# sbokov/AddingDisparityFiltering

Measured on AMD Instinct MI355X. Metric: filtered Mpixels/s (+ achieved HBM GB/s) on 4K disparity, 1/2/4/8 GPUs vs CPU ref, higher is better.
Workload: dtype f32

## Files before the change

### addingdisparityfiltering_amd/__init__.py

```python
from .ximgproc import (
    AdfError,
    COLOR_BGR2GRAY,
    DisparityFilter,
    DisparityWLSFilter,
    FastGlobalSmootherFilter,
    INTER_LINEAR,
    PATH_CONF_BAND,
    PATH_FUSED_FIRST_PASS,
    PATH_MERGED_PREP,
    PATH_SCALED_FUSED,
    PATH_SCALED_HALF,
    SOLVER_EXACT,
    SOLVER_WAVE,
    StereoBM,
    StereoMatcher,
    StereoSGBM,
    UNKNOWN_DISPARITY,
    computeBadPixelPercent,
    computeMSE,
    createDisparityWLSFilter,
    createDisparityWLSFilterGeneric,
    createFastGlobalSmootherFilter,
    createRightMatcher,
    cvtColor,
    fastGlobalSmootherFilter,
    filterSpeckles,
    releaseCachedMemory,
    getDisparityVis,
    halfSize,
    matcherViews,
    readGT,
    resize,
    speckleWorkspaceBytes,
)

__version__ = "0.1.0"
```

### addingdisparityfiltering_amd/_lib.py

```python
import ctypes as C
import os

_HERE = os.path.dirname(os.path.abspath(__file__))
LIB_PATH = os.environ.get("ADF_WLS_LIB") or os.path.join(_HERE, "libadf_wls.so")

ADF_OK, ADF_EBADARG, ADF_ESIZE, ADF_EHIP, ADF_ENOMEM, ADF_ENODEV = range(6)
SOLVER_EXACT, SOLVER_WAVE = 0, 1
PATH_CONF_BAND, PATH_FUSED_FIRST_PASS, PATH_MERGED_PREP, PATH_SCALED_FUSED, PATH_SCALED_HALF = 1, 2, 4, 8, 16
DEPTH_8U, DEPTH_16S, DEPTH_32F = 0, 3, 5


class AdfError(RuntimeError):

    def __init__(self, code, msg):
        super().__init__("adf error %d: %s" % (code, msg))
        self.code = code


class KernelTime(C.Structure):
    _fields_ = [("name", C.c_char * 48), ("launches", C.c_int), ("total_ms", C.c_double),
                ("alg_bytes", C.c_double), ("moved_bytes", C.c_double)]


class Rect(C.Structure):
    _fields_ = [("x", C.c_int), ("y", C.c_int), ("width", C.c_int), ("height", C.c_int)]


_vp, _i, _d, _pd, _sz = C.c_void_p, C.c_int, C.c_double, C.c_ssize_t, C.c_size_t
_FILTER_DEV = [_vp, _i, _vp, _pd, _pd, _vp, _pd, _pd, _i, _i, _i, _vp, _pd, _pd, _vp, _pd, _pd,
               C.POINTER(Rect), _vp]
_FILTER_SCALED_DEV = [_vp, _i, _vp, _pd, _pd, _i, _i, _vp, _pd, _pd, _i, _i, _i, _vp, _pd, _pd, _vp, _pd, _pd,
                      C.POINTER(Rect), _vp]
SYMBOLS = [
    ("adf_version", _i, []),
    ("adf_last_error", C.c_char_p, []),
    ("adf_device_count", _i, []),
    ("adf_device_pci_bus_id", _i, [_i, C.c_char_p, _i]),
    ("adf_wls_create", _i, [C.POINTER(_vp), _i, _i, _i, _i, _i, _i]),
    ("adf_wls_destroy", None, [_vp]),
    ("adf_wls_set_lambda", _i, [_vp, _d]),
    ("adf_wls_get_lambda", _i, [_vp, C.POINTER(_d)]),
    ("adf_wls_set_sigma_color", _i, [_vp, _d]),
    ("adf_wls_get_sigma_color", _i, [_vp, C.POINTER(_d)]),
    ("adf_wls_set_lrc_thresh", _i, [_vp, _i]),
    ("adf_wls_get_lrc_thresh", _i, [_vp, C.POINTER(_i)]),
    ("adf_wls_set_depth_discontinuity_radius", _i, [_vp, _i]),
    ("adf_wls_get_depth_discontinuity_radius", _i, [_vp, C.POINTER(_i)]),
    ("adf_wls_set_fgs_params", _i, [_vp, _d, _i]),
    ("adf_wls_set_solver", _i, [_vp, _i]),
    ("adf_wls_get_solver", _i, [_vp, C.POINTER(_i)]),
    ("adf_wls_get_last_solver", _i, [_vp, C.POINTER(_i)]),
    ("adf_wls_get_last_path", _i, [_vp, C.POINTER(_i)]),
    ("adf_wls_filter_device", _i, _FILTER_DEV),
    ("adf_wls_filter_host", _i, _FILTER_DEV[:-1]),
    ("adf_wls_filter_scaled_device", _i, _FILTER_SCALED_DEV),
    ("adf_wls_filter_scaled_host", _i, _FILTER_SCALED_DEV[:-1]),
    ("adf_wls_get_confidence_device", _i, [_vp, _i, _vp, _pd, _vp]),
    ("adf_wls_get_confidence_host", _i, [_vp, _i, _vp, _pd]),
    ("adf_wls_get_device", _i, [_vp, C.POINTER(_i)]),
    ("adf_wls_get_roi", _i, [_vp, C.POINTER(Rect)]),
    ("adf_wls_sync", _i, [_vp, _vp]),
    ("adf_wls_workspace_bytes", _sz, [_vp]),
    ("adf_wls_profile_enable", _i, [_vp, _i]),
    ("adf_wls_profile_read", _i, [_vp, _vp, _i, C.POINTER(_i)]),
    ("adf_fgs_create", _i, [C.POINTER(_vp), _vp, _pd, _i, _i, _i, _d, _d, _d, _i, _i]),
    ("adf_fgs_create_device", _i, [C.POINTER(_vp), _vp, _pd, _i, _i, _i, _d, _d, _d, _i, _i, _vp]),
    ("adf_fgs_destroy", None, [_vp]),
    ("adf_release_cached_memory", None, []),
    ("adf_weight_table_host", _i, [C.c_float, _vp, _i]),
    ("adf_fgs_get_device", _i, [_vp, C.POINTER(_i)]),
    ("adf_fgs_get_solver", _i, [_vp, C.POINTER(_i)]),
    ("adf_fgs_filter_host", _i, [_vp, _vp, _pd, _vp, _pd, _i, _i]),
    ("adf_fgs_filter_device", _i, [_vp, _vp, _pd, _vp, _pd, _i, _i, _vp]),
    ("adf_compute_mse_host", _i, [_vp, _pd, _vp, _pd, _i, _i, C.POINTER(Rect), C.POINTER(_d)]),
    ("adf_compute_mse_device", _i, [_vp, _pd, _vp, _pd, _i, _i, C.POINTER(Rect), C.POINTER(_d), _vp]),
    ("adf_compute_bad_pixel_percent_host", _i, [_vp, _pd, _vp, _pd, _i, _i, C.POINTER(Rect), _i, C.POINTER(_d)]),
    ("adf_compute_bad_pixel_percent_device", _i, [_vp, _pd, _vp, _pd, _i, _i, C.POINTER(Rect), _i, C.POINTER(_d), _vp]),
    ("adf_get_disparity_vis_host", _i, [_vp, _pd, _vp, _pd, _i, _i, _d]),
    ("adf_get_disparity_vis_device", _i, [_vp, _pd, _vp, _pd, _i, _i, _d, _vp]),
    ("adf_bm_create", _i, [C.POINTER(_vp), _i, _i]),
    ("adf_bm_destroy", None, [_vp]),
    ("adf_bm_set_params", _i, [_vp, _i, _i, _i, _i, _i, _i]),
    ("adf_bm_get_device", _i, [_vp, C.POINTER(_i)]),
    ("adf_bm_get_params", _i, [_vp] + [C.POINTER(_i)] * 6),
    ("adf_bm_compute_device", _i, [_vp, _i, _vp, _pd, _pd, _vp, _pd, _pd, _i, _i, _vp, _pd, _pd, _vp]),
    ("adf_bm_compute_both_device", _i, [_vp, _i, _vp, _pd, _pd, _vp, _pd, _pd, _i, _i, _vp, _pd, _pd, _vp, _pd, _pd, _vp]),
    ("adf_bm_compute_host", _i, [_vp, _i, _vp, _pd, _pd, _vp, _pd, _pd, _i, _i, _vp, _pd, _pd]),
    ("adf_sgbm_create", _i, [C.POINTER(_vp), _i, _i, _i]),
    ("adf_sgbm_destroy", None, [_vp]),
    ("adf_sgbm_get_device", _i, [_vp, C.POINTER(_i)]),
    ("adf_sgbm_set_params", _i, [_vp] + [_i] * 8),
    ("adf_sgbm_get_params", _i, [_vp] + [C.POINTER(_i)] * 8),
    ("adf_sgbm_set_disp12_max_diff", _i, [_vp, _i]),
    ("adf_sgbm_get_disp12_max_diff", _i, [_vp, C.POINTER(_i)]),
    ("adf_sgbm_compute_device", _i, [_vp, _i, _vp, _pd, _pd, _vp, _pd, _pd, _i, _i, _i, _vp, _pd, _pd, _vp]),
    ("adf_sgbm_compute_host", _i, [_vp, _i, _vp, _pd, _pd, _vp, _pd, _pd, _i, _i, _i, _vp, _pd, _pd]),
    ("adf_filter_speckles_workspace_bytes", _sz, [_i, _i, _i]),
    ("adf_filter_speckles_device", _i, [_i, _vp, _pd, _pd, _i, _i, _i, _i, _i, _vp, _sz, _vp]),
    ("adf_filter_speckles_host", _i, [_i, _vp, _pd, _pd, _i, _i, _i, _i, _i]),
    ("adf_half_size", _i, [_i, C.POINTER(_i)]),
    ("adf_prepare_views_device", _i, [_i, _vp, _pd, _pd, _i, _i, _i, _vp, _pd, _pd, _i, _i, _i, _vp]),
    ("adf_prepare_views_host", _i, [_i, _vp, _pd, _pd, _i, _i, _i, _vp, _pd, _pd, _i, _i, _i]),
]

_lib = None


def lib():
    global _lib
    if _lib is None:
        if not os.path.exists(LIB_PATH):
            raise ImportError(
                "%s is missing: build the HIP extension first "
                "(python -c 'import __graft_entry__ as g; g.build()')" % LIB_PATH)
        L = C.CDLL(LIB_PATH)
        for name, res, args in SYMBOLS:
            try:
                fn = getattr(L, name)
            except AttributeError:
                if os.environ.get("ADF_WLS_LIB"):
                    continue
                raise
            fn.restype = res
            fn.argtypes = args
        _lib = L
    return _lib


def check(rc):
    if rc != ADF_OK:
        raise AdfError(rc, lib().adf_last_error().decode("utf-8", "replace"))


def device_pci_bus_id(device):
    buf = C.create_string_buffer(64)
    check(lib().adf_device_pci_bus_id(int(device), buf, 64))
    return buf.value.decode()
```

### addingdisparityfiltering_amd/csrc/adf_api.hip

```cpp
#include "adf_host.h"

#include <cmath>
#include <cstdio>
#include <cstdlib>
#include <cstring>
#include <new>

using namespace adf;

static inline int round_up(int v, int m) { return (v + m - 1) / m * m; }

static Geom make_geom(int W, int H, int rx, int ry, int rw, int rh)
{
    Geom g;
    g.W = W; g.H = H; g.rx = rx; g.ry = ry; g.rw = rw; g.rh = rh;
    g.pw = round_up(rw, 64);
    g.ph = round_up(rh, 64);
    size_t a = (size_t)round_up(rh, TILE_ROWS) * g.pw, b = (size_t)rw * g.ph;
    g.plane = ((a > b ? a : b) + 63) / 64 * 64;
    g.frame = (size_t)W * H;
    g.cx0 = (4 - (rx & 3)) & 3;
    g.cpitch = round_up(W + g.cx0 + 3, 4);
    g.cframe = (size_t)g.cpitch * H;
    return g;
}

static Geom plain_conf_layout(Geom g) { g.cx0 = 0; g.cpitch = g.W; g.cframe = g.frame; return g; }

enum KClass { K_FILL = 0, K_WEIGHTS, K_DISC, K_LRC, K_PROLOGUE, K_PASS_H_FIRST, K_PASS_H, K_PASS_V, K_PASS_V_LAST, K_RESIZE, K_COUNT };
static const char* const kclass_names[K_COUNT] = {"fill_outside", "weights", "discontinuity", "lrc_confidence",
                                                  "plain_prologue", "pass_h_first", "pass_h", "pass_v", "pass_v_last", "resize"};
struct Profiler {
    bool on = false;
    struct Rec { int cls; hipEvent_t a, b; double alg, moved; };
    std::vector<Rec> recs;
    std::vector<hipEvent_t> pool;
    hipEvent_t get()
    {
        if (!pool.empty()) { hipEvent_t e = pool.back(); pool.pop_back(); return e; }
        hipEvent_t e = nullptr;
        if (hipEventCreate(&e) != hipSuccess) return nullptr;
        return e;
    }
    void clear() { for (auto& r : recs) { pool.push_back(r.a); pool.push_back(r.b); } recs.clear(); }
    void destroy() { clear(); for (auto e : pool) hipEventDestroy(e); pool.clear(); }
};
struct ProfScope {
    Profiler* p; hipStream_t st; Profiler::Rec r{};
    ProfScope(Profiler* prof, int cls, double alg, double moved, hipStream_t s) : p(prof && prof->on ? prof : nullptr), st(s)
    {
        if (!p) return;
        r.cls = cls; r.alg = alg; r.moved = moved; r.a = p->get(); r.b = p->get();
        if (r.a) hipEventRecord(r.a, st);
    }
    ~ProfScope()
    {
        if (!p) return;
        if (r.b) hipEventRecord(r.b, st);
        if (r.a && r.b) p->recs.push_back(r);
    }
};

struct SolvePlanes {
    float* CH; float* CV;
    float* D; float* F0; float* F1;
    float* A0; float* A1;
    float* B0; float* B1;
};

struct FinalOut {
    int epilogue; void* out; ptrdiff_t stride, pair_stride; int x0, y0, cn, c;
};

static double epilogue_bytes(int epilogue) { return epilogue == EPI_F32 ? 4.0 : epilogue == EPI_U8 ? 1.0 : 2.0; }

template <class Args>
static void set_final_out(Args& a, const FinalOut& fo)
{
    a.out = fo.out; a.out_stride = fo.stride; a.out_pair_stride = fo.pair_stride;
    a.out_x0 = fo.x0; a.out_y0 = fo.y0; a.out_cn = fo.cn; a.out_c = fo.c;
}

static int run_passes(bool wave, const Geom& g, const SolvePlanes& p, int n_rhs, float lambda, float atten, int num_iter,
                      const FinalOut& fo, int n_pairs, hipStream_t st, Profiler* prof = nullptr,
                      const FusedInputs* fuse = nullptr)
{
    const double px = (double)g.rw * g.rh * n_pairs;
    float lam = lambda;
    for (int it = 0; it < num_iter; it++, lam *= atten) {
        const bool fused = it == 0 && fuse, last = it == num_iter - 1;
        const int epi = last ? fo.epilogue : EPI_PLANES;
        const double lo_b = (fused && fuse->lo_conf) ? 6.0 * fuse->lo_scale_x * fuse->lo_scale_y : 6.0;
        const double hb = fused ? (4.0 + lo_b + 8.0) * px : (4.0 + 8.0 * n_rhs) * px;
        const double out_b = (last ? epilogue_bytes(fo.epilogue) : 4.0 * n_rhs) * px;
        const double vb = (4.0 + 4.0 * n_rhs) * px + out_b;
        if (wave) {
            WavePassArgs h{}, v{};
            h.C = p.CH; h.U0 = p.A0; h.U1 = p.A1;
            h.nscan = g.rh; h.len = g.rw; h.pitch = g.pw; h.plane = g.plane; h.lambda = lam;
            if (fused) h.fuse = *fuse;
            v.C = p.CV; v.U0 = p.A0; v.U1 = p.A1;
            v.nscan = g.rw; v.len = g.rh; v.pitch = g.pw; v.plane = g.plane; v.lambda = lam;
            if (last) set_final_out(v, fo);
            {
                ProfScope ps(prof, fused ? K_PASS_H_FIRST : K_PASS_H, hb, hb, st);
                HIP_TRY(launch_wave_hpass(h, n_rhs, n_pairs, st));
            }
            ProfScope ps(prof, last ? K_PASS_V_LAST : K_PASS_V, vb, vb, st);
            HIP_TRY(launch_wave_vpass(v, n_rhs, epi, n_pairs, st));
        } else {
            PassArgs h{}, v{};
            h.C = p.CH; h.U0 = p.A0; h.U1 = p.A1; h.D = p.D; h.F0 = p.F0; h.F1 = p.F1; h.O0 = p.B0; h.O1 = p.B1;
            h.nscan = g.rh; h.len = g.rw; h.pitch_in = g.ph; h.pitch_out = g.pw; h.plane = g.plane; h.lambda = lam;
            v.C = p.CV; v.U0 = p.B0; v.U1 = p.B1; v.D = p.D; v.F0 = p.F0; v.F1 = p.F1; v.O0 = p.A0; v.O1 = p.A1;
            v.nscan = g.rw; v.len = g.rh; v.pitch_in = g.pw; v.pitch_out = g.ph; v.plane = g.plane; v.lambda = lam;
            if (last) set_final_out(v, fo);
            {
                ProfScope ps(prof, K_PASS_H, hb, (12.0 + 16.0 * n_rhs) * px, st);
                HIP_TRY(launch_exact_pass(h, n_rhs, EPI_PLANES, n_pairs, st));
            }
            ProfScope ps(prof, last ? K_PASS_V_LAST : K_PASS_V, vb, (12.0 + 12.0 * n_rhs) * px + out_b, st);
            HIP_TRY(launch_exact_pass(v, n_rhs, epi, n_pairs, st));
        }
    }
    return ADF_OK;
}

static bool wave_fits(const Geom& g)
{
    return g.rw >= 2 && g.rh >= 2 && g.rw <= wave_max_row_len() && g.rh <= wave_max_col_len();
}

struct ConfResize {
    float* clo; int dW, dH; adf_rect rlo;
    Geom ghi;
    bool band_map;
    int n_pairs;
};

struct adf_wls {
    int device = 0;
    int left_offset = 0, right_offset = 0, top_offset = 0, bottom_offset = 0;
    int min_disp = 0;
    bool use_confidence = true;
    double lambda = 8000.0, sigma_color = 1.0;
    int lrc_thresh = 24, disc_radius = 5;
    float roll_off = 0.001f;
    double atten = 0.25; int num_iter = 3;
    int solver = ADF_SOLVER_WAVE;
    int last_solver = ADF_SOLVER_WAVE;
    adf_rect roi{0, 0, 0, 0};
    int last_W = 0, last_H = 0, last_pairs = 0;
    int last_cpitch = 0, last_cx0 = 0;
    long long conf_sig[4] = {0, 0, 0, 0};
    int last_path = 0;
    Lut lut;
    DevBuf ws;
    DevBuf conf;
    DevBuf stage;
    DevBuf scaled;
    size_t ws_limit = (size_t)64 << 30;
    Profiler prof;
    long long ws_sig[8] = {0, 0, 0, 0, 0, 0, 0, 0};
    hipStream_t side = nullptr;
    hipEvent_t ev_fork = nullptr, ev_join = nullptr;
    bool overlap = true;
    struct LazyConf { bool pending = false; ConfResize resize{}; } lazy_conf;
    bool scaled_half = true;
    bool scaled_fuse = true;
    bool conf_band = true;
    bool merge_small = true;
    static bool null_caller_of(hipStream_t s) { return s == nullptr || s == hipStreamLegacy || s == hipStreamPerThread; }
    int ensure_side(hipStream_t caller)
    {
        if (side) return ADF_OK;
        int least = 0, greatest = 0, prio = 0, cp = 0;
        if (hipDeviceGetStreamPriorityRange(&least, &greatest) != hipSuccess) { least = greatest = 0; (void)hipGetLastError(); }
        if (null_caller_of(caller) || stream_is_capturing(caller) || hipStreamGetPriority(caller, &cp) != hipSuccess) { cp = 0; (void)hipGetLastError(); }
        prio = (cp != greatest) ? greatest : (greatest < least ? greatest + 1 : greatest);
        if (null_caller_of(caller)) HIP_TRY(hipStreamCreateWithFlags(&side, hipStreamNonBlocking));
        else HIP_TRY(hipStreamCreateWithPriority(&side, hipStreamNonBlocking, prio));
        HIP_TRY(hipEventCreateWithFlags(&ev_fork, hipEventDisableTiming));
        HIP_TRY(hipEventCreateWithFlags(&ev_join, hipEventDisableTiming));
        return ADF_OK;
    }
};

extern "C" int adf_wls_create(adf_wls_t** out, int use_confidence, int l, int r, int t, int b, int min_disp)
{
    if (!out) return fail(ADF_EBADARG, "adf_wls_create: out is NULL");
    *out = nullptr;
    if (l < 0 || r < 0 || t < 0 || b < 0) return fail(ADF_EBADARG, "adf_wls_create: negative offset");
    int n = 0;
    if (hipGetDeviceCount(&n) != hipSuccess || n <= 0)
        return fail(ADF_ENODEV, "adf_wls_create: no HIP device visible");
    adf_wls* h = new (std::nothrow) adf_wls();
    if (!h) return fail(ADF_ENOMEM, "adf_wls_create: out of host memory");
    if (hipGetDevice(&h->device) != hipSuccess) { delete h; return fail(ADF_EHIP, "hipGetDevice failed"); }
    h->use_confidence = use_confidence != 0;
    h->left_offset = l; h->right_offset = r; h->top_offset = t; h->bottom_offset = b;
    h->min_disp = 0; (void)min_disp;
    if (const char* e = getenv("ADF_WS_LIMIT_GB")) {
        double gb = atof(e);
        if (gb > 0) h->ws_limit = (size_t)(gb * (double)((size_t)1 << 30));
    }
    if (const char* e = getenv("ADF_NO_OVERLAP")) h->overlap = atoi(e) == 0;
    if (const char* e = getenv("ADF_CONF_BAND")) h->conf_band = atoi(e) != 0;
    if (const char* e = getenv("ADF_SCALED_FUSE")) h->scaled_fuse = atoi(e) != 0;
    if (const char* e = getenv("ADF_LO_HALF")) h->scaled_half = atoi(e) != 0;
    if (const char* e = getenv("ADF_MERGE_SMALL")) h->merge_small = atoi(e) != 0;
    *out = h;
    return ADF_OK;
}

extern "C" void adf_wls_destroy(adf_wls_t* h)
{
    if (!h) return;
    DeviceScope ds(h->device);
    h->lut.release(); h->ws.release(); h->conf.release(); h->stage.release(); h->scaled.release();
    h->prof.destroy();
    if (h->ev_fork) hipEventDestroy(h->ev_fork);
    if (h->ev_join) hipEventDestroy(h->ev_join);
    if (h->side) hipStreamDestroy(h->side);
    delete h;
}


extern "C" int adf_wls_set_lambda(adf_wls_t* h, double v) { NEED_HANDLE(h); h->lambda = v; return ADF_OK; }
extern "C" int adf_wls_get_lambda(const adf_wls_t* h, double* v) { NEED_HANDLE(h); if (v) *v = h->lambda; return ADF_OK; }
extern "C" int adf_wls_set_sigma_color(adf_wls_t* h, double v) { NEED_HANDLE(h); h->sigma_color = v; return ADF_OK; }
extern "C" int adf_wls_get_sigma_color(const adf_wls_t* h, double* v) { NEED_HANDLE(h); if (v) *v = h->sigma_color; return ADF_OK; }
extern "C" int adf_wls_set_lrc_thresh(adf_wls_t* h, int v) { NEED_HANDLE(h); h->lrc_thresh = v; return ADF_OK; }
extern "C" int adf_wls_get_lrc_thresh(const adf_wls_t* h, int* v) { NEED_HANDLE(h); if (v) *v = h->lrc_thresh; return ADF_OK; }
extern "C" int adf_wls_set_depth_discontinuity_radius(adf_wls_t* h, int v) { NEED_HANDLE(h); h->disc_radius = v; return ADF_OK; }
extern "C" int adf_wls_get_depth_discontinuity_radius(const adf_wls_t* h, int* v) { NEED_HANDLE(h); if (v) *v = h->disc_radius; return ADF_OK; }

extern "C" int adf_wls_set_fgs_params(adf_wls_t* h, double atten, int num_iter)
{
    NEED_HANDLE(h);
    if (num_iter < 1) return fail(ADF_EBADARG, "num_iter must be >= 1 (FGS.cpp:143)");
    h->atten = atten; h->num_iter = num_iter;
    return ADF_OK;
}

extern "C" int adf_wls_set_solver(adf_wls_t* h, int solver)
{
    NEED_HANDLE(h);
    if (solver != ADF_SOLVER_EXACT && solver != ADF_SOLVER_WAVE) return fail(ADF_EBADARG, "unknown solver %d", solver);
    h->solver = solver;
    return ADF_OK;
}
extern "C" int adf_wls_get_solver(const adf_wls_t* h, int* v) { NEED_HANDLE(h); if (v) *v = h->solver; return ADF_OK; }
extern "C" int adf_wls_get_last_solver(const adf_wls_t* h, int* v) { NEED_HANDLE(h); if (v) *v = h->last_solver; return ADF_OK; }
extern "C" int adf_wls_get_last_path(const adf_wls_t* h, int* v) { NEED_HANDLE(h); if (v) *v = h->last_path; return ADF_OK; }

extern "C" int adf_wls_get_device(const adf_wls_t* h, int* device) { NEED_HANDLE(h); if (device) *device = h->device; return ADF_OK; }
extern "C" int adf_wls_get_roi(const adf_wls_t* h, adf_rect* roi) { NEED_HANDLE(h); if (roi) *roi = h->roi; return ADF_OK; }
extern "C" size_t adf_wls_workspace_bytes(const adf_wls_t* h)
{
    return h ? h->ws.bytes + h->conf.bytes + h->stage.bytes + h->scaled.bytes + h->lut.bytes() : 0;
}

extern "C" int adf_wls_sync(adf_wls_t* h, void* stream)
{
    NEED_HANDLE(h);
    DeviceScope ds(h->device);
    HIP_TRY(hipStreamSynchronize((hipStream_t)stream));
    return ADF_OK;
}

static int ensure_conf_planes(adf_wls* h, const Geom& g, int n_pairs, hipStream_t st)
{
    int rc = h->conf.reserve(g.cframe * sizeof(float) * (size_t)n_pairs, st, FILL_ZERO);
    if (rc) return rc;
    const long long sig[4] = {g.W, g.H, g.cx0, n_pairs};
    if (memcmp(sig, h->conf_sig, sizeof(sig)) != 0) {
        HIP_TRY(hipMemsetAsync(h->conf.p, 0, h->conf.bytes, st));
        memcpy(h->conf_sig, sig, sizeof(sig));
    }
    return ADF_OK;
}

static size_t wls_pair_ws_bytes(const Geom& g, bool conf, bool wave, bool disc_maps)
{
    size_t planes = wave ? (conf ? 4 : 3) : (conf ? 9 : 6);
    return planes * g.plane * sizeof(float) + (conf && disc_maps ? 2 * g.frame * sizeof(float) : 0);
}

static int resolve_roi(const adf_wls* h, const adf_rect* roi_in, int w, int hgt, adf_rect& roi)
{
    if (roi_in && roi_in->width * roi_in->height != 0) roi = *roi_in;
    else roi = adf_rect{h->left_offset, h->top_offset, w - h->left_offset - h->right_offset, hgt - h->top_offset - h->bottom_offset};
    if (roi.width <= 0 || roi.height <= 0 || roi.x < 0 || roi.y < 0 || roi.x + roi.width > w || roi.y + roi.height > hgt)
        return fail(ADF_ESIZE, "ROI (%d,%d,%d,%d) does not fit a %dx%d map", roi.x, roi.y, roi.width, roi.height, w, hgt);
    return ADF_OK;
}

static int check_right_map(const int16_t* dispR, ptrdiff_t sR, int w)
{
    if (!dispR) return fail(ADF_EBADARG, "disparity_map_right is required with use_confidence");
    if (sR < (ptrdiff_t)w * 2) return fail(ADF_ESIZE, "right disparity stride smaller than a row");
    return ADF_OK;
}

static int check_radius(const adf_wls* h)
{
    if (h->disc_radius < 0 || h->disc_radius > max_disc_radius())
        return fail(ADF_EBADARG, "depth discontinuity radius %d outside [0,%d]", h->disc_radius, max_disc_radius());
    return ADF_OK;
}

static float* const UNALLOCATED = reinterpret_cast<float*>(uintptr_t(256));

static WavePassArgs first_pass_probe(const FusedInputs& f, int len)
{
    WavePassArgs a{};
    a.fuse = f; a.len = len;
    return a;
}

static FusedInputs view_fuse(const float* conf, const int16_t* dl, ptrdiff_t sL, ptrdiff_t psL, const Geom& g)
{
    FusedInputs f{};
    f.conf_in = conf; f.conf_frame = g.cframe; f.conf_pitch = g.cpitch; f.conf_x0 = g.cx0 + g.rx; f.conf_y0 = g.ry;
    f.dl_in = dl; f.dl_stride = sL; f.dl_pair_stride = psL; f.dl_x0 = g.rx; f.dl_y0 = g.ry;
    return f;
}

struct ScaledStage {
    const int16_t* dispL; ptrdiff_t sL, psL;
    const int16_t* dispR; ptrdiff_t sR, psR;
    float resize_factor, x_ratio;
    char* dhi; size_t dhi_bytes;
    float *cl, *cr;
    ConfResize lo;
    bool fuse_lo;
    float* taps;
};

static FusedInputs lo_fuse(const adf_wls* h, const ScaledStage& s, int first, const Geom& g)
{
    const ConfResize& c = s.lo;
    const size_t lo = (size_t)c.dW * c.dH;
    FusedInputs f{};
    f.lo_conf = c.clo + (size_t)first * lo; f.lo_conf_stride = c.dW; f.lo_conf_pair = (ptrdiff_t)lo;
    f.lo_dl = (const int16_t*)((const char*)s.dispL + (ptrdiff_t)first * s.psL); f.lo_dl_stride = s.sL; f.lo_dl_pair = s.psL;
    f.lo_w = c.dW; f.lo_h = c.dH; f.hi_x0 = g.rx; f.hi_y0 = g.ry;
    f.lo_scale_x = (double)c.dW / c.ghi.W; f.lo_scale_y = (double)c.dH / c.ghi.H; f.lo_post_scale = s.x_ratio;
    if (c.band_map) {
        f.lo_zero_outside = 1; f.lo_vx0 = c.rlo.x; f.lo_vy0 = c.rlo.y; f.lo_vx1 = c.rlo.x + c.rlo.width; f.lo_vy1 = c.rlo.y + c.rlo.height;
    }
    f.lo_taps = s.taps; f.lo_half = h->scaled_half ? 1 : 0;
    return f;
}

static int resize_conf_planes(adf_wls_t* h, const ConfResize& c, hipStream_t st, Profiler* prof)
{
    const size_t lo = (size_t)c.dW * c.dH;
    const Geom& ghi = c.ghi;
    const double Fhi = (double)ghi.W * ghi.H * c.n_pairs;
    ResizeArgs rc32{c.clo, (ptrdiff_t)c.dW * 4, (ptrdiff_t)(lo * 4), c.dW, c.dH, (float*)h->conf.p + ghi.cx0, (ptrdiff_t)ghi.cpitch * 4,
                    (ptrdiff_t)(ghi.cframe * 4), ghi.W, ghi.H, (double)c.dW / ghi.W, (double)c.dH / ghi.H, 1.0f, 0};
    if (c.band_map) { rc32.zero_outside = 1; rc32.vx0 = c.rlo.x; rc32.vy0 = c.rlo.y; rc32.vx1 = c.rlo.x + c.rlo.width; rc32.vy1 = c.rlo.y + c.rlo.height; }
    ProfScope ps(prof, K_RESIZE, 4.0 * Fhi + 4.0 * (double)lo * c.n_pairs, 4.0 * Fhi + 4.0 * (double)lo * c.n_pairs, st);
    HIP_TRY(launch_resize_linear(rc32, c.n_pairs, st));
    return ADF_OK;
}

static int scaled_conf_map(adf_wls_t* h, const ScaledStage& s, hipStream_t st, Profiler* prof)
{
    const ConfResize& c = s.lo;
    const Geom glo = plain_conf_layout(make_geom(c.dW, c.dH, c.rlo.x, c.rlo.y, c.rlo.width, c.rlo.height));
    const size_t lo = (size_t)c.dW * c.dH;
    const double Plo = (double)c.rlo.width * c.rlo.height * c.n_pairs;
    const int rrx = c.dW - (c.rlo.x + c.rlo.width);
    const float roll_off = h->roll_off / (s.resize_factor * s.resize_factor);
    const int thresh_lo = (int)(s.resize_factor * h->lrc_thresh);
    if (c.band_map) {
        ConfBandArgs ba{s.dispL, s.sL, s.psL, s.dispR, s.sR, s.psR, c.clo, glo, rrx, thresh_lo, h->disc_radius, roll_off, 0};
        ProfScope ps(prof, K_LRC, 8.0 * Plo, 8.0 * Plo, st);
        HIP_TRY(launch_conf_band(ba, c.n_pairs, st));
        return ADF_OK;
    }
    DiscArgs da{{s.dispL, s.dispR}, {s.sL, s.sR}, {s.psL, s.psR}, {c.rlo.x, rrx}, c.rlo.y, c.rlo.width, c.rlo.height,
                h->disc_radius, roll_off, {s.cl, s.cr}, c.dW, lo, -1};
    {
        ProfScope ps(prof, K_DISC, 4.0 * Plo, 12.0 * Plo, st);
        HIP_TRY(launch_discontinuity(da, c.n_pairs, st));
    }
    LrcArgs la{s.dispL, s.sL, s.psL, s.dispR, s.sR, s.psR, s.cl, s.cr, c.clo, nullptr, 0, 0, 0, nullptr, nullptr, glo, rrx, thresh_lo, ORIENT_N};
    ProfScope ps(prof, K_LRC, 4.0 * (double)lo * c.n_pairs, 4.0 * (double)lo * c.n_pairs + 12.0 * Plo, st);
    HIP_TRY(launch_lrc_prologue(la, c.n_pairs, st));
    return ADF_OK;
}

static int scaled_resize(adf_wls_t* h, const ScaledStage& s, hipStream_t st, Profiler* prof)
{
    const ConfResize& c = s.lo;
    int rc = h->use_confidence ? resize_conf_planes(h, c, st, prof) : ADF_OK;
    if (rc) return rc;
    const int W = c.ghi.W, H = c.ghi.H;
    const size_t lo = (size_t)c.dW * c.dH;
    const double Fhi = (double)W * H * c.n_pairs;
    ResizeArgs r16{s.dispL, s.sL, s.psL, c.dW, c.dH, s.dhi, (ptrdiff_t)W * 2, (ptrdiff_t)s.dhi_bytes, W, H, (double)c.dW / W, (double)c.dH / H, s.x_ratio, 1};
    ProfScope ps(prof, K_RESIZE, 2.0 * Fhi + 2.0 * (double)lo * c.n_pairs, 2.0 * Fhi + 2.0 * (double)lo * c.n_pairs, st);
    HIP_TRY(launch_resize_linear(r16, c.n_pairs, st));
    return ADF_OK;
}

enum ConfStage {
    CONF_NONE,
    CONF_SCALED,
    CONF_SCALED_LO,
    CONF_MERGED,
    CONF_BAND,
    CONF_LEFT,
    CONF_TWO_KERNEL,
};

struct ChunkPlan {
    ConfStage stage;
    bool fork_weights;
    bool outside_on_side;
};

struct WlsPlan {
    bool wave;
    bool fused_first;
    bool band;
    size_t per_pair; int chunk;
    ChunkPlan full, tail;
    int path;
};

static ChunkPlan plan_chunk(const adf_wls* h, ConfStage stage, bool wave)
{
    const bool fork = stage != CONF_NONE && stage != CONF_MERGED && h->overlap;
    return ChunkPlan{stage, fork, fork && wave && stage != CONF_TWO_KERNEL};
}

static WlsPlan plan_wls(const adf_wls* h, const Geom& g, int n_pairs, const int16_t* dispL, ptrdiff_t sL, ptrdiff_t psL,
                        ptrdiff_t sG, int gch, const ScaledStage* scaled)
{
    WlsPlan p{};
    const bool conf = h->use_confidence;
    p.wave = h->solver == ADF_SOLVER_WAVE && wave_fits(g);
    ConfStage stage = !conf ? CONF_NONE
                    : scaled ? (scaled->fuse_lo ? CONF_SCALED_LO : CONF_SCALED)
                    : (p.wave && h->disc_radius <= conf_left_max_radius()) ? CONF_LEFT : CONF_TWO_KERNEL;
    const float* planes = h->conf.p ? (const float*)h->conf.p : UNALLOCATED;
    p.fused_first = stage == CONF_SCALED_LO ||
                    ((stage == CONF_SCALED || stage == CONF_LEFT) && p.wave &&
                     wave_hpass_can_fuse(first_pass_probe(view_fuse(planes, dispL, sL, psL, g), g.rw)));
    p.band = stage == CONF_LEFT && p.fused_first && h->conf_band && conf_band_fits(g, h->disc_radius);
    if (p.band) stage = CONF_BAND;
    p.per_pair = wls_pair_ws_bytes(g, conf, p.wave, !p.band);
    p.chunk = (int)(h->ws_limit / p.per_pair);
    if (p.chunk < 1) p.chunk = 1;
    if (p.chunk > n_pairs) p.chunk = n_pairs;
    auto chunk_of = [&](int n) {
        const bool merged = p.band && h->merge_small && prep_small_fits(g, h->disc_radius, gch, n) && prep_small_guide_fits(g, sG, gch);
        return plan_chunk(h, merged ? CONF_MERGED : stage, p.wave);
    };
    p.full = chunk_of(p.chunk);
    p.tail = chunk_of(n_pairs % p.chunk ? n_pairs % p.chunk : p.chunk);
    p.path = ((p.band || (scaled && scaled->lo.band_map)) ? ADF_PATH_CONF_BAND : 0) |
             (p.fused_first ? ADF_PATH_FUSED_FIRST_PASS : 0) |
             ((p.full.stage == CONF_MERGED || p.tail.stage == CONF_MERGED) ? ADF_PATH_MERGED_PREP : 0);
    if (stage == CONF_SCALED_LO)
        p.path |= ADF_PATH_SCALED_FUSED |
                  (wave_hpass_lo_half(first_pass_probe(lo_fuse(h, *scaled, 0, g), g.rw)) ? ADF_PATH_SCALED_HALF : 0);
    return p;
}

static int wls_filter_impl(adf_wls_t* h, int n_pairs,
                           const int16_t* dispL, ptrdiff_t sL, ptrdiff_t psL,
                           const uint8_t* view, ptrdiff_t sG, ptrdiff_t psG, int gch, int W, int H,
                           int16_t* out, ptrdiff_t sO, ptrdiff_t psO,
                           const int16_t* dispR, ptrdiff_t sR, ptrdiff_t psR,
                           const adf_rect* roi_in, hipStream_t st, const ScaledStage* scaled = nullptr)
{
    NEED_HANDLE(h);
    if (!dispL || W <= 0 || H <= 0) return fail(ADF_EBADARG, "disparity_map_left is empty");
    if (!view || (gch != 1 && gch != 3)) return fail(ADF_EBADARG, "left_view must be CV_8UC1 or CV_8UC3");
    if (!out) return fail(ADF_EBADARG, "filtered_disparity_map is NULL");
    if (n_pairs < 1) return fail(ADF_EBADARG, "n_pairs must be >= 1");
    if (sL < (ptrdiff_t)W * 2 || sO < (ptrdiff_t)W * 2 || sG < (ptrdiff_t)W * gch)
        return fail(ADF_ESIZE, "row stride smaller than a row");
    const bool conf = h->use_confidence;
    int rc;
    if (conf && !scaled && (rc = check_right_map(dispR, sR, W))) return rc;
    if (h->lambda < 0 || h->sigma_color < 0) return fail(ADF_EBADARG, "lambda and sigma_color must be >= 0 (FGS.cpp:143)");
    adf_rect roi;
    if ((rc = resolve_roi(h, roi_in, W, H, roi))) return rc;
    if (conf && (rc = check_radius(h))) return rc;

    DeviceScope ds(h->device);
    const Geom g = make_geom(W, H, roi.x, roi.y, roi.width, roi.height);
    h->lazy_conf.pending = false;
    h->roi = roi; h->last_W = W; h->last_H = H; h->last_pairs = n_pairs;
    h->last_cpitch = g.cpitch; h->last_cx0 = g.cx0; h->last_path = 0;

    if ((rc = h->lut.ensure((float)h->sigma_color, st))) return rc;
    const WlsPlan plan = plan_wls(h, g, n_pairs, dispL, sL, psL, sG, gch, scaled);
    const bool wave = plan.wave;
    h->last_solver = wave ? ADF_SOLVER_WAVE : ADF_SOLVER_EXACT;
    if ((rc = h->ws.reserve(plan.per_pair * (size_t)plan.chunk, st, FILL_ZERO))) return rc;
    if (conf && !scaled && (rc = ensure_conf_planes(h, g, n_pairs, st))) return rc;
    {
        const long long sig[8] = {W, H, roi.x, roi.y, roi.width, roi.height, (long long)plan.band * 4 + (long long)wave * 2 + conf, plan.chunk};
        if (memcmp(sig, h->ws_sig, sizeof(sig)) != 0) {
            HIP_TRY(hipMemsetAsync(h->ws.p, 0, h->ws.bytes, st));
            memcpy(h->ws_sig, sig, sizeof(sig));
        }
    }
    float* base = (float*)h->ws.p;
    auto take = [&](size_t elems) { float* p = base; base += elems * (size_t)plan.chunk; return p; };
    SolvePlanes p{};
    p.CH = take(g.plane); p.CV = take(g.plane); p.A0 = take(g.plane);
    if (!wave) { p.D = take(g.plane); p.F0 = take(g.plane); p.B0 = take(g.plane); }
    float *cL = nullptr, *cR = nullptr;
    if (conf) {
        p.A1 = take(g.plane);
        if (!wave) { p.F1 = take(g.plane); p.B1 = take(g.plane); }
        if (!plan.band) { cL = take(g.frame); cR = take(g.frame); }
    }
    const int orient_h = wave ? ORIENT_N : ORIENT_T;
    const int orient_u2 = wave ? ORIENT_PAIR : ORIENT_T;
    const int orient_cv = wave ? ORIENT_STRIP : ORIENT_N;
    const int16_t fill = (int16_t)(16 * (h->min_disp - 1));
    const int rrx = W - (roi.x + roi.width);
    const int thresh = (int)(1.0f * h->lrc_thresh);
    Profiler* prof = &h->prof;
    h->last_path = plan.path;

    for (int first = 0; first < n_pairs; first += plan.chunk) {
        const int n = (n_pairs - first < plan.chunk) ? n_pairs - first : plan.chunk;
        const ChunkPlan& cp = n == plan.chunk ? plan.full : plan.tail;
        const int16_t* dL = (const int16_t*)((const char*)dispL + (ptrdiff_t)first * psL);
        const int16_t* dR = dispR ? (const int16_t*)((const char*)dispR + (ptrdiff_t)first * psR) : nullptr;
        const uint8_t* gv = view + (ptrdiff_t)first * psG;
        int16_t* o = (int16_t*)((char*)out + (ptrdiff_t)first * psO);
        float* confp = conf ? (float*)h->conf.p + (size_t)first * g.cframe : nullptr;
        const double F = (double)g.frame * n, P = (double)g.rw * g.rh * n;
        OutsideArgs oa{o, sO, psO, fill, scaled ? nullptr : confp, g};
        const double ob = (oa.conf ? 6.0 : 2.0) * (F - P);
        auto fill_outside = [&](hipStream_t s) { ProfScope ps(prof, K_FILL, ob, ob, s); return launch_outside(oa, n, s); };
        WeightArgs wa{gv, sG, psG, gch, h->lut.cur, p.CH, p.CV, orient_h, orient_cv, g,
                      wave ? nullptr : p.B0};
        ConfBandArgs ba{dL, sL, psL, dR, sR, psR, confp, g, rrx, thresh, h->disc_radius, h->roll_off, 0};
        DiscArgs da{{dL, dR}, {sL, sR}, {psL, psR}, {roi.x, rrx}, roi.y, roi.width, roi.height, h->disc_radius, h->roll_off,
                    {cL, cR}, W, g.frame, cp.stage == CONF_LEFT ? 1 : -1};
        const FusedInputs fuse = cp.stage == CONF_SCALED_LO ? lo_fuse(h, *scaled, first, g) : view_fuse(confp, dL, sL, psL, g);

        hipStream_t wst = st;
        if (cp.fork_weights) {
            if ((rc = h->ensure_side(st))) return rc;
            HIP_TRY(hipEventRecord(h->ev_fork, st));
            HIP_TRY(hipStreamWaitEvent(h->side, h->ev_fork, 0));
            wst = h->side;
        }
        if (cp.stage == CONF_NONE || cp.outside_on_side) HIP_TRY(fill_outside(wst));
        if (cp.stage == CONF_NONE && scaled && first == 0 && (rc = scaled_resize(h, *scaled, st, prof))) return rc;
        if (cp.stage != CONF_MERGED) {
            ProfScope ps(prof, K_WEIGHTS, (gch + 8.0) * P, (gch + 8.0) * P, wst);
            HIP_TRY(launch_weights(wa, n, wst));
        }
        if (cp.fork_weights) HIP_TRY(hipEventRecord(h->ev_join, h->side));

        switch (cp.stage) {
        case CONF_NONE: {
            PlainPrologueArgs pa{dL, sL, psL, ADF_16S, 1, 0, p.A0, g, orient_h};
            ProfScope ps(prof, K_PROLOGUE, 6.0 * P, 6.0 * P, st);
            HIP_TRY(launch_plain_prologue(pa, n, st));
            break;
        }
        case CONF_SCALED: {
            if (!cp.outside_on_side) HIP_TRY(fill_outside(st));
            if (first == 0 && ((rc = scaled_conf_map(h, *scaled, st, prof)) || (rc = scaled_resize(h, *scaled, st, prof)))) return rc;
            if (plan.fused_first) break;
            PlainPrologueArgs pa{dL, sL, psL, ADF_16S, 1, 0, p.A0, g, orient_u2, confp, p.A1};
            ProfScope ps(prof, K_PROLOGUE, 14.0 * P, 14.0 * P, st);
            HIP_TRY(launch_plain_prologue(pa, n, st));
            break;
        }
        case CONF_SCALED_LO:
            if (!cp.outside_on_side) HIP_TRY(fill_outside(st));
            if (first != 0) break;
            if ((rc = scaled_conf_map(h, *scaled, st, prof))) return rc;
            if (!stream_is_capturing(st)) h->lazy_conf = adf_wls::LazyConf{true, scaled->lo};
            else if ((rc = resize_conf_planes(h, scaled->lo, st, prof))) return rc;
            break;
        case CONF_MERGED: {
            const double b = (8.0 + gch + 8.0) * P + 6.0 * (F - P);
            ProfScope ps(prof, K_LRC, b, b, st);
            HIP_TRY(launch_prep_small(ba, wa, oa, n, st));
            break;
        }
        case CONF_BAND: {
            {
                ProfScope ps(prof, K_LRC, 8.0 * P, 8.0 * P, st);
                HIP_TRY(launch_conf_band(ba, n, st));
            }
            if (!cp.outside_on_side) HIP_TRY(fill_outside(st));
            break;
        }
        case CONF_LEFT: {
            {
                ProfScope ps(prof, K_DISC, 2.0 * P, 6.0 * P, st);
                HIP_TRY(launch_discontinuity(da, n, st));
            }
            const bool fused = plan.fused_first;
            ConfLeftArgs ca{dL, sL, psL, dR, sR, psR, cR, confp, fused ? nullptr : p.A0, fused ? nullptr : p.A1,
                            g, rrx, thresh, h->disc_radius, h->roll_off};
            {
                const double wu = fused ? 0.0 : 8.0;
                ProfScope ps(prof, K_LRC, (4.0 + wu) * P, (12.0 + wu) * P, st);
                HIP_TRY(launch_conf_left(ca, n, st));
            }
            if (!cp.outside_on_side) HIP_TRY(fill_outside(st));
            break;
        }
        case CONF_TWO_KERNEL: {
            {
                ProfScope ps(prof, K_DISC, 4.0 * P, 12.0 * P, st);
                HIP_TRY(launch_discontinuity(da, n, st));
            }
            LrcArgs la{dL, sL, psL, dR, sR, psR, cL, cR, confp, o, sO, psO, fill, p.A0, p.A1, g, rrx, thresh, orient_u2};
            ProfScope ps(prof, K_LRC, 4.0 * F + 8.0 * P + 2.0 * (F - P), 4.0 * F + 20.0 * P + 2.0 * (F - P), st);
            HIP_TRY(launch_lrc_prologue(la, n, st));
            break;
        }
        }
        if (cp.fork_weights) HIP_TRY(hipStreamWaitEvent(st, h->ev_join, 0));
        FinalOut fo{conf ? EPI_WLS_CONF : EPI_I16, o, sO, psO, roi.x, roi.y, 1, 0};
        rc = run_passes(wave, g, p, conf ? 2 : 1, (float)h->lambda, (float)h->atten, h->num_iter, fo, n, st, prof,
                        plan.fused_first ? &fuse : nullptr);
        if (rc) return rc;
    }
    return ADF_OK;
}

extern "C" int adf_wls_filter_device(adf_wls_t* h, int n_pairs,
                                     const int16_t* dispL, ptrdiff_t sL, ptrdiff_t psL,
                                     const uint8_t* view, ptrdiff_t sG, ptrdiff_t psG, int gch, int W, int H,
                                     int16_t* out, ptrdiff_t sO, ptrdiff_t psO,
                                     const int16_t* dispR, ptrdiff_t sR, ptrdiff_t psR,
                                     const adf_rect* roi_in, void* stream)
{
    return wls_filter_impl(h, n_pairs, dispL, sL, psL, view, sG, psG, gch, W, H, out, sO, psO, dispR, sR, psR, roi_in,
                           (hipStream_t)stream);
}

extern "C" int adf_wls_filter_scaled_device(adf_wls_t* h, int n_pairs,
                                            const int16_t* dispL, ptrdiff_t sL, ptrdiff_t psL, int dW, int dH,
                                            const uint8_t* view, ptrdiff_t sG, ptrdiff_t psG, int gch, int W, int H,
                                            int16_t* out, ptrdiff_t sO, ptrdiff_t psO,
                                            const int16_t* dispR, ptrdiff_t sR, ptrdiff_t psR,
                                            const adf_rect* roi_in, void* stream)
{
    NEED_HANDLE(h);
    hipStream_t st = (hipStream_t)stream;
    if (dW == W && dH == H)
        return wls_filter_impl(h, n_pairs, dispL, sL, psL, view, sG, psG, gch, W, H, out, sO, psO, dispR, sR, psR, roi_in, st);
    if (!dispL || dW <= 0 || dH <= 0 || W <= 0 || H <= 0) return fail(ADF_EBADARG, "disparity_map_left is empty");
    if (n_pairs < 1) return fail(ADF_EBADARG, "n_pairs must be >= 1");
    if (sL < (ptrdiff_t)dW * 2) return fail(ADF_ESIZE, "row stride smaller than a row");
    const bool conf = h->use_confidence;
    int rc;
    if (conf && ((rc = check_right_map(dispR, sR, dW)) || (rc = check_radius(h)))) return rc;
    adf_rect rlo;
    if ((rc = resolve_roi(h, roi_in, dW, dH, rlo))) return rc;
    const float resize_factor = dW / (float)W;
    const float x_ratio = W / (float)dW, y_ratio = H / (float)dH;
    adf_rect rhi{(int)(rlo.x * x_ratio), (int)(rlo.y * y_ratio), (int)(rlo.width * x_ratio), (int)(rlo.height * y_ratio)};
    if (rhi.width <= 0 || rhi.height <= 0 || rhi.x + rhi.width > W || rhi.y + rhi.height > H)
        return fail(ADF_ESIZE, "scaled ROI (%d,%d,%d,%d) does not fit the %dx%d view", rhi.x, rhi.y, rhi.width, rhi.height, W, H);

    DeviceScope ds(h->device);
    h->lazy_conf.pending = false;
    const size_t lo = (size_t)dW * dH, hi = (size_t)W * H;
    const Geom ghi = make_geom(W, H, rhi.x, rhi.y, rhi.width, rhi.height);
    ScaledStage s{dispL, sL, psL, dispR, sR, psR, resize_factor, x_ratio, nullptr, 0, nullptr, nullptr,
                  ConfResize{UNALLOCATED, dW, dH, rlo, ghi, false, n_pairs}, false, nullptr};
    s.lo.band_map = conf && h->conf_band &&
                    conf_band_fits(plain_conf_layout(make_geom(dW, dH, rlo.x, rlo.y, rlo.width, rlo.height)), h->disc_radius);
    s.fuse_lo = conf && h->scaled_fuse && h->solver == ADF_SOLVER_WAVE && wave_fits(ghi) &&
                wave_hpass_can_fuse_lo(first_pass_probe(lo_fuse(h, s, 0, ghi), ghi.rw));
    s.dhi_bytes = s.fuse_lo ? 0 : (hi * 2 + 255) / 256 * 256;
    const size_t maps_bytes = ((size_t)n_pairs * (s.dhi_bytes + (conf ? 3 * lo * sizeof(float) : 0)) + 255) / 256 * 256;
    const size_t need = maps_bytes + (s.fuse_lo ? 2 * ((size_t)rhi.width + 4) * sizeof(float) : 0);
    if ((rc = h->scaled.reserve(need, st, FILL_ZERO))) return rc;
    s.dhi = (char*)h->scaled.p;
    s.cl = (float*)(s.dhi + (size_t)n_pairs * s.dhi_bytes);
    s.cr = s.cl + (size_t)n_pairs * lo;
    s.lo.clo = s.cr + (size_t)n_pairs * lo;
    s.taps = s.fuse_lo ? (float*)((char*)h->scaled.p + maps_bytes) : nullptr;
    if (conf && (rc = ensure_conf_planes(h, ghi, n_pairs, st))) return rc;
    rc = wls_filter_impl(h, n_pairs, s.fuse_lo ? dispL : (const int16_t*)s.dhi, (ptrdiff_t)W * 2, (ptrdiff_t)s.dhi_bytes,
                         view, sG, psG, gch, W, H, out, sO, psO, nullptr, 0, 0, &rhi, st, &s);
    h->roi = rlo;
    return rc;
}

extern "C" int adf_wls_filter_scaled_host(adf_wls_t* h, int n_pairs,
                                          const int16_t* dispL, ptrdiff_t sL, ptrdiff_t psL, int dW, int dH,
                                          const uint8_t* view, ptrdiff_t sG, ptrdiff_t psG, int gch, int W, int H,
                                          int16_t* out, ptrdiff_t sO, ptrdiff_t psO,
                                          const int16_t* dispR, ptrdiff_t sR, ptrdiff_t psR,
                                          const adf_rect* roi)
{
    NEED_HANDLE(h);
    if (!dispL || !view || !out || W <= 0 || H <= 0 || dW <= 0 || dH <= 0 || n_pairs < 1)
        return fail(ADF_EBADARG, "adf_wls_filter_host: empty input");
    if (gch != 1 && gch != 3) return fail(ADF_EBADARG, "left_view must be CV_8UC1 or CV_8UC3");
    if (h->use_confidence && !dispR) return fail(ADF_EBADARG, "disparity_map_right is required with use_confidence");
    DeviceScope ds(h->device);
    hipStream_t st = nullptr;
    const size_t dbytes = (size_t)dW * dH * 2, obytes = (size_t)W * H * 2, gbytes = (size_t)W * H * gch;
    const size_t dpad = (dbytes + 255) / 256 * 256, opad = (obytes + 255) / 256 * 256, gpad = (gbytes + 255) / 256 * 256;
    const size_t need = (size_t)n_pairs * (2 * dpad + opad + gpad);
    int rc = h->stage.reserve(need, st, FILL_ZERO);
    if (rc) return rc;
    char* dLd = (char*)h->stage.p;
    char* dRd = dLd + (size_t)n_pairs * dpad;
    char* od = dRd + (size_t)n_pairs * dpad;
    char* gd = od + (size_t)n_pairs * opad;
    if ((rc = copy_images(dLd, (size_t)dW * 2, dpad, dispL, sL, psL, (size_t)dW * 2, dH, n_pairs, hipMemcpyHostToDevice, st))) return rc;
    if (dispR && (rc = copy_images(dRd, (size_t)dW * 2, dpad, dispR, sR, psR, (size_t)dW * 2, dH, n_pairs, hipMemcpyHostToDevice, st))) return rc;
    if ((rc = copy_images(gd, (size_t)W * gch, gpad, view, sG, psG, (size_t)W * gch, H, n_pairs, hipMemcpyHostToDevice, st))) return rc;
    rc = adf_wls_filter_scaled_device(h, n_pairs, (const int16_t*)dLd, (ptrdiff_t)dW * 2, (ptrdiff_t)dpad, dW, dH,
                                      (const uint8_t*)gd, (ptrdiff_t)W * gch, (ptrdiff_t)gpad, gch, W, H,
                                      (int16_t*)od, (ptrdiff_t)W * 2, (ptrdiff_t)opad,
                                      dispR ? (const int16_t*)dRd : nullptr, (ptrdiff_t)dW * 2, (ptrdiff_t)dpad, roi, st);
    if (rc) return rc;
    if ((rc = copy_images(out, sO, psO, od, (size_t)W * 2, opad, (size_t)W * 2, H, n_pairs, hipMemcpyDeviceToHost, st))) return rc;
    HIP_TRY(hipStreamSynchronize(st));
    return ADF_OK;
}

extern "C" int adf_wls_filter_host(adf_wls_t* h, int n_pairs,
                                   const int16_t* dispL, ptrdiff_t sL, ptrdiff_t psL,
                                   const uint8_t* view, ptrdiff_t sG, ptrdiff_t psG, int gch, int W, int H,
                                   int16_t* out, ptrdiff_t sO, ptrdiff_t psO,
                                   const int16_t* dispR, ptrdiff_t sR, ptrdiff_t psR,
                                   const adf_rect* roi)
{
    return adf_wls_filter_scaled_host(h, n_pairs, dispL, sL, psL, W, H, view, sG, psG, gch, W, H, out, sO, psO,
                                      dispR, sR, psR, roi);
}

extern "C" int adf_wls_profile_enable(adf_wls_t* h, int on)
{
    NEED_HANDLE(h);
    DeviceScope ds(h->device);
    h->prof.clear();
    h->prof.on = on != 0;
    return ADF_OK;
}

extern "C" int adf_wls_profile_read(adf_wls_t* h, adf_kernel_time* out, int capacity, int* count)
{
    NEED_HANDLE(h);
    if (!out || !count || capacity < 1) return fail(ADF_EBADARG, "adf_wls_profile_read: bad output buffer");
    DeviceScope ds(h->device);
    adf_kernel_time acc[K_COUNT];
    memset(acc, 0, sizeof(acc));
    for (int k = 0; k < K_COUNT; k++) snprintf(acc[k].name, sizeof(acc[k].name), "%s", kclass_names[k]);
    for (auto& r : h->prof.recs) {
        HIP_TRY(hipEventSynchronize(r.b));
        float ms = 0.0f;
        HIP_TRY(hipEventElapsedTime(&ms, r.a, r.b));
        acc[r.cls].launches++; acc[r.cls].total_ms += ms; acc[r.cls].alg_bytes += r.alg; acc[r.cls].moved_bytes += r.moved;
    }
    int n = 0;
    for (int k = 0; k < K_COUNT && n < capacity; k++)
        if (acc[k].launches) out[n++] = acc[k];
    *count = n;
    return ADF_OK;
}

static int conf_copy(adf_wls_t* h, int pair, float* dst, ptrdiff_t stride, hipMemcpyKind kind, hipStream_t st)
{
    if (!dst) return fail(ADF_EBADARG, "confidence destination is NULL");
    if (!h->use_confidence || !h->conf.p || h->last_pairs == 0)
        return fail(ADF_EBADARG, "no confidence map: filter() has not run with use_confidence");
    if (pair < 0 || pair >= h->last_pairs) return fail(ADF_EBADARG, "pair %d out of range [0,%d)", pair, h->last_pairs);
    if (stride < (ptrdiff_t)h->last_W * 4) return fail(ADF_ESIZE, "confidence stride smaller than a row");
    if (h->lazy_conf.pending) {
        int rc = resize_conf_planes(h, h->lazy_conf.resize, st, nullptr);
// ... 214 lines not shown
```

### addingdisparityfiltering_amd/csrc/adf_host.h

```cpp
#pragma once

#include "adf_internal.h"
#include "../../include/adf_wls.h"

#include <memory>
#include <vector>

namespace adf {

int fail(int code, const char* fmt, ...);

#define HIP_TRY(expr)                                                                              \
    do {                                                                                           \
        hipError_t e_ = (expr);                                                                    \
        if (e_ != hipSuccess)                                                                      \
            return adf::fail(e_ == hipErrorOutOfMemory ? ADF_ENOMEM : ADF_EHIP, "%s failed: %s",   \
                             #expr, hipGetErrorString(e_));                                        \
    } while (0)
#define NEED_HANDLE(h) do { if (!(h)) return adf::fail(ADF_EBADARG, "%s: handle is NULL", __func__); } while (0)

struct DeviceScope {
    int prev = -1; bool switched = false;
    explicit DeviceScope(int dev)
    {
        if (hipGetDevice(&prev) == hipSuccess && prev != dev) switched = hipSetDevice(dev) == hipSuccess;
    }
    ~DeviceScope() { if (switched) hipSetDevice(prev); }
};

bool stream_is_capturing(hipStream_t st);

enum Fill { FILL_NONE, FILL_ZERO };
struct DevBuf {
    void* p = nullptr; size_t bytes = 0;
    int reserve(size_t need, hipStream_t st, Fill fill);
    void release() { if (p) hipFree(p); p = nullptr; bytes = 0; }
};

hipError_t device_malloc(void** p, size_t bytes);
void* cache_take(int device, size_t need, hipStream_t st, size_t* bytes);
void cache_give(int device, void* p, size_t bytes, hipStream_t st);
void cache_give_event(int device, void* p, size_t bytes, hipEvent_t ready);

struct Scratch {
    int device = 0; void* p = nullptr; size_t bytes = 0; hipStream_t st = nullptr;
    Scratch() = default;
    Scratch(const Scratch&) = delete;
    Scratch& operator=(const Scratch&) = delete;
    int take(size_t need, hipStream_t stream);
    ~Scratch() { if (p) cache_give(device, p, bytes, st); }
};

struct LutTable;
struct Lut {
    static constexpr int LUT_CACHE = 8;
    struct Entry { std::shared_ptr<LutTable> t; unsigned long long used; };
    std::vector<Entry> tables;
    const float* cur = nullptr;
    unsigned long long tick = 0;
    size_t bytes() const { return tables.size() * sizeof(float) * ADF_LUT_LEVELS; }
    int ensure(float s, hipStream_t st);
    void release() { tables.clear(); cur = nullptr; }
};

int copy_images(void* dst, size_t dst_pitch, ptrdiff_t dst_image_stride, const void* src, size_t src_pitch,
                ptrdiff_t src_image_stride, size_t row_bytes, size_t rows, int n, hipMemcpyKind kind, hipStream_t st);

}
```

### addingdisparityfiltering_amd/csrc/adf_host.hip

```cpp
#include "adf_host.h"

#include <cmath>
#include <cstdarg>
#include <cstdio>
#include <mutex>
#include <thread>

using namespace adf;

static thread_local char g_err[512] = "";

int adf::fail(int code, const char* fmt, ...)
{
    va_list ap;
    va_start(ap, fmt);
    vsnprintf(g_err, sizeof(g_err), fmt, ap);
    va_end(ap);
    return code;
}

extern "C" int adf_version(void) { return ADF_VERSION; }
extern "C" const char* adf_last_error(void) { return g_err; }
extern "C" int adf_device_count(void)
{
    int n = 0;
    if (hipGetDeviceCount(&n) != hipSuccess) return 0;
    return n;
}

extern "C" int adf_device_pci_bus_id(int device, char* buf, int len)
{
    if (!buf || len < 16) return fail(ADF_EBADARG, "adf_device_pci_bus_id: buffer of at least 16 bytes required");
    buf[0] = 0;
    HIP_TRY(hipDeviceGetPCIBusId(buf, len, device));
    return ADF_OK;
}

bool adf::stream_is_capturing(hipStream_t st)
{
    hipStreamCaptureStatus cs = hipStreamCaptureStatusNone;
    if (hipStreamIsCapturing(st, &cs) != hipSuccess) { (void)hipGetLastError(); return false; }
    return cs != hipStreamCaptureStatusNone;
}

int adf::DevBuf::reserve(size_t need, hipStream_t st, Fill fill)
{
    if (need <= bytes) return ADF_OK;
    if (p) { HIP_TRY(hipStreamSynchronize(st)); HIP_TRY(hipFree(p)); p = nullptr; bytes = 0; }
    need = (need + 255) / 256 * 256;
    HIP_TRY(device_malloc(&p, need));
    bytes = need;
    if (fill == FILL_ZERO) HIP_TRY(hipMemsetAsync(p, 0, need, st));
    return ADF_OK;
}

struct adf::LutTable {
    int device = 0; float sigma = 0; float* dev = nullptr;
    LutTable() = default;
    LutTable(const LutTable&) = delete;
    LutTable& operator=(const LutTable&) = delete;
    ~LutTable() { if (dev) { DeviceScope ds(device); hipFree(dev); } }
};

struct LutStore {
    static constexpr size_t CAP = 16;
    std::mutex m;
    std::vector<std::shared_ptr<LutTable>> tables;
    static LutStore& get() { static LutStore* s = new LutStore; return *s; }
    std::shared_ptr<LutTable> find(int device, float sigma)
    {
        std::lock_guard<std::mutex> lk(m);
        for (size_t k = 0; k < tables.size(); k++)
            if (tables[k]->device == device && tables[k]->sigma == sigma) {
                auto t = tables[k];
                tables.erase(tables.begin() + (ptrdiff_t)k); tables.push_back(t);
                return t;
            }
        return nullptr;
    }
    void add(const std::shared_ptr<LutTable>& t)
    {
        std::lock_guard<std::mutex> lk(m);
        if (tables.size() >= CAP) tables.erase(tables.begin());
        tables.push_back(t);
    }
    void clear() { std::lock_guard<std::mutex> lk(m); tables.clear(); }
};

static void lut_build_host(float s, float* host)
{
    auto span = [&](int a, int b) { for (int i = a; i < b; i++) host[i] = -expf(-sqrtf((float)i) / s); };
    int n = ADF_LUT_LEVELS;
    if (s > 0.0f) {
        const double lim = 110.0 * (double)s;
        if (lim * lim * 1.001 + 2.0 < (double)ADF_LUT_LEVELS) {
            int i0 = (int)(lim * lim * 1.001) + 2;
            while (i0 < ADF_LUT_LEVELS && !(-sqrtf((float)i0) / s <= -110.0f)) i0++;
            n = i0;
        }
    }
    for (int i = n; i < ADF_LUT_LEVELS; i++) host[i] = -0.0f;
    unsigned hw = std::thread::hardware_concurrency();
    int nt = (int)(hw >= 16 ? 8 : hw >= 4 ? hw / 2 : 1);
    if (n < 32768) nt = 1;
    if (nt <= 1) { span(0, n); return; }
    std::vector<std::thread> th;
    const int per = (n + nt - 1) / nt;
    bool ok = true;
    int done = std::min(per, n);
    for (int t = 1; t < nt && ok; t++) {
        const int a = t * per, b = std::min(n, a + per);
        if (a >= b) break;
        try { th.emplace_back(span, a, b); done = b; } catch (...) { ok = false; }
    }
    span(0, std::min(per, n));
    for (auto& t : th) t.join();
    if (done < n) span(done, n);
}

int adf::Lut::ensure(float s, hipStream_t st)
{
    for (auto& e : tables)
        if (e.t->sigma == s) { e.used = ++tick; cur = e.t->dev; return ADF_OK; }
    if ((int)tables.size() >= LUT_CACHE) {
        size_t lru = 0;
        for (size_t k = 1; k < tables.size(); k++) if (tables[k].used < tables[lru].used) lru = k;
        HIP_TRY(hipStreamSynchronize(st));
        tables.erase(tables.begin() + (ptrdiff_t)lru);
    }
    int device = 0;
    HIP_TRY(hipGetDevice(&device));
    std::shared_ptr<LutTable> t = LutStore::get().find(device, s);
    if (!t) {
        std::vector<float> host(ADF_LUT_LEVELS);
        lut_build_host(s, host.data());
        float* d = nullptr;
        HIP_TRY(hipMalloc(&d, sizeof(float) * ADF_LUT_LEVELS));
        hipError_t e = hipMemcpy(d, host.data(), sizeof(float) * ADF_LUT_LEVELS, hipMemcpyHostToDevice);
        if (e != hipSuccess) { hipFree(d); return fail(ADF_EHIP, "LUT upload failed: %s", hipGetErrorString(e)); }
        t = std::make_shared<LutTable>();
        t->device = device; t->sigma = s; t->dev = d;
        LutStore::get().add(t);
    }
    tables.push_back(Entry{t, ++tick});
    cur = t->dev;
    return ADF_OK;
}

struct BlockCache {
    struct Ent { int device; void* p; size_t bytes; hipEvent_t ready; };
    static constexpr size_t CAP_BYTES = (size_t)3 << 30;
    static constexpr size_t CAP_ENTRIES = 8;
    std::mutex m;
    std::vector<Ent> ents;
    size_t total = 0;
    static BlockCache& get() { static BlockCache* c = new BlockCache; return *c; }
    static void drop(const Ent& e)
    {
        DeviceScope ds(e.device);
        if (e.ready) { hipEventSynchronize(e.ready); hipEventDestroy(e.ready); }
        hipFree(e.p);
    }
    void* take(int device, size_t need, hipStream_t st, size_t* bytes)
    {
        Ent hit{};
        {
            std::lock_guard<std::mutex> lk(m);
            size_t best = ents.size();
            for (size_t k = 0; k < ents.size(); k++)
                if (ents[k].device == device && ents[k].bytes >= need && ents[k].bytes <= need + need / 4 + ((size_t)1 << 20) &&
                    (best == ents.size() || ents[k].bytes < ents[best].bytes))
                    best = k;
            if (best == ents.size()) return nullptr;
            hit = ents[best];
            ents.erase(ents.begin() + (ptrdiff_t)best);
            total -= hit.bytes;
        }
        if (hit.ready) {
            const hipError_t e = hipStreamWaitEvent(st, hit.ready, 0);
            if (e != hipSuccess) hipEventSynchronize(hit.ready);
            hipEventDestroy(hit.ready);
        }
        *bytes = hit.bytes;
        return hit.p;
    }
    void give(int device, void* p, size_t bytes, hipEvent_t ready)
    {
        std::vector<Ent> out;
        {
            std::lock_guard<std::mutex> lk(m);
            ents.push_back(Ent{device, p, bytes, ready});
            total += bytes;
            while (!ents.empty() && (total > CAP_BYTES || ents.size() > CAP_ENTRIES)) {
                out.push_back(ents.front());
                total -= ents.front().bytes;
                ents.erase(ents.begin());
            }
        }
        for (auto& e : out) drop(e);
    }
    void clear()
    {
        std::vector<Ent> out;
        { std::lock_guard<std::mutex> lk(m); out.swap(ents); total = 0; }
        for (auto& e : out) drop(e);
    }
};

extern "C" int adf_weight_table_host(float sigma_color, float* table, int levels)
{
    if (!table || levels != ADF_LUT_LEVELS) return fail(ADF_EBADARG, "table must hold %d floats", ADF_LUT_LEVELS);
    if (!(sigma_color >= 0.0f)) return fail(ADF_EBADARG, "sigma_color must be >= 0 (FGS.cpp:143)");
    lut_build_host(sigma_color, table);
    return ADF_OK;
}

namespace adf {
hipError_t device_malloc(void** p, size_t bytes)
{
    hipError_t e = hipMalloc(p, bytes);
    if (e == hipErrorOutOfMemory) {
        (void)hipGetLastError();
        BlockCache::get().clear();
        e = hipMalloc(p, bytes);
    }
    if (e != hipSuccess) *p = nullptr;
    return e;
}

void* cache_take(int device, size_t need, hipStream_t st, size_t* bytes) { return BlockCache::get().take(device, need, st, bytes); }

void cache_give(int device, void* p, size_t bytes, hipStream_t st)
{
    hipEvent_t ev = nullptr;
    if (hipEventCreateWithFlags(&ev, hipEventDisableTiming) != hipSuccess || hipEventRecord(ev, st) != hipSuccess) {
        (void)hipGetLastError();
        if (ev) hipEventDestroy(ev);
        ev = nullptr;
        hipStreamSynchronize(st);
    }
    BlockCache::get().give(device, p, bytes, ev);
}

void cache_give_event(int device, void* p, size_t bytes, hipEvent_t ready) { BlockCache::get().give(device, p, bytes, ready); }

int Scratch::take(size_t need, hipStream_t stream)
{
    if (hipGetDevice(&device) != hipSuccess) return fail(ADF_ENODEV, "no HIP device");
    st = stream;
    if ((p = cache_take(device, need, st, &bytes))) return ADF_OK;
    HIP_TRY(device_malloc(&p, need));
    bytes = need;
    return ADF_OK;
}

int copy_images(void* dst, size_t dst_pitch, ptrdiff_t dst_image_stride, const void* src, size_t src_pitch,
                ptrdiff_t src_image_stride, size_t row_bytes, size_t rows, int n, hipMemcpyKind kind, hipStream_t st)
{
    for (int k = 0; k < n; k++)
        HIP_TRY(hipMemcpy2DAsync((char*)dst + k * dst_image_stride, dst_pitch, (const char*)src + k * src_image_stride, src_pitch,
                                 row_bytes, rows, kind, st));
    return ADF_OK;
}
}

extern "C" void adf_release_cached_memory(void)
{
    BlockCache::get().clear();
    LutStore::get().clear();
}
```

### addingdisparityfiltering_amd/csrc/adf_internal.h

```cpp
#pragma once

#include <hip/hip_runtime.h>
#include <stddef.h>
#include <stdint.h>

#define ADF_LUT_LEVELS (3 * 256 * 256)
#define ADF_EPS 1e-43f

namespace adf {

struct Geom {
    int W, H;
    int rx, ry, rw, rh;
    int pw, ph;
    size_t plane;
    size_t frame;
    int cpitch, cx0;
    size_t cframe;
};

enum Orient { ORIENT_N = 0, ORIENT_T = 1, ORIENT_PAIR = 2, ORIENT_STRIP = 3 };
#define ADF_STRIP 16
constexpr int TILE_ROWS = 2;

enum Epilogue {
    EPI_PLANES = 0,
    EPI_WLS_CONF = 1,
    EPI_I16 = 2,
    EPI_F32 = 3,
    EPI_U8 = 4
};

struct DiscArgs {
    const int16_t* disp[2]; ptrdiff_t stride[2], pair_stride[2];
    int rx[2]; int ry, rw, rh;
    int radius; float roll_off;
    float* dst[2]; int W; size_t frame;
    int only_view;
};

struct ConfLeftArgs {
    const int16_t* dL; ptrdiff_t sL, psL;
    const int16_t* dR; ptrdiff_t sR, psR;
    const float* cR;
    float* conf;
    float* U0; float* U1;
    Geom g; int rrx; int thresh;
    int radius; float roll_off;
};

struct ConfBandArgs {
    const int16_t* dL; ptrdiff_t sL, psL;
    const int16_t* dR; ptrdiff_t sR, psR;
    float* conf;
    Geom g; int rrx; int thresh;
    int radius; float roll_off;
    int rows_per_band;
};

struct OutsideArgs {
    int16_t* out; ptrdiff_t stride, pair_stride; int16_t fill;
    float* conf;
    Geom g;
};

struct LrcArgs {
    const int16_t* dL; ptrdiff_t sL, psL;
    const int16_t* dR; ptrdiff_t sR, psR;
    const float* cL; const float* cR;
    float* conf;
    int16_t* out; ptrdiff_t sO, psO; int16_t fill;
    float* U0; float* U1;
    Geom g; int rrx;
    int thresh; int orient;
};

struct PlainPrologueArgs {
    const void* src; ptrdiff_t stride, pair_stride;
    int depth, cn, c;
    float* U0; Geom g; int orient;
    const float* conf; float* U1;
    int pair2, c2;
};

struct ResizeArgs {
    const void* src; ptrdiff_t sstride, spair; int sw, sh;
    void* dst; ptrdiff_t dstride, dpair; int dw, dh;
    double scale_x, scale_y;
    float post_scale; int is16;
    int zero_outside = 0, vx0 = 0, vy0 = 0, vx1 = 0, vy1 = 0;
};

struct WeightArgs {
    const uint8_t* guide; ptrdiff_t stride, pair_stride; int ch;
    const float* lut;
    float* chor; float* cvert; int chor_orient, cvert_orient;
    Geom g;
    float* scratch;
};

struct PassArgs {
    const float* C; const float* U0; const float* U1;
    float* D; float* F0; float* F1;
    float* O0; float* O1;
    void* out; ptrdiff_t out_stride, out_pair_stride;
    int out_x0, out_y0, out_cn, out_c;
    int nscan, len, pitch_in, pitch_out;
    size_t plane;
    float lambda;
};

struct FusedInputs {
    const float* conf_in; size_t conf_frame; int conf_pitch, conf_x0, conf_y0;
    const int16_t* dl_in; ptrdiff_t dl_stride, dl_pair_stride; int dl_x0, dl_y0;
    const float* lo_conf; ptrdiff_t lo_conf_stride, lo_conf_pair;
    const int16_t* lo_dl; ptrdiff_t lo_dl_stride, lo_dl_pair;
    int lo_w, lo_h, hi_x0, hi_y0;
    double lo_scale_x, lo_scale_y; float lo_post_scale;
    int lo_zero_outside, lo_vx0, lo_vy0, lo_vx1, lo_vy1;
    int lo_half;
    float* lo_taps;
};

struct WavePassArgs {
    const float* C; float* U0; float* U1;
    FusedInputs fuse;
    void* out; ptrdiff_t out_stride, out_pair_stride;
    int out_x0, out_y0, out_cn, out_c;
    int nscan, len, pitch;
    size_t plane;
    float lambda;
};
static_assert(sizeof(WavePassArgs) == 280 && offsetof(WavePassArgs, out) == 208 && offsetof(WavePassArgs, nscan) == 248 &&
              offsetof(WavePassArgs, plane) == 264 && offsetof(WavePassArgs, lambda) == 272, "WavePassArgs layout");

hipError_t launch_discontinuity(const DiscArgs& a, int n_pairs, hipStream_t st);
hipError_t launch_lrc_prologue(const LrcArgs& a, int n_pairs, hipStream_t st);
hipError_t launch_conf_left(const ConfLeftArgs& a, int n_pairs, hipStream_t st);
hipError_t launch_outside(const OutsideArgs& a, int n_pairs, hipStream_t st);
bool conf_band_fits(const Geom& g, int radius);
hipError_t launch_conf_band(const ConfBandArgs& a, int n_pairs, hipStream_t st);
bool prep_small_guide_fits(const Geom& g, ptrdiff_t guide_stride, int channels);
bool prep_small_fits(const Geom& g, int radius, int channels, int n_pairs);
hipError_t launch_prep_small(const ConfBandArgs& c, const WeightArgs& w, const OutsideArgs& o, int n_pairs, hipStream_t st);
int conf_left_max_radius();
hipError_t launch_plain_prologue(const PlainPrologueArgs& a, int n_pairs, hipStream_t st);
hipError_t launch_weights(const WeightArgs& a, int n_pairs, hipStream_t st);
hipError_t launch_resize_linear(const ResizeArgs& a, int n_pairs, hipStream_t st);
hipError_t launch_exact_pass(const PassArgs& a, int n_rhs, int epilogue, int n_pairs, hipStream_t st);
hipError_t launch_wave_hpass(const WavePassArgs& a, int n_rhs, int n_pairs, hipStream_t st);
hipError_t launch_wave_vpass(const WavePassArgs& a, int n_rhs, int epilogue, int n_pairs, hipStream_t st);
int wave_max_row_len();
bool wave_hpass_can_fuse(const WavePassArgs& a);
bool wave_hpass_can_fuse_lo(const WavePassArgs& a);
bool wave_hpass_lo_half(const WavePassArgs& a);
int wave_max_col_len();
int max_disc_radius();

#if defined(__HIPCC__)
__device__ __forceinline__ size_t pair_index(int i, int j, int pw)
{
    constexpr int TR = TILE_ROWS;
    return (size_t)(i / TR) * (size_t)(2 * TR * pw) + (size_t)((j >> 4) * (32 * TR) + (i % TR) * 32 + (j & 15));
}
__device__ __forceinline__ size_t strip_index(int i, int j, int rh)
{
    return ((size_t)(j >> 4) * (size_t)rh + (size_t)i) * ADF_STRIP + (size_t)(j & 15);
}
__device__ __forceinline__ int16_t sat16(float v)
{
    if (!(v >= -2147483648.0f && v < 2147483648.0f)) return (int16_t)-32768;
    float r = rintf(v);
    r = fminf(fmaxf(r, -32768.0f), 32767.0f);
    return (int16_t)(int)r;
}
__device__ __forceinline__ uint8_t sat8(float v)
{
    if (!(v >= -2147483648.0f && v < 2147483648.0f)) return (uint8_t)0;
    float r = rintf(v);
    r = fminf(fmaxf(r, 0.0f), 255.0f);
    return (uint8_t)(int)r;
}
__device__ __forceinline__ int reflect101(int p, int len)
{
    if (len == 1) return 0;
    while (p < 0 || p >= len) p = p < 0 ? -p : 2 * (len - 1) - p;
    return p;
}
#endif

}
```

### addingdisparityfiltering_amd/csrc/fgs_wave_h.hip

```cpp
#include "fgs_wave_common.h"

#include <algorithm>

namespace adf {

namespace {
using namespace wave;

constexpr int H_TWO_WAVE_MAX = 60;

constexpr int FUSE_NONE = 0, FUSE_VIEW = 1, FUSE_LO = 2, FUSE_LO_HALF = 3;

__host__ __device__ __forceinline__ void lin_tap(int d, double scale, int sn, int& s0, float& fx)
{
    fx = (float)(((double)d + 0.5) * scale - 0.5);
    s0 = (int)floorf(fx);
    fx -= (float)s0;
    if (s0 < 0) { fx = 0.0f; s0 = 0; }
    if (s0 >= sn - 1) { fx = 0.0f; s0 = sn - 1; }
}
__global__ void __launch_bounds__(256) lo_tap_table_kernel(float* table, int n, int len, int hi_x0, double scale, int sn)
{
    const int j = blockIdx.x * 256 + threadIdx.x;
    if (j >= n) return;
    int s0; float fx;
    lin_tap(hi_x0 + min(j, len - 1), scale, sn, s0, fx);
    table[j] = (float)s0 + fx;
}
__host__ __device__ constexpr int lo_row_cap(int m) { return (((m * 64) / 3) & ~7) < 168 ? 168 : (((m * 64) / 3) & ~7); }
__host__ __device__ constexpr int lo_stage_vec4(int m) { return 12 * lo_row_cap(m) > 256 * m ? (12 * lo_row_cap(m) + 15) / 16 : m * 16; }

template <int M, int R, int FUSED, int NW = 1>
__global__ void __launch_bounds__(64 * NW, (M > (NW == 2 ? 40 : H_TWO_WAVE_MAX) && R > 1) ? 1 : 2) wave_hpass_kernel(WavePassArgs a)
{
    static_assert(M % 4 == 0 && M >= 4, "chunk length must be a multiple of 4");
    static_assert(NW == 1 || NW == 2, "one or two wavefronts per row");
    constexpr bool LO = FUSED == FUSE_LO || FUSED == FUSE_LO_HALF;
    __shared__ float4 stage_all[NW][LO ? lo_stage_vec4(M) : M * 16];
    __shared__ float xch[NW == 2 ? 5 : 1];
    __shared__ float red[NW == 2 ? 5 : 1][NW == 2 ? 128 : 1];
    __shared__ float xsol[NW == 2 ? 2 : 1][NW == 2 ? 128 : 1];
    const int lane = threadIdx.x & 63, wv = NW == 2 ? (int)(threadIdx.x >> 6) : 0;
    float4* stage = stage_all[wv];
    const int v0 = wv * 16 * M;
    const size_t off = (size_t)blockIdx.y * a.plane + (size_t)blockIdx.x * a.pitch;
    const int nvec = a.pitch >> 2;
    constexpr bool PAIR = R > 1;
    constexpr int TR = TILE_ROWS;
    const size_t offU = PAIR ? (size_t)blockIdx.y * 2 * a.plane + (size_t)(blockIdx.x / TR) * (size_t)(2 * TR * a.pitch) + (size_t)(blockIdx.x % TR) * 32 : off;
#define ADF_PIDX(q) (PAIR ? ((((q) >> 3) * (8 * TR)) + ((q) & 7)) : (q))
    const int nvecU = PAIR ? 2 * nvec : nvec;
    constexpr int MQ = M / 4;
    float c[M], f0[M], f1[M];

    float4 tC[M / 4], t0[M / 4], t1[M / 4];
    {
        const float4* sC = reinterpret_cast<const float4*>(a.C + off);
        const float4* s0 = reinterpret_cast<const float4*>(a.U0 + offU);
        const float4* sF = nullptr; const char* sD = nullptr;
        if (FUSED == FUSE_VIEW) {
            sF = reinterpret_cast<const float4*>(a.fuse.conf_in + (size_t)blockIdx.y * a.fuse.conf_frame +
                                                 (size_t)(a.fuse.conf_y0 + blockIdx.x) * a.fuse.conf_pitch + a.fuse.conf_x0);
            sD = reinterpret_cast<const char*>(a.fuse.dl_in) + (ptrdiff_t)blockIdx.y * a.fuse.dl_pair_stride +
                 (ptrdiff_t)(a.fuse.dl_y0 + blockIdx.x) * a.fuse.dl_stride + (ptrdiff_t)a.fuse.dl_x0 * 2;
        }
        const int nfull = a.len >> 2, rem = a.len & 3;
        const int nfused = nfull + (rem ? 1 : 0);
        const unsigned dl_last = (unsigned)a.len * 2u - 8u;
        typedef short v4s_u __attribute__((ext_vector_type(4), aligned(2)));
        short4 draw[FUSED == FUSE_VIEW ? M / 4 : 1];
        const int u0 = PAIR ? 2 * v0 : v0;
        if constexpr (LO) {
            typedef float v4f __attribute__((ext_vector_type(4)));
            typedef float f4u __attribute__((ext_vector_type(4), aligned(4)));
            typedef short s8u __attribute__((ext_vector_type(8), aligned(2)));
            constexpr int KH = (MQ + 1) / 2;
            constexpr int CROW = lo_row_cap(M);
            constexpr int TC4 = (CROW / 4 + 63) / 64, TD8 = (CROW / 8 + 63) / 64;
            static_assert(12 * CROW <= 16 * lo_stage_vec4(M) && CROW % 8 == 0, "two confidence rows and two disparity rows fit the staging buffer");
            const int sw = a.fuse.lo_w, sh = a.fuse.lo_h;
#pragma unroll
            for (int k = 0; k < MQ; k++) {
                const int idx = v0 + 64 * k + lane;
                tC[k] = make_float4(0.f, 0.f, 0.f, 0.f); t0[k] = tC[k]; t1[k] = tC[k];
                if (idx < nvec) { const v4f q = __builtin_nontemporal_load(reinterpret_cast<const v4f*>(sC) + idx); tC[k] = make_float4(q.x, q.y, q.z, q.w); }
            }
            int sy; float fy;
            {
                const int dy = a.fuse.hi_y0 + (int)blockIdx.x;
                fy = (float)(((double)dy + 0.5) * a.fuse.lo_scale_y - 0.5);
                sy = (int)floorf(fy);
                fy -= (float)sy;
            }
            const float b0 = 1.0f - fy, b1 = fy;
            const bool post_scaled = a.fuse.lo_post_scale != 1.0f;
            int yr[2] = {min(max(sy, 0), sh - 1), min(max(sy + 1, 0), sh - 1)};
            yr[0] = __builtin_amdgcn_readfirstlane(yr[0]); yr[1] = __builtin_amdgcn_readfirstlane(yr[1]);
            const float* cbase = a.fuse.lo_conf + (ptrdiff_t)blockIdx.y * a.fuse.lo_conf_pair;
            const char* dbase = reinterpret_cast<const char*>(a.fuse.lo_dl) + (ptrdiff_t)blockIdx.y * a.fuse.lo_dl_pair;
            int ss[2], ns[2];
#pragma unroll
            for (int hh = 0; hh < 2; hh++) {
                const int cfirst = 64 * M * wv + 256 * (hh ? KH : 0);
                const int clast = min(64 * M * wv + 256 * (hh ? MQ : KH), a.len) - 1;
                int s_first = 0, s_last = -2; float f_;
                if (clast >= cfirst) { lin_tap(a.fuse.hi_x0 + cfirst, a.fuse.lo_scale_x, sw, s_first, f_); lin_tap(a.fuse.hi_x0 + clast, a.fuse.lo_scale_x, sw, s_last, f_); }
                ss[hh] = __builtin_amdgcn_readfirstlane(s_first);
                ns[hh] = __builtin_amdgcn_readfirstlane(s_last + 2 - s_first);
            }
            bool need_mask[2];
#pragma unroll
            for (int hh = 0; hh < 2; hh++)
                need_mask[hh] = a.fuse.lo_zero_outside && (yr[0] < a.fuse.lo_vy0 || yr[1] >= a.fuse.lo_vy1 || ss[hh] < a.fuse.lo_vx0 || min(ss[hh] + ns[hh], sw) > a.fuse.lo_vx1);
            v4f rc[2][2][TC4]; s8u rd[2][2][TD8];
            auto fetch = [&](int hh, v4f (&qc)[2][TC4], s8u (&qd)[2][TD8]) {
#pragma unroll
                for (int r = 0; r < 2; r++) {
                    const float* crow = cbase + (ptrdiff_t)yr[r] * a.fuse.lo_conf_stride;
                    const int16_t* drow = reinterpret_cast<const int16_t*>(dbase + (ptrdiff_t)yr[r] * a.fuse.lo_dl_stride);
#pragma unroll
                    for (int t = 0; t < TC4; t++) {
                        const int e = ss[hh] + 4 * (64 * t + lane);
                        qc[r][t] = v4f{0.f, 0.f, 0.f, 0.f};
                        if (4 * (64 * t + lane) < ns[hh]) {
                            if (e + 3 < sw) qc[r][t] = *reinterpret_cast<const f4u*>(crow + e);
                            else {
#pragma unroll
                                for (int c = 0; c < 4; c++) qc[r][t][c] = crow[min(e + c, sw - 1)];
                            }
                        }
                    }
#pragma unroll
                    for (int t = 0; t < TD8; t++) {
                        const int e = ss[hh] + 8 * (64 * t + lane);
                        qd[r][t] = s8u{0, 0, 0, 0, 0, 0, 0, 0};
                        if (8 * (64 * t + lane) < ns[hh]) {
                            if (e + 7 < sw) qd[r][t] = *reinterpret_cast<const s8u*>(drow + e);
                            else {
#pragma unroll
                                for (int c = 0; c < 8; c++) qd[r][t][c] = drow[min(e + c, sw - 1)];
                            }
                        }
                    }
                }
            };
            const float* Lf = reinterpret_cast<const float*>(stage);
            const short* Ls = reinterpret_cast<const short*>(stage) + 4 * CROW;
            v4f* Lf4 = reinterpret_cast<v4f*>(stage);
            typedef short s8a __attribute__((ext_vector_type(8)));
            s8a* Ls8 = reinterpret_cast<s8a*>(stage) + CROW / 2;
            auto put = [&](int hh, const v4f (&qc)[2][TC4], const s8u (&qd)[2][TD8]) {
                const bool rin0 = !a.fuse.lo_zero_outside || (yr[0] >= a.fuse.lo_vy0 && yr[0] < a.fuse.lo_vy1);
                const bool rin1 = !a.fuse.lo_zero_outside || (yr[1] >= a.fuse.lo_vy0 && yr[1] < a.fuse.lo_vy1);
#pragma unroll
                for (int t = 0; t < TC4; t++) {
                    const int i4 = 64 * t + lane, e = ss[hh] + 4 * i4;
                    v4f q0 = qc[0][t], q1 = qc[1][t];
                    if (need_mask[hh]) {
#pragma unroll
                        for (int c = 0; c < 4; c++) {
                            const int ec = min(e + c, sw - 1);
                            const bool cin = ec >= a.fuse.lo_vx0 && ec < a.fuse.lo_vx1;
                            if (!(rin0 && cin)) q0[c] = 0.0f;
                            if (!(rin1 && cin)) q1[c] = 0.0f;
                        }
                    }
                    if (4 * i4 < CROW) {
                        Lf4[2 * i4] = v4f{q0[0], q1[0], q0[1], q1[1]};
                        Lf4[2 * i4 + 1] = v4f{q0[2], q1[2], q0[3], q1[3]};
                    }
                }
#pragma unroll
                for (int t = 0; t < TD8; t++) {
                    const int i8 = 64 * t + lane;
                    const s8u q0 = qd[0][t], q1 = qd[1][t];
                    if (8 * i8 < CROW) {
                        Ls8[2 * i8] = s8a{q0[0], q1[0], q0[1], q1[1], q0[2], q1[2], q0[3], q1[3]};
                        Ls8[2 * i8 + 1] = s8a{q0[4], q1[4], q0[5], q1[5], q0[6], q1[6], q0[7], q1[7]};
                    }
                }
            };
            typedef float f4a8 __attribute__((ext_vector_type(4), aligned(8)));
            typedef short s4a4 __attribute__((ext_vector_type(4), aligned(4)));
            typedef float v2f __attribute__((ext_vector_type(2)));
            const v2f bb0 = {b0, b0}, bb1 = {b1, b1};
            v4f tp[MQ];
            auto load_taps = [&](int hh) {
#pragma unroll
                for (int k = (hh ? KH : 0); k < (hh ? MQ : KH); k++) {
                    const int idx = v0 + 64 * k + lane;
                    tp[k] = v4f{0.f, 0.f, 0.f, 0.f};
                    if (idx < nfused) tp[k] = reinterpret_cast<const v4f*>(a.fuse.lo_taps)[idx];
                }
            };
            fetch(0, rc[0], rd[0]);
            load_taps(0); load_taps(1);
#pragma unroll
            for (int hh = 0; hh < 2; hh++) {
                put(hh, rc[hh], rd[hh]);
                __syncthreads();
                if (hh == 0) {
                    asm volatile("" ::: "memory");
                    fetch(1, rc[1], rd[1]);
                }
#pragma unroll
                for (int k = (hh ? KH : 0); k < (hh ? MQ : KH); k++) {
                    int lane_t = lane;
                    asm volatile("" : "+v"(lane_t) :: "memory");
                    const int idx = v0 + 64 * k + lane_t;
                    f4a8 cq[4]; s4a4 dq[4]; float fxs[4];
                    if constexpr (FUSED == FUSE_LO_HALF) {
                        typedef short s8a4 __attribute__((ext_vector_type(8), aligned(4)));
                        const int sl0 = min(max((int)tp[k][0] - ss[hh], 0), CROW - 4);
                        const f4a8 ca = *reinterpret_cast<const f4a8*>(Lf + 2 * sl0), cb = *reinterpret_cast<const f4a8*>(Lf + 2 * sl0 + 4);
                        const s8a4 da = *reinterpret_cast<const s8a4*>(Ls + 2 * sl0);
                        cq[0] = f4a8{ca[0], ca[1], ca[2], ca[3]}; dq[0] = s4a4{da[0], da[1], da[2], da[3]};
                        cq[1] = f4a8{ca[2], ca[3], cb[0], cb[1]}; dq[1] = s4a4{da[2], da[3], da[4], da[5]};
                        cq[2] = cq[1]; dq[2] = dq[1];
                        cq[3] = f4a8{cb[0], cb[1], cb[2], cb[3]}; dq[3] = s4a4{da[4], da[5], da[6], da[7]};
#pragma unroll
                        for (int c = 0; c < 4; c++) fxs[c] = __builtin_amdgcn_fractf(tp[k][c]);
                    } else {
#pragma unroll
                    for (int c = 0; c < 4; c++) {
                        const float t = tp[k][c];
                        fxs[c] = __builtin_amdgcn_fractf(t);
                        const int sl = min(max((int)t - ss[hh], 0), CROW - 2);
                        cq[c] = *reinterpret_cast<const f4a8*>(Lf + 2 * sl);
                        dq[c] = *reinterpret_cast<const s4a4*>(Ls + 2 * sl);
                    }
                    }
                    float cv[4], dv[4];
#pragma unroll
                    for (int c = 0; c < 4; c++) {
                        const float a0 = 1.0f - fxs[c], a1 = fxs[c];
                        const v2f aa0 = {a0, a0}, aa1 = {a1, a1};
                        const v2f p0 = {cq[c][0], (float)dq[c][0]}, p1 = {cq[c][1], (float)dq[c][1]};
                        const v2f n0 = {cq[c][2], (float)dq[c][2]}, n1 = {cq[c][3], (float)dq[c][3]};
                        const v2f h0 = p0 * aa0 + n0 * aa1, h1 = p1 * aa0 + n1 * aa1;
                        const v2f v = h0 * bb0 + h1 * bb1;
                        const float q1 = fminf(fmaxf(rintf(v[1]), -32768.0f), 32767.0f);
                        const float q2 = fminf(fmaxf(rintf(q1 * a.fuse.lo_post_scale), -32768.0f), 32767.0f);
                        cv[c] = v[0];
                        dv[c] = post_scaled ? q2 : q1;
                    }
                    if (4 * (v0 + 64 * k + 64) > a.len) {
                        const int left = a.len - 4 * idx;
#pragma unroll
                        for (int c = 0; c < 4; c++) { const bool on = c < left; cv[c] = on ? cv[c] : 0.0f; dv[c] = on ? dv[c] : 0.0f; }
                    }
                    t1[k] = make_float4(cv[0], cv[1], cv[2], cv[3]);
                    t0[k] = make_float4(cv[0] * dv[0], cv[1] * dv[1], cv[2] * dv[2], cv[3] * dv[3]);
                    asm volatile("" : "+v"(t1[k].x), "+v"(t1[k].y), "+v"(t1[k].z), "+v"(t1[k].w),
                                      "+v"(t0[k].x), "+v"(t0[k].y), "+v"(t0[k].z), "+v"(t0[k].w));
                    __builtin_amdgcn_sched_barrier(0);
                }
                __syncthreads();
            }
        } else {
#pragma unroll
        for (int k = 0; k < M / 4; k++) {
            const int idx = v0 + 64 * k + lane, uidx = u0 + 64 * k + lane;
            tC[k] = make_float4(0.f, 0.f, 0.f, 0.f); t0[k] = tC[k]; t1[k] = tC[k];
            if (FUSED == FUSE_VIEW) draw[k] = make_short4(0, 0, 0, 0);
            if (FUSED == FUSE_VIEW) {
                typedef float v4f __attribute__((ext_vector_type(4)));
                if (idx < nvec) { const v4f q = __builtin_nontemporal_load(reinterpret_cast<const v4f*>(sC) + idx); tC[k] = make_float4(q.x, q.y, q.z, q.w); }
                if (idx < nfused) {
                    const v4f cq = __builtin_nontemporal_load(reinterpret_cast<const v4f*>(sF) + idx);
                    const unsigned doff = min((unsigned)idx * 8u, dl_last);
                    const v4s_u dq = __builtin_nontemporal_load(reinterpret_cast<const v4s_u*>(sD + doff));
                    t1[k] = make_float4(cq.x, cq.y, cq.z, cq.w);
                    draw[k] = make_short4(dq.x, dq.y, dq.z, dq.w);
                }
            } else {
                typedef float v4f __attribute__((ext_vector_type(4)));
                if (idx < nvec) { const v4f q = __builtin_nontemporal_load(reinterpret_cast<const v4f*>(sC) + idx); tC[k] = make_float4(q.x, q.y, q.z, q.w); }
                if (uidx < nvecU) { const v4f q = __builtin_nontemporal_load(reinterpret_cast<const v4f*>(s0) + ADF_PIDX(uidx)); t0[k] = make_float4(q.x, q.y, q.z, q.w); }
                if (PAIR && uidx + 64 * MQ < nvecU) { const v4f q = __builtin_nontemporal_load(reinterpret_cast<const v4f*>(s0) + ADF_PIDX(uidx + 64 * MQ)); t1[k] = make_float4(q.x, q.y, q.z, q.w); }
            }
        }
        }
        if (FUSED == FUSE_VIEW) {
            const int tl = nfull - v0;
            const int ktail = (rem && tl >= 0 && tl < 16 * M) ? (tl >> 6) : -1;
#pragma unroll
            for (int k = 0; k < M / 4; k++) {
                if (k == ktail && lane == (tl & 63)) {
                    const int sh = 16 * (4 - rem);
                    unsigned long long w = (unsigned long long)(unsigned short)draw[k].x | ((unsigned long long)(unsigned short)draw[k].y << 16) |
                                           ((unsigned long long)(unsigned short)draw[k].z << 32) | ((unsigned long long)(unsigned short)draw[k].w << 48);
                    w >>= sh;
                    draw[k] = make_short4((short)(w & 0xffff), (short)((w >> 16) & 0xffff), (short)((w >> 32) & 0xffff), (short)(w >> 48));
                    if (rem < 2) t1[k].y = 0.0f;
                    if (rem < 3) t1[k].z = 0.0f;
                    t1[k].w = 0.0f;
                }
                t0[k] = make_float4(t1[k].x * (float)draw[k].x, t1[k].y * (float)draw[k].y, t1[k].z * (float)draw[k].z, t1[k].w * (float)draw[k].w);
            }
        }
    }
#define ADF_TRANSPOSE_IN(T, DST, SCALE)                                                   \
    {                                                                                     \
        _Pragma("unroll") for (int k = 0; k < M / 4; k++) stage[64 * k + lane] = T[k];    \
        __syncthreads();                                                                  \
        _Pragma("unroll") for (int k = 0; k < M / 4; k++) {                               \
            const float4 v = stage[lane * (M / 4) + k];                                   \
            DST[4 * k + 0] = v.x * (SCALE); DST[4 * k + 1] = v.y * (SCALE);               \
            DST[4 * k + 2] = v.z * (SCALE); DST[4 * k + 3] = v.w * (SCALE);               \
        }                                                                                 \
        __syncthreads();                                                                  \
    }
#define ADF_PAIR_IN(T, HALF)                                                              \
    {                                                                                     \
        _Pragma("unroll") for (int k = 0; k < MQ; k++) stage[64 * k + lane] = T[k];       \
        __syncthreads();                                                                  \
        if ((lane >> 5) == (HALF)) {                                                      \
            _Pragma("unroll") for (int k = 0; k < MQ; k++) {                              \
                const int j = (lane & 31) * M + 4 * k;                                    \
                const int sidx = ((j >> 4) << 3) + ((j & 15) >> 2);                       \
                const float4 v = stage[sidx], w = stage[sidx + 4];                        \
                f0[4 * k + 0] = v.x; f0[4 * k + 1] = v.y; f0[4 * k + 2] = v.z; f0[4 * k + 3] = v.w; \
                f1[4 * k + 0] = w.x; f1[4 * k + 1] = w.y; f1[4 * k + 2] = w.z; f1[4 * k + 3] = w.w; \
            }                                                                             \
        }                                                                                 \
        __syncthreads();                                                                  \
    }
    ADF_TRANSPOSE_IN(tC, c, a.lambda)
    if (PAIR && FUSED == FUSE_NONE) {
        ADF_PAIR_IN(t0, 0)
        ADF_PAIR_IN(t1, 1)
    } else {
        ADF_TRANSPOSE_IN(t0, f0, 1.0f)
        if (R > 1) ADF_TRANSPOSE_IN(t1, f1, 1.0f)
        else {
#pragma unroll
            for (int i = 0; i < M; i++) f1[i] = 0.0f;
        }
    }
#undef ADF_PAIR_IN
#undef ADF_TRANSPOSE_IN

    float a_s = __shfl_up(c[M - 1], 1);
    if (lane == 0) a_s = 0.0f;
    if constexpr (NW == 2) {
        if (wv == 0 && lane == 63) xch[0] = c[M - 1];
        __syncthreads();
        if (wv == 1 && lane == 0) a_s = xch[0];
    }

    Boundary<float, R> bd;
    chunk_boundary<M, R>(c, f0, f1, a_s, bd);
    float nGS0 = __shfl_down(bd.GS0, 1), nGS1 = (R > 1) ? __shfl_down(bd.GS1, 1) : 0.0f;
    float nPS = __shfl_down(bd.PS, 1), nQS = __shfl_down(bd.QS, 1);
    if (lane == 63) { nGS0 = 0.0f; nGS1 = 0.0f; nPS = 0.0f; nQS = 0.0f; }
    if constexpr (NW == 2) {
        if (wv == 1 && lane == 0) { xch[1] = bd.GS0; xch[2] = (R > 1) ? bd.GS1 : 0.0f; xch[3] = bd.PS; xch[4] = bd.QS; }
        __syncthreads();
        if (wv == 0 && lane == 63) { nGS0 = xch[1]; nGS1 = xch[2]; nPS = xch[3]; nQS = xch[4]; }
    }
    float al, be, ga, p0, p1, xs0, xs1;
    separator_row<M, R>(c, f0, f1, bd, nGS0, nGS1, nPS, nQS, al, be, ga, p0, p1);
    float xL0, xL1;
    if constexpr (NW == 2) {
        const int g = 64 * wv + lane;
        red[0][g] = al; red[1][g] = be; red[2][g] = ga; red[3][g] = p0; red[4][g] = p1;
        __syncthreads();
        if (wv == 0) reduced128<R>(lane, red[0], red[1], red[2], red[3], red[4], 1, xsol[0], xsol[1]);
        __syncthreads();
        xs0 = xsol[0][g]; xs1 = (R > 1) ? xsol[1][g] : 0.0f;
        xL0 = g > 0 ? xsol[0][g - 1] : 0.0f; xL1 = (R > 1 && g > 0) ? xsol[1][g - 1] : 0.0f;
    } else {
        pcr64<R>(lane, al, be, ga, p0, p1, xs0, xs1);
        xL0 = __shfl_up(xs0, 1); xL1 = (R > 1) ? __shfl_up(xs1, 1) : 0.0f;
        if (lane == 0) { xL0 = 0.0f; xL1 = 0.0f; }
    }
    chunk_solve<M, R>(c, f0, f1, a_s, xL0, xL1, xs0, xs1);

    typedef float v4f __attribute__((ext_vector_type(4)));
    int lane_s = lane;
    asm volatile("" : "+v"(lane_s));
    if (!PAIR) {
#pragma unroll
        for (int k = 0; k < MQ; k++)
            stage[lane * MQ + k] = make_float4(f0[4 * k], f0[4 * k + 1], f0[4 * k + 2], f0[4 * k + 3]);
        __syncthreads();
        v4f* d4 = reinterpret_cast<v4f*>(a.U0 + off);
#pragma unroll
        for (int k = 0; k < MQ; k++) {
            const int idx = 64 * k + lane_s;
            if (v0 + idx < nvec) { const float4 q = stage[idx]; const v4f o = {q.x, q.y, q.z, q.w}; __builtin_nontemporal_store(o, d4 + v0 + idx); }
        }
    } else {
        v4f* d4 = reinterpret_cast<v4f*>(a.U0 + offU);
#pragma unroll
        for (int half = 0; half < 2; half++) {
            if ((lane >> 5) == half) {
#pragma unroll
                for (int k = 0; k < MQ; k++) {
                    const int j = (lane & 31) * M + 4 * k;
                    const int sidx = ((j >> 4) << 3) + ((j & 15) >> 2);
                    stage[sidx] = make_float4(f0[4 * k], f0[4 * k + 1], f0[4 * k + 2], f0[4 * k + 3]);
                    stage[sidx + 4] = make_float4(f1[4 * k], f1[4 * k + 1], f1[4 * k + 2], f1[4 * k + 3]);
                }
            }
            __syncthreads();
#pragma unroll
            for (int k = 0; k < MQ; k++) {
                const int idx = 2 * v0 + 64 * (k + half * MQ) + lane_s;
                if (idx < nvecU) { const float4 q = stage[64 * k + lane_s]; const v4f o = {q.x, q.y, q.z, q.w}; __builtin_nontemporal_store(o, d4 + ADF_PIDX(idx)); }
            }
            __syncthreads();
        }
    }
}

template <int M, int NW = 1>
hipError_t launch_h(const WavePassArgs& a, int n_rhs, int n_pairs, hipStream_t st)
{
    dim3 grid(a.nscan, n_pairs), block(64 * NW);
    if (a.fuse.lo_conf) {
        if (n_rhs != 2 || !a.fuse.lo_taps) return hipErrorInvalidValue;
        const int n = ((a.len + 3) / 4) * 4;
        hipLaunchKernelGGL(lo_tap_table_kernel, dim3((n + 255) / 256), dim3(256), 0, st, a.fuse.lo_taps, n, a.len, a.fuse.hi_x0, a.fuse.lo_scale_x, a.fuse.lo_w);
        if (wave_hpass_lo_half(a))
            hipLaunchKernelGGL((wave_hpass_kernel<M, 2, FUSE_LO_HALF, NW>), grid, block, 0, st, a);
        else
            hipLaunchKernelGGL((wave_hpass_kernel<M, 2, FUSE_LO, NW>), grid, block, 0, st, a);
    } else if (a.fuse.conf_in) {
        if (n_rhs != 2) return hipErrorInvalidValue;
        hipLaunchKernelGGL((wave_hpass_kernel<M, 2, FUSE_VIEW, NW>), grid, block, 0, st, a);
    } else if (n_rhs == 2) hipLaunchKernelGGL((wave_hpass_kernel<M, 2, FUSE_NONE, NW>), grid, block, 0, st, a);
    else hipLaunchKernelGGL((wave_hpass_kernel<M, 1, FUSE_NONE, NW>), grid, block, 0, st, a);
    return hipGetLastError();
}

constexpr Bucket ROW_BUCKETS[] = {{4, 64}, {8, 64}, {16, 64}, {20, 64}, {28, 64}, {40, 64}, {56, 64}, {60, 64}, {64, 64},
                                  {40, 128}, {48, 128}, {56, 128}, {60, 128}, {64, 128}};
constexpr int N_ROW_BUCKETS = sizeof(ROW_BUCKETS) / sizeof(ROW_BUCKETS[0]);

void pick_row_bucket(int len, int& m, int& nw)
{
    const Bucket& b = ROW_BUCKETS[bucket_index(ROW_BUCKETS, len)];
    m = b.m; nw = b.chunks / 64;
}

}

int wave_max_row_len() { return ROW_BUCKETS[N_ROW_BUCKETS - 1].m * ROW_BUCKETS[N_ROW_BUCKETS - 1].chunks; }

bool wave_hpass_can_fuse(const WavePassArgs& a)
{
    if (!a.fuse.conf_in || !a.fuse.dl_in) return false;
    if (a.len < 4 || a.fuse.conf_pitch % 4 != 0 || a.fuse.conf_x0 % 4 != 0 || a.fuse.conf_frame % 4 != 0) return false;
    if ((reinterpret_cast<uintptr_t>(a.fuse.conf_in) & 15u) != 0) return false;
    if (a.fuse.dl_stride % 2 != 0 || a.fuse.dl_pair_stride % 2 != 0 || (reinterpret_cast<uintptr_t>(a.fuse.dl_in) & 1u) != 0) return false;
    return true;
}

bool wave_hpass_lo_half(const WavePassArgs& a)
{
    if (!(a.fuse.lo_conf && a.fuse.lo_half && a.fuse.lo_scale_x == 0.5 && (a.fuse.hi_x0 & 1) == 0 && a.fuse.hi_x0 >= 2)) return false;
    int m, nw;
    pick_row_bucket(a.len, m, nw);
    return !(m == 60 && nw == 1);
}

bool wave_hpass_can_fuse_lo(const WavePassArgs& a)
{
    if (!a.fuse.lo_conf || !a.fuse.lo_dl || a.fuse.lo_w < 2 || a.fuse.lo_w > 65535 || a.fuse.lo_h < 1 || a.len < 2 || a.len > wave_max_row_len()) return false;
    if ((reinterpret_cast<uintptr_t>(a.fuse.lo_conf) & 3u) != 0 || (reinterpret_cast<uintptr_t>(a.fuse.lo_dl) & 1u) != 0) return false;
    if (a.fuse.lo_dl_stride % 2 != 0 || a.fuse.lo_dl_pair % 2 != 0) return false;
    if (!(a.fuse.lo_scale_x > 0.0 && a.fuse.lo_scale_y > 0.0) || a.fuse.hi_x0 < 0 || a.fuse.hi_y0 < 0) return false;
    int m, nw;
    pick_row_bucket(a.len, m, nw);
    const int mq = m / 4, kh = (mq + 1) / 2, cap = lo_row_cap(m);
    for (int wv = 0; wv < nw; wv++)
        for (int hh = 0; hh < 2; hh++) {
            const int cfirst = 64 * m * wv + 256 * (hh ? kh : 0);
            const int clast = std::min(64 * m * wv + 256 * (hh ? mq : kh), a.len) - 1;
            if (clast < cfirst) continue;
            int s_first, s_last; float f_;
            lin_tap(a.fuse.hi_x0 + cfirst, a.fuse.lo_scale_x, a.fuse.lo_w, s_first, f_);
            lin_tap(a.fuse.hi_x0 + clast, a.fuse.lo_scale_x, a.fuse.lo_w, s_last, f_);
            if (s_last + 2 - s_first > cap) return false;
        }
    return true;
}

hipError_t launch_wave_hpass(const WavePassArgs& a, int n_rhs, int n_pairs, hipStream_t st)
{
    if (a.len < 2 || a.len > wave_max_row_len() || a.pitch % 64 != 0 || a.pitch < a.len) return hipErrorInvalidValue;
    if (a.fuse.lo_conf && !wave_hpass_can_fuse_lo(a)) return hipErrorInvalidValue;
    if (!a.fuse.lo_conf && a.fuse.conf_in && !wave_hpass_can_fuse(a)) return hipErrorInvalidValue;
    return dispatch_index<N_ROW_BUCKETS>(bucket_index(ROW_BUCKETS, a.len), [&](auto I) {
        constexpr Bucket b = ROW_BUCKETS[decltype(I)::value];
        return launch_h<b.m, b.chunks / 64>(a, n_rhs, n_pairs, st);
    });
}

}
```

### addingdisparityfiltering_amd/csrc/fgs_wave_v.hip

```cpp
#include "fgs_wave_common.h"

namespace adf {

namespace {
using namespace wave;

constexpr int VT = 512;
constexpr int VC = 16;

template <int EPI>
__device__ __forceinline__ unsigned epi_pack16(v2f u0, v2f u1)
{
    v2f x = u0;
    if (EPI == EPI_WLS_CONF) {
        const v2f sc = vsplat(0x1p64f);
        x = u0 * (vrcp_nr(vfma(u1, sc, vsplat(ADF_EPS * 0x1p64f))) * sc);
    }
    const bool o0 = !(__builtin_fabsf(x.x) < 2147483648.0f), o1 = !(__builtin_fabsf(x.y) < 2147483648.0f);
    const int i0 = (int)(o0 ? -32768.0f : __builtin_rintf(x.x)), i1 = (int)(o1 ? -32768.0f : __builtin_rintf(x.y));
    typedef short s2 __attribute__((ext_vector_type(2)));
    return __builtin_bit_cast(unsigned, (s2)__builtin_amdgcn_cvt_pk_i16(i0, i1));
}

template <int M, int R, int EPI, int VCW = VC, int NCH = 64>
// ... 68 lines not shown
            nGS0 = *reinterpret_cast<const v2f*>(&nb[0][cidx + 1][2 * xp]); nGS1 = *reinterpret_cast<const v2f*>(&nb[1][cidx + 1][2 * xp]);
            nPS = *reinterpret_cast<const v2f*>(&nb[2][cidx + 1][2 * xp]); nQS = *reinterpret_cast<const v2f*>(&nb[3][cidx + 1][2 * xp]);
        }
        v2f al, be, ga, p0, p1;
        separator_row<M, R>(c, f0, f1, bd, nGS0, nGS1, nPS, nQS, al, be, ga, p0, p1);
        red[0][2 * xp][cidx] = al.x; red[1][2 * xp][cidx] = be.x; red[2][2 * xp][cidx] = ga.x;
        red[3][2 * xp][cidx] = p0.x; red[4][2 * xp][cidx] = p1.x;
        red[0][2 * xp + 1][cidx] = al.y; red[1][2 * xp + 1][cidx] = be.y; red[2][2 * xp + 1][cidx] = ga.y;
        red[3][2 * xp + 1][cidx] = p0.y; red[4][2 * xp + 1][cidx] = p1.y;
    }
    __syncthreads();
    if constexpr (NCH == 64) {
        const int wv = tid >> 6, lane = tid & 63;
#pragma unroll
        for (int e = 0; e < 2; e++) {
            const int cc = 2 * wv + e;
            float x0, x1;
            pcr64<R>(lane, red[0][cc][lane], red[1][cc][lane], red[2][cc][lane], red[3][cc][lane], red[4][cc][lane], x0, x1);
            xs[0][cc][lane] = x0; xs[1][cc][lane] = x1;
        }
    } else {
        const int cc = tid >> 6, lane = tid & 63;
        reduced128<R>(lane, red[0][cc], red[1][cc], red[2][cc], red[3][cc], red[4][cc], 1, xs[0][cc], xs[1][cc]);
    }
    __syncthreads();
    {
        const int cc = 2 * xp;
        const v2f xR0 = {xs[0][cc][cidx], xs[0][cc + 1][cidx]}, xR1 = {xs[1][cc][cidx], xs[1][cc + 1][cidx]};
        v2f xL0 = vsplat(0.0f), xL1 = xL0;
        if (cidx > 0) {
            xL0 = (v2f){xs[0][cc][cidx - 1], xs[0][cc + 1][cidx - 1]};
            xL1 = (v2f){xs[1][cc][cidx - 1], xs[1][cc + 1][cidx - 1]};
        }
        chunk_solve<M, R>(c, f0, f1, a_s, xL0, xL1, xR0, xR1);
    }

    unsigned voff = voff0;
    asm volatile("" : "+v"(voff));
    if (EPI == EPI_PLANES) {
#pragma unroll
        for (int i = 0; i < M; i++) {
            if (r0 + i < h) {
                *reinterpret_cast<v2f*>(b0 + voff) = f0[i];
                if (R > 1) *reinterpret_cast<v2f*>(b1 + voff) = f1[i];
            }
            voff += ADF_VSTEP(i);
        }
    } else {
        int r0e = r0, cole = col;
        asm volatile("" : "+v"(r0e), "+v"(cole));
        char* ob = reinterpret_cast<char*>(a.out) + (ptrdiff_t)blockIdx.y * a.out_pair_stride +
                   (ptrdiff_t)(a.out_y0 + r0e) * a.out_stride;
        const int esz = (EPI == EPI_F32) ? 4 : (EPI == EPI_U8) ? 1 : 2;
        unsigned ooff = (unsigned)((a.out_x0 + cole) * a.out_cn + a.out_c) * (unsigned)esz;
        const bool fast16 = (EPI == EPI_WLS_CONF || EPI == EPI_I16) && a.out_cn == 1;
        if (fast16 && (a.nscan & 1)) {
            const bool al4 = ((reinterpret_cast<uintptr_t>(a.out) | (uintptr_t)a.out_stride | (uintptr_t)a.out_pair_stride) & 3u) == 0 &&
                             ((a.out_x0 * 2) & 3) == 0;
            const int hv2 = (cole + 1 < a.nscan ? h : 0) - r0e;
            const int hv1 = (cole + 1 == a.nscan ? h : 0) - r0e;
            char* dst = ob + ooff;
#pragma unroll
            for (int i = 0; i < M; i++) {
                const unsigned v = epi_pack16<EPI>(f0[i], f1[i]);
                if (i < hv2) {
                    if (al4) *reinterpret_cast<unsigned*>(dst) = v;
                    else { reinterpret_cast<uint16_t*>(dst)[0] = (uint16_t)v; reinterpret_cast<uint16_t*>(dst)[1] = (uint16_t)(v >> 16); }
                }
                if (i < hv1) reinterpret_cast<uint16_t*>(dst)[0] = (uint16_t)v;
                dst += a.out_stride;
                ADF_STEP_FENCE();
            }
        } else if (fast16) {
            const bool al4 = ((reinterpret_cast<uintptr_t>(a.out) | (uintptr_t)a.out_stride | (uintptr_t)a.out_pair_stride) & 3u) == 0 &&
                             ((a.out_x0 * 2) & 3) == 0;
            const int hv = (cole < a.nscan ? h : 0) - r0e;
            char* dst = ob + ooff;
            if (al4) {
#pragma unroll
                for (int i = 0; i < M; i++) {
                    const unsigned v = epi_pack16<EPI>(f0[i], f1[i]);
                    if (i < hv) *reinterpret_cast<unsigned*>(dst) = v;
                    dst += a.out_stride;
                    ADF_STEP_FENCE();
                }
            } else {
#pragma unroll
                for (int i = 0; i < M; i++) {
                    const unsigned v = epi_pack16<EPI>(f0[i], f1[i]);
                    if (i < hv) {
                        reinterpret_cast<uint16_t*>(dst)[0] = (uint16_t)v;
                        reinterpret_cast<uint16_t*>(dst)[1] = (uint16_t)(v >> 16);
                    }
                    dst += a.out_stride;
                    ADF_STEP_FENCE();
                }
            }
        } else {
#pragma unroll
        for (int i = 0; i < M; i++) {
            if (r0 + i < h) {
#pragma unroll
                for (int e = 0; e < 2; e++) {
                    if (col + e < a.nscan) {
                        char* dst = ob + ooff + (unsigned)(e * a.out_cn * esz);
                        if (EPI == EPI_WLS_CONF) {
                            const float rcp = 1.0f / (f1[i][e] + ADF_EPS);
                            *reinterpret_cast<int16_t*>(dst) = sat16(f0[i][e] * rcp);
                        } else {
#pragma unroll
                            for (int r = 0; r < R; r++) {
                                const float x = r ? f1[i][e] : f0[i][e];
                                char* d = dst + r * esz;
                                if (EPI == EPI_I16) *reinterpret_cast<int16_t*>(d) = sat16(x);
                                else if (EPI == EPI_U8) *reinterpret_cast<uint8_t*>(d) = sat8(x);
                                else *reinterpret_cast<float*>(d) = x;
                            }
                        }
                    }
                }
            }
            ooff += (unsigned)a.out_stride;
        }
        }
    }
}

template <int M, int VCW = VC, int NCH = 64>
hipError_t launch_v(const WavePassArgs& a, int n_rhs, int epi, int n_pairs, hipStream_t st)
{
    dim3 grid(a.pitch / VCW, n_pairs), block(VT);
    constexpr int N_EPI = EPI_U8 + 1;
    if (n_rhs < 1 || n_rhs > 2 || epi < 0 || epi >= N_EPI) return hipErrorInvalidValue;
    return dispatch_index<2 * N_EPI>((n_rhs - 1) * N_EPI + epi, [&](auto K) {
        constexpr int R = decltype(K)::value / N_EPI + 1, EPI = decltype(K)::value % N_EPI;
        if constexpr (R == 1 && EPI == EPI_WLS_CONF) return hipErrorInvalidValue;
        else {
            hipLaunchKernelGGL((wave_vpass_kernel<M, R, EPI, VCW, NCH>), grid, block, 0, st, a);
            return hipGetLastError();
        }
    });
}

constexpr Bucket COL_BUCKETS[] = {{2, 64}, {4, 64}, {8, 64}, {12, 64}, {18, 64}, {26, 64}, {34, 64}, {20, 128}, {26, 128}, {34, 128}};
constexpr int N_COL_BUCKETS = sizeof(COL_BUCKETS) / sizeof(COL_BUCKETS[0]);

}

int wave_max_col_len() { return COL_BUCKETS[N_COL_BUCKETS - 1].m * COL_BUCKETS[N_COL_BUCKETS - 1].chunks; }

hipError_t launch_wave_vpass(const WavePassArgs& a, int n_rhs, int epilogue, int n_pairs, hipStream_t st)
{
    if (a.len < 2 || a.len > wave_max_col_len() || a.pitch % 64 != 0 || a.pitch < a.nscan) return hipErrorInvalidValue;
    return dispatch_index<N_COL_BUCKETS>(bucket_index(COL_BUCKETS, a.len), [&](auto I) {
        constexpr Bucket b = COL_BUCKETS[decltype(I)::value];
        return launch_v<b.m, b.chunks == 64 ? VC : VC / 2, b.chunks>(a, n_rhs, epilogue, n_pairs, st);
    });
}

}
```

### addingdisparityfiltering_amd/csrc/prep_bodies.h

```cpp
#pragma once
#include "adf_internal.h"

namespace adf {
namespace prep {

#define ADF_PREP_ST(p, v) __builtin_nontemporal_store((v), (p))

constexpr int WS_U = 4;
constexpr int WS_NT = 128;
constexpr int WS_COLS = 4;
constexpr int WS_BCOLS = WS_NT * WS_COLS;
constexpr int WS_LUT_HEAD = 2048;

template <int CH>
struct WsShared {
    float lut_head[WS_LUT_HEAD];
};

typedef unsigned ws_v4u __attribute__((ext_vector_type(4)));
typedef unsigned ws_v2u __attribute__((ext_vector_type(2)));
typedef float ws_v4f __attribute__((ext_vector_type(4)));

template <int CH> struct WsWin;
template <> struct WsWin<3> { ws_v4u a; unsigned b; };
template <> struct WsWin<1> { ws_v2u a; };
template <int CH> struct WsPrev { unsigned q[WS_COLS], qa[WS_COLS]; };

struct WsGuide {
    __amdgpu_buffer_rsrc_t rsrc; unsigned mis, stride;
};
__device__ __forceinline__ WsGuide ws_guide(uintptr_t base0, ptrdiff_t stride_bytes, int rows, int row_bytes)
{
    WsGuide gd;
    gd.mis = (unsigned)__builtin_amdgcn_readfirstlane((int)(base0 & 3u));
    const unsigned blo = (unsigned)__builtin_amdgcn_readfirstlane((int)(unsigned)((base0 - gd.mis) & 0xffffffffu));
    const unsigned bhi = (unsigned)__builtin_amdgcn_readfirstlane((int)(unsigned)((base0 - gd.mis) >> 32));
    gd.stride = (unsigned)__builtin_amdgcn_readfirstlane((int)(unsigned)stride_bytes);
    const unsigned records = (unsigned)__builtin_amdgcn_readfirstlane(
        (int)((gd.mis + (unsigned)(rows - 1) * gd.stride + (unsigned)row_bytes + 3u) & ~3u));
    gd.rsrc = __builtin_amdgcn_make_buffer_rsrc(reinterpret_cast<void*>((uintptr_t)blo | ((uintptr_t)bhi << 32)), (short)0, (int)records, 0x00020000);
    return gd;
}

template <int CH>
__device__ __forceinline__ WsWin<CH> ws_load(const WsGuide& gd, unsigned wo)
{
    WsWin<CH> w;
    if constexpr (CH == 3) {
        w.a = __builtin_amdgcn_raw_buffer_load_b128(gd.rsrc, wo, 0, 0);
        w.b = __builtin_amdgcn_raw_buffer_load_b32(gd.rsrc, wo + 16u, 0, 0);
    } else {
        w.a = __builtin_amdgcn_raw_buffer_load_b64(gd.rsrc, wo, 0, 0);
    }
    return w;
}

template <int CH>
__device__ __forceinline__ void ws_indices(const WsWin<CH>& w, unsigned m, WsPrev<CH>& pv, int (&hidx)[WS_COLS], int (&vidx)[WS_COLS])
{
    if constexpr (CH == 3) {
        const unsigned e0 = __builtin_amdgcn_alignbyte(w.a.y, w.a.x, m), e1 = __builtin_amdgcn_alignbyte(w.a.z, w.a.y, m);
        const unsigned e2 = __builtin_amdgcn_alignbyte(w.a.w, w.a.z, m), e3 = __builtin_amdgcn_alignbyte(w.b, w.a.w, m);
        unsigned p[WS_COLS + 1], pa[WS_COLS + 1];
        p[0] = e0 & 0x00ffffffu;
        p[1] = __builtin_amdgcn_perm(e1, e0, 0x0c050403u);
        p[2] = __builtin_amdgcn_perm(e2, e1, 0x0c040302u);
        p[3] = e2 >> 8;
        p[4] = e3 & 0x00ffffffu;
#pragma unroll
        for (int k = 0; k <= WS_COLS; k++) pa[k] = __builtin_amdgcn_udot4(p[k], p[k], 0u, false);
#pragma unroll
        for (int k = 0; k < WS_COLS; k++) {
            hidx[k] = (int)(pa[k] + pa[k + 1]) - 2 * (int)__builtin_amdgcn_udot4(p[k], p[k + 1], 0u, false);
            vidx[k] = (int)(pa[k] + pv.qa[k]) - 2 * (int)__builtin_amdgcn_udot4(p[k], pv.q[k], 0u, false);
            pv.q[k] = p[k]; pv.qa[k] = pa[k];
        }
    } else {
        const unsigned e = __builtin_amdgcn_alignbyte(w.a.y, w.a.x, m);
        const unsigned nb = __builtin_amdgcn_alignbyte(0u, w.a.y, m) & 0xffu;
#pragma unroll
        for (int k = 0; k < WS_COLS; k++) {
            const int v = (int)((e >> (8 * k)) & 0xffu);
            const int r = k < WS_COLS - 1 ? (int)((e >> (8 * k + 8)) & 0xffu) : (int)nb;
            const int u = (int)((pv.q[0] >> (8 * k)) & 0xffu);
            hidx[k] = (v - r) * (v - r);
            vidx[k] = (u - v) * (u - v);
        }
        pv.q[0] = e;
    }
}

__device__ __forceinline__ __amdgpu_buffer_rsrc_t ws_window(const void* p, size_t bytes)
{
    const uintptr_t b = reinterpret_cast<uintptr_t>(p);
    const unsigned lo = (unsigned)__builtin_amdgcn_readfirstlane((int)(unsigned)(b & 0xffffffffu));
    const unsigned hi = (unsigned)__builtin_amdgcn_readfirstlane((int)(unsigned)(b >> 32));
    const unsigned n = (unsigned)__builtin_amdgcn_readfirstlane((int)(unsigned)bytes);
    return __builtin_amdgcn_make_buffer_rsrc(reinterpret_cast<void*>((uintptr_t)lo | ((uintptr_t)hi << 32)), (short)0, (int)n, 0x00020000);
}
constexpr unsigned WS_DROP = 0x80000000u;

struct WsPending { float wl[2 * WS_COLS]; unsigned g[2 * WS_COLS]; };
__device__ __forceinline__ void ws_lookup_issue(const float* lut_head, const __amdgpu_buffer_rsrc_t& lutwin, const int (&hidx)[WS_COLS],
                                                const int (&vidx)[WS_COLS], WsPending& p)
{
#pragma unroll
    for (int k = 0; k < WS_COLS; k++) {
        p.wl[k] = lut_head[min(hidx[k], WS_LUT_HEAD - 1)];
        p.wl[WS_COLS + k] = lut_head[min(vidx[k], WS_LUT_HEAD - 1)];
    }
#pragma unroll
    for (int k = 0; k < WS_COLS; k++) {
        p.g[k] = __builtin_amdgcn_raw_buffer_load_b32(lutwin, hidx[k] >= WS_LUT_HEAD ? (unsigned)hidx[k] * 4u : WS_DROP, 0, 0);
        p.g[WS_COLS + k] = __builtin_amdgcn_raw_buffer_load_b32(lutwin, vidx[k] >= WS_LUT_HEAD ? (unsigned)vidx[k] * 4u : WS_DROP, 0, 0);
    }
}
__device__ __forceinline__ void ws_lookup_finish(const WsPending& p, float (&wh)[WS_COLS], float (&wv)[WS_COLS])
{
#pragma unroll
    for (int k = 0; k < WS_COLS; k++) {
        wh[k] = p.g[k] != 0u ? __uint_as_float(p.g[k]) : p.wl[k];
        wv[k] = p.g[WS_COLS + k] != 0u ? __uint_as_float(p.g[WS_COLS + k]) : p.wl[WS_COLS + k];
    }
}

struct WsOut {
    __amdgpu_buffer_rsrc_t chor, cvert; unsigned mh[WS_COLS], mv[WS_COLS]; unsigned ho, vo, hstep, vstep; bool st_ok, strip;
    __device__ __forceinline__ void init(const WeightArgs& a, size_t pz, int j0, int y_first)
    {
        const Geom& g = a.g;
        chor = ws_window(a.chor + pz * g.plane, g.plane * sizeof(float));
        cvert = ws_window(a.cvert + pz * g.plane, g.plane * sizeof(float));
        strip = a.cvert_orient == ORIENT_STRIP;
#pragma unroll
        for (int k = 0; k < WS_COLS; k++) { mh[k] = (j0 + k < g.rw - 1) ? 0xffffffffu : 0u; mv[k] = (j0 + k < g.rw) ? 0xffffffffu : 0u; }
        st_ok = j0 >= 0 && j0 < g.pw;
        ho = ((unsigned)y_first * (unsigned)g.pw + (unsigned)j0) * 4u;
        vo = (strip ? ((unsigned)(j0 >> 4) * (unsigned)g.rh + (unsigned)y_first) * ADF_STRIP + (unsigned)(j0 & 15)
                    : (unsigned)y_first * (unsigned)g.pw + (unsigned)j0) * 4u;
        hstep = (unsigned)g.pw * 4u; vstep = (strip ? (unsigned)ADF_STRIP : (unsigned)g.pw) * 4u;
    }
    __device__ __forceinline__ void store_h(int t, const float (&wh)[WS_COLS], bool on) const
    {
        ws_v4u o;
#pragma unroll
        for (int k = 0; k < WS_COLS; k++) o[k] = __float_as_uint(wh[k]) & mh[k];
        __builtin_amdgcn_raw_buffer_store_b128(o, chor, (on && st_ok) ? ho + (unsigned)t * hstep : WS_DROP, 0, 2 );
    }
    __device__ __forceinline__ void store_v(int t, const float (&wv)[WS_COLS], bool last_row, bool on) const
    {
        const unsigned last = last_row ? 0u : 0xffffffffu;
        ws_v4u o;
#pragma unroll
        for (int k = 0; k < WS_COLS; k++) o[k] = __float_as_uint(wv[k]) & mv[k] & last;
        const unsigned off = (on && st_ok) ? vo + (unsigned)t * vstep : WS_DROP;
        if (strip) __builtin_amdgcn_raw_buffer_store_b128(o, cvert, off, 0, 0);
        else __builtin_amdgcn_raw_buffer_store_b128(o, cvert, off, 0, 2);
    }
};

template <int CH>
__device__ __forceinline__ void weights_stream_body(const WeightArgs& a, int bx, int by, int nby, size_t pz, WsShared<CH>& sh, bool active)
{
    static_assert(CH == 1 || CH == 3, "guides have one or three channels");
    float (&lut_head)[WS_LUT_HEAD] = sh.lut_head;
    const Geom& g = a.g;
    const int tid = active ? (int)threadIdx.x : 0;
    if (active)
        for (int q = tid; q < WS_LUT_HEAD; q += WS_NT) lut_head[q] = a.lut[q];
    __syncthreads();
    const int ws_rows = (g.rh + nby - 1) / nby;
    const int x0 = bx * WS_BCOLS, y0 = by * ws_rows;
    if (!active || y0 >= g.rh) return;
    constexpr int WS_PRIO = 3;
    __builtin_amdgcn_s_setprio(WS_PRIO);
    const int nrows = min(ws_rows, g.rh - y0) + 1;
    const int j0 = x0 + WS_COLS * tid;

    const int r_first = g.ry + y0, r_last = g.ry + min(y0 + nrows - 1, g.rh - 1);
    const WsGuide gd = ws_guide(reinterpret_cast<uintptr_t>(a.guide) + (uintptr_t)((ptrdiff_t)pz * a.pair_stride + (ptrdiff_t)r_first * a.stride),
                                a.stride, r_last - r_first + 1, g.W * CH);
    const unsigned col_off = gd.mis + (unsigned)((g.rx + x0) * CH);
    const unsigned lane_off = (unsigned)(tid * WS_COLS * CH);
    auto row_off = [&](int n) -> unsigned { return col_off + (unsigned)(min(y0 + n, g.rh - 1) - y0) * gd.stride; };
    auto load = [&](int n) -> WsWin<CH> { return ws_load<CH>(gd, (row_off(n) & ~3u) + lane_off); };

    WsOut out;
    out.init(a, pz, j0, y0);
    const __amdgpu_buffer_rsrc_t lutwin = ws_window(a.lut, sizeof(float) * ADF_LUT_LEVELS);
    WsPrev<CH> pv;
#pragma unroll
    for (int k = 0; k < WS_COLS; k++) { pv.q[k] = 0; pv.qa[k] = 0; }
    WsWin<CH> nxt[WS_U], cur[WS_U];
#pragma unroll
    for (int s = 0; s < WS_U; s++) nxt[s] = load(s < nrows ? s : nrows - 1);
    WsPending pend;
    {
        int hidx[WS_COLS], vidx[WS_COLS];
        ws_indices<CH>(nxt[0], row_off(0) & 3u, pv, hidx, vidx);
        ws_lookup_issue(lut_head, lutwin, hidx, vidx, pend);
    }
    for (int n0 = 0; n0 < nrows; n0 += WS_U) {
#pragma unroll
        for (int s = 0; s < WS_U; s++) {
            cur[s] = nxt[s];
            if constexpr (CH == 3) asm volatile("" : "+v"(cur[s].a), "+v"(cur[s].b)); else asm volatile("" : "+v"(cur[s].a));
        }
#pragma unroll
        for (int s = 0; s < WS_U; s++) nxt[s] = load(min(n0 + WS_U + s, nrows - 1));
#pragma unroll
        for (int s = 0; s < WS_U; s++) {
            const int n = n0 + s;
            WsPending ahead;
            {
                int hidx[WS_COLS], vidx[WS_COLS];
                ws_indices<CH>(s + 1 < WS_U ? cur[s + 1 < WS_U ? s + 1 : 0] : nxt[0], row_off(min(n + 1, nrows - 1)) & 3u, pv, hidx, vidx);
                ws_lookup_issue(lut_head, lutwin, hidx, vidx, ahead);
            }
            float wh[WS_COLS], wv[WS_COLS];
            ws_lookup_finish(pend, wh, wv);
            out.store_h(n, wh, n < nrows - 1);
            out.store_v(n - 1, wv, y0 + n - 1 == g.rh - 1, n >= 1 && n < nrows);
            pend = ahead;
        }
    }
}


}
}
```

### addingdisparityfiltering_amd/csrc/weights_kernels.hip

```cpp
#include "adf_internal.h"
#include "prep_bodies.h"
#include <cstdlib>

namespace adf {

namespace {

#define ADF_ST(p, v) __builtin_nontemporal_store((v), (p))
constexpr int TX = 64, TY = 32, NT = 256;
constexpr int LUT_HEAD = 2048;

template <int CH>
__global__ void __launch_bounds__(NT) weights_kernel(WeightArgs a)
{
    constexpr int RB = (TX + 1) * CH;
    constexpr int RW = (RB + 3) / 4 + 1;
    __shared__ unsigned gw[(TY + 1) * RW];
    __shared__ int mis[TY + 1];
    __shared__ float th[TX * (TY + 1)];
    __shared__ float lut_head[LUT_HEAD];
    const Geom& g = a.g;
    const int tid = threadIdx.x, tx = tid % TX, ty = tid / TX;
    const int x0 = blockIdx.x * TX, y0 = blockIdx.y * TY;
    const size_t pz = blockIdx.z;
    const unsigned char* gp = a.guide + (ptrdiff_t)pz * a.pair_stride;
    const int last_px = min(x0 + TX, g.rw - 1);
    const int need = (last_px - x0 + 1) * CH;

    for (int rr = ty; rr < TY + 1; rr += NT / TX) {
        const int gi = min(y0 + rr, g.rh - 1);
        const unsigned char* rowp = gp + (ptrdiff_t)(g.ry + gi) * a.stride + (ptrdiff_t)(g.rx + x0) * CH;
        const int m = (int)(reinterpret_cast<uintptr_t>(rowp) & 3u);
        const unsigned* wp = reinterpret_cast<const unsigned*>(rowp - m);
        const int nw = (m + need + 3) >> 2;
        for (int w = tx; w < nw; w += TX) gw[rr * RW + w] = wp[w];
        if (tx == 0) mis[rr] = m;
    }
    for (int q = tid; q < LUT_HEAD; q += NT) lut_head[q] = a.lut[q];
    __syncthreads();

    const unsigned char* gb = reinterpret_cast<const unsigned char*>(gw);
    float* chor = a.chor + pz * g.plane;
    float* cvert = a.cvert + pz * g.plane;
    int hidx[TY / 4], vidx[TY / 4];
#pragma unroll
    for (int kk = 0; kk < TY / 4; kk++) {
        const int r = ty + 4 * kk;
        const unsigned char* p = gb + r * (RW * 4) + mis[r] + tx * CH;
        const unsigned char* pd = gb + (r + 1) * (RW * 4) + mis[r + 1] + tx * CH;
        int hi = 0, vi = 0;
#pragma unroll
        for (int c = 0; c < CH; c++) {
            const int v = p[c];
            const int dh = v - (int)p[CH + c];
            const int dv = v - (int)pd[c];
            hi += dh * dh; vi += dv * dv;
        }
        hidx[kk] = hi; vidx[kk] = vi;
    }
    float wh[TY / 4], wv[TY / 4];
    bool big = false;
#pragma unroll
    for (int kk = 0; kk < TY / 4; kk++) {
        wh[kk] = lut_head[min(hidx[kk], LUT_HEAD - 1)];
        wv[kk] = lut_head[min(vidx[kk], LUT_HEAD - 1)];
        big = big || hidx[kk] >= LUT_HEAD || vidx[kk] >= LUT_HEAD;
    }
    if (big) {
#pragma unroll
        for (int kk = 0; kk < TY / 4; kk++) {
            if (hidx[kk] >= LUT_HEAD) wh[kk] = a.lut[hidx[kk]];
            if (vidx[kk] >= LUT_HEAD) wv[kk] = a.lut[vidx[kk]];
        }
    }
    const int j = x0 + tx;
#pragma unroll
    for (int kk = 0; kk < TY / 4; kk++) {
        const int r = ty + 4 * kk;
        const int i = y0 + r;
        const bool ok = i < g.rh && j < g.rw;
        const float h = (j == g.rw - 1) ? 0.0f : wh[kk];
        const float v = (i == g.rh - 1) ? 0.0f : wv[kk];
        if (a.chor_orient == ORIENT_N) { if (ok) chor[(size_t)i * g.pw + j] = h; }
        else th[tx * (TY + 1) + r] = ok ? h : 0.0f;
        if (ok) cvert[a.cvert_orient == ORIENT_STRIP ? strip_index(i, j, g.rh) : (size_t)i * g.pw + j] = v;
    }
    if (a.chor_orient == ORIENT_T) {
        __syncthreads();
#pragma unroll
        for (int m = 0; m < TX / 8; m++) {
            const int cidx = tid / TY + 8 * m, ridx = tid % TY;
            const int jj = x0 + cidx, ii = y0 + ridx;
            if (jj < g.rw && ii < g.rh) chor[(size_t)jj * g.ph + ii] = th[cidx * (TY + 1) + ridx];
        }
    }
}

template <int CH>
__global__ void __launch_bounds__(prep::WS_NT) weights_stream_kernel(WeightArgs a)
{
    __shared__ prep::WsShared<CH> sh;
    prep::weights_stream_body<CH>(a, blockIdx.x, blockIdx.y, gridDim.y, blockIdx.z, sh, true);
}

__global__ void __launch_bounds__(256) transpose_n_to_t_kernel(const float* __restrict__ src, float* __restrict__ dst, Geom g)
{
    __shared__ float tile[64][65];
    const int tid = threadIdx.x;
    const int j0 = blockIdx.x * 64, i0 = blockIdx.y * 64;
    const size_t pb = (size_t)blockIdx.z * g.plane;
    const int c4 = tid & 15, r = tid >> 4;
#pragma unroll
    for (int m = 0; m < 4; m++) {
        const int row = r + 16 * m;
        float4 v = make_float4(0.f, 0.f, 0.f, 0.f);
        if (i0 + row < g.rh) v = *reinterpret_cast<const float4*>(src + pb + (size_t)(i0 + row) * g.pw + j0 + 4 * c4);
        tile[row][4 * c4 + 0] = v.x; tile[row][4 * c4 + 1] = v.y; tile[row][4 * c4 + 2] = v.z; tile[row][4 * c4 + 3] = v.w;
    }
    __syncthreads();
#pragma unroll
    for (int m = 0; m < 4; m++) {
        const int col = r + 16 * m;
        if (j0 + col < g.rw) {
            const float4 v = make_float4(tile[4 * c4 + 0][col], tile[4 * c4 + 1][col], tile[4 * c4 + 2][col], tile[4 * c4 + 3][col]);
            *reinterpret_cast<float4*>(dst + pb + (size_t)(j0 + col) * g.ph + i0 + 4 * c4) = v;
        }
    }
}

}

hipError_t launch_weights(const WeightArgs& a, int n_pairs, hipStream_t st)
{
    if (a.chor_orient == ORIENT_T && a.cvert_orient == ORIENT_N && a.scratch) {
        WeightArgs b = a;
        b.chor = a.scratch; b.chor_orient = ORIENT_N; b.scratch = nullptr;
        hipError_t e = launch_weights(b, n_pairs, st);
        if (e != hipSuccess) return e;
        dim3 grid(a.g.pw / 64, a.g.ph / 64, n_pairs);
        hipLaunchKernelGGL(transpose_n_to_t_kernel, grid, dim3(256), 0, st, a.scratch, a.chor, a.g);
        return hipGetLastError();
    }
    if (a.cvert_orient != ORIENT_N && !(a.cvert_orient == ORIENT_STRIP && a.chor_orient == ORIENT_N)) return hipErrorInvalidValue;
    static const bool force_generic = [] { const char* e = getenv("ADF_WEIGHTS_GENERIC"); return e && atoi(e) != 0; }();
    if (!force_generic && a.chor_orient == ORIENT_N && a.stride > 0 && a.stride < ((ptrdiff_t)1 << 29) && (size_t)a.g.W * a.ch < ((size_t)1 << 29)) {
        dim3 sgrid((a.g.rw + prep::WS_BCOLS - 1) / prep::WS_BCOLS, 1, n_pairs);
        {
            int rpb = 128;
            while (rpb > 16 && ((a.g.rh + rpb - 1) / rpb) * (int)(sgrid.x * sgrid.z) < 2048) rpb >>= 1;
            while (rpb > 4 && ((a.g.rh + rpb - 1) / rpb) * (int)(sgrid.x * sgrid.z) < 512) rpb >>= 1;
            while (rpb > 1 && (size_t)(rpb + 1) * (size_t)a.stride >= ((size_t)1 << 30)) rpb >>= 1;
            sgrid.y = (a.g.rh + rpb - 1) / rpb;
        }
        if (a.ch == 1) hipLaunchKernelGGL(weights_stream_kernel<1>, sgrid, dim3(prep::WS_NT), 0, st, a);
        else if (a.ch == 3) hipLaunchKernelGGL(weights_stream_kernel<3>, sgrid, dim3(prep::WS_NT), 0, st, a);
        else return hipErrorInvalidValue;
        return hipGetLastError();
    }
    dim3 grid((a.g.rw + TX - 1) / TX, (a.g.rh + TY - 1) / TY, n_pairs);
    if (a.ch == 1) hipLaunchKernelGGL(weights_kernel<1>, grid, dim3(NT), 0, st, a);
    else if (a.ch == 3) hipLaunchKernelGGL(weights_kernel<3>, grid, dim3(NT), 0, st, a);
    else return hipErrorInvalidValue;
    return hipGetLastError();
}

}
```

### addingdisparityfiltering_amd/ximgproc.py

```python
import ctypes as C
import math

import numpy as np

from . import _lib
from ._lib import AdfError, PATH_CONF_BAND, PATH_FUSED_FIRST_PASS, PATH_MERGED_PREP, PATH_SCALED_FUSED, PATH_SCALED_HALF, Rect, SOLVER_EXACT, SOLVER_WAVE

try:
    import torch
except Exception:
    torch = None


def _is_torch(a):
    return torch is not None and isinstance(a, torch.Tensor)


def _as_rect(roi):
    if roi is None:
        return None
    if isinstance(roi, Rect):
        return roi
    x, y, w, h = roi
    return Rect(int(x), int(y), int(w), int(h))


_ITEMSIZE = {np.int16: 2, np.uint8: 1, np.float32: 4}
_TORCH_DTYPE = {np.int16: torch.int16, np.uint8: torch.uint8, np.float32: torch.float32} if torch is not None else {}
_raw_stream = getattr(getattr(torch, "_C", None), "_cuda_getCurrentRawStream", None) if torch is not None else None


class _Image:

    def __init__(self, arr, dtype_np, what, batched, allow_channels=(1,)):
        self.keep = arr
        if _is_torch(arr):
            if not arr.is_cuda:
                arr = arr.cpu().numpy()
            else:
                if arr.dtype != _TORCH_DTYPE[dtype_np]:
                    raise AdfError(_lib.ADF_EBADARG, "%s must have dtype %s" % (what, _TORCH_DTYPE[dtype_np]))
                self.device = True
                isz = _ITEMSIZE[dtype_np]
                self.ptr = arr.data_ptr()
                self._finish(arr.shape, [q * isz for q in arr.stride()], isz, what, batched, allow_channels)
                return
        a = np.asarray(arr)
        if a.dtype != np.dtype(dtype_np):
            raise AdfError(_lib.ADF_EBADARG, "%s must have dtype %s (got %s)" % (what, np.dtype(dtype_np), a.dtype))
        self.device = False
        self.keep = a
        self.ptr = a.ctypes.data
        self._finish(a.shape, a.strides, a.itemsize, what, batched, allow_channels)

    def _finish(self, shape, strides, itemsize, what, batched, allow_channels):
        nd = len(shape)
        k = 1 if batched else 0
        if nd - k == 2:
            self.c, sc, sx = 1, itemsize, strides[k + 1]
        elif nd - k == 3:
            self.c, sc, sx = shape[k + 2], strides[k + 2], strides[k + 1]
        else:
            raise AdfError(_lib.ADF_EBADARG, "%s has an unsupported shape %s" % (what, tuple(shape)))
        self.n, self.pair_stride = (shape[0], strides[0]) if batched else (1, 0)
        self.h, self.w, self.stride = shape[k], shape[k + 1], strides[k]
        if self.n < 1 or self.h < 1 or self.w < 1:
            raise AdfError(_lib.ADF_EBADARG, "%s is empty" % what)
        if self.c not in allow_channels:
            raise AdfError(_lib.ADF_EBADARG, "%s must have %s channel(s)" % (what, " or ".join(map(str, allow_channels))))
        if sc != itemsize or sx != itemsize * self.c:
            raise AdfError(_lib.ADF_ESIZE, "%s rows must be dense (channel-interleaved, unit pixel stride)" % what)


def _empty(img, shape, dtype_np):
    if img.device:
        return torch.empty(shape, dtype=_TORCH_DTYPE[dtype_np], device=img.keep.device)
    return np.empty(shape, dtype_np)


def _out_like(img, batched, dtype_np):
    return _empty(img, (img.n, img.h, img.w) if batched else (img.h, img.w), dtype_np)


def _stream_of(img):
    if img.device:
        dev = img.keep.device
        if _raw_stream is not None and dev.index is not None:
            return _raw_stream(dev.index)
        return torch.cuda.current_stream(dev).cuda_stream
    return None


def _read(fn, ctype, *args):
    v = ctype()
    _lib.check(fn(*args, C.byref(v)))
    return v.value


_entries = {}


def _call(name, img, args):
    pair = _entries.get(name)
    if pair is None:
        pair = _entries[name] = (getattr(_lib.lib(), name + "_host"), getattr(_lib.lib(), name + "_device"))
    if img.device:
        _lib.check(pair[1](*args, _stream_of(img)))
    else:
        _lib.check(pair[0](*args))


class _Handle:
    _h, _destroy = None, None

    def __del__(self):
        h, self._h = self._h, None
        if h:
            try:
                getattr(_lib.lib(), self._destroy)(h)
            except Exception:
                pass


def _check_device(dev, imgs, what):
    for im in imgs:
        if im is not None and im.device and im.keep.device.index != dev:
            raise AdfError(_lib.ADF_EBADARG, "%s lives on cuda:%d; tensors on cuda:%s cannot be passed to it "
                                             "(create one handle per GPU)" % (what, dev, im.keep.device.index))


class DisparityFilter:

    def filter(self, disparity_map_left, left_view, filtered_disparity_map=None,
               disparity_map_right=None, ROI=None, right_view=None):
        raise NotImplementedError


class DisparityWLSFilter(_Handle, DisparityFilter):
    _destroy = "adf_wls_destroy"

    def __init__(self, use_confidence, left_offset=0, right_offset=0, top_offset=0, bottom_offset=0,
                 min_disp=0):
        self._h = C.c_void_p()
        _lib.check(_lib.lib().adf_wls_create(C.byref(self._h), int(bool(use_confidence)), left_offset,
                                             right_offset, top_offset, bottom_offset, min_disp))
        self._use_confidence = bool(use_confidence)
        self._last = None
        self._dev = _read(_lib.lib().adf_wls_get_device, C.c_int, self._h)

    def getLambda(self):
        return _read(_lib.lib().adf_wls_get_lambda, C.c_double, self._h)

    def setLambda(self, _lambda):
        _lib.check(_lib.lib().adf_wls_set_lambda(self._h, float(_lambda)))

    def getSigmaColor(self):
        return _read(_lib.lib().adf_wls_get_sigma_color, C.c_double, self._h)

    def setSigmaColor(self, _sigma_color):
        _lib.check(_lib.lib().adf_wls_set_sigma_color(self._h, float(_sigma_color)))

    def getLRCthresh(self):
        return _read(_lib.lib().adf_wls_get_lrc_thresh, C.c_int, self._h)

    def setLRCthresh(self, _LRC_thresh):
        _lib.check(_lib.lib().adf_wls_set_lrc_thresh(self._h, int(_LRC_thresh)))

    def getDepthDiscontinuityRadius(self):
        return _read(_lib.lib().adf_wls_get_depth_discontinuity_radius, C.c_int, self._h)

    def setDepthDiscontinuityRadius(self, _disc_radius):
        _lib.check(_lib.lib().adf_wls_set_depth_discontinuity_radius(self._h, int(_disc_radius)))

    def setFGSParams(self, lambda_attenuation=0.25, num_iter=3):
        _lib.check(_lib.lib().adf_wls_set_fgs_params(self._h, float(lambda_attenuation), int(num_iter)))

    def setSolver(self, solver):
        _lib.check(_lib.lib().adf_wls_set_solver(self._h, int(solver)))

    def getSolver(self):
        return _read(_lib.lib().adf_wls_get_solver, C.c_int, self._h)

    def getLastSolver(self):
        return _read(_lib.lib().adf_wls_get_last_solver, C.c_int, self._h)

    def getLastPath(self):
        return _read(_lib.lib().adf_wls_get_last_path, C.c_int, self._h)

    def enableProfiling(self, on=True):
        _lib.check(_lib.lib().adf_wls_profile_enable(self._h, int(bool(on))))

    def readProfile(self):
        buf = (_lib.KernelTime * 16)()
        n = C.c_int()
        _lib.check(_lib.lib().adf_wls_profile_read(self._h, buf, 16, C.byref(n)))
        return {buf[k].name.decode(): dict(launches=buf[k].launches, total_ms=buf[k].total_ms,
                                           alg_bytes=buf[k].alg_bytes, moved_bytes=buf[k].moved_bytes)
                for k in range(n.value)}

    def workspaceBytes(self):
        return int(_lib.lib().adf_wls_workspace_bytes(self._h))

    def filter(self, disparity_map_left, left_view, filtered_disparity_map=None,
               disparity_map_right=None, ROI=None, right_view=None):
        if disparity_map_left is None:
            raise AdfError(_lib.ADF_EBADARG, "disparity_map_left is empty")
        if left_view is None:
            raise AdfError(_lib.ADF_EBADARG, "left_view is empty")
        batched = len(disparity_map_left.shape) == 3
        dl = _Image(disparity_map_left, np.int16, "disparity_map_left", batched)
        gv = _Image(left_view, np.uint8, "left_view", batched, allow_channels=(1, 3))
        if gv.n != dl.n:
            raise AdfError(_lib.ADF_ESIZE, "batch sizes of disparity maps and views differ")
        dr = None
        if disparity_map_right is not None and getattr(disparity_map_right, "size", 1) != 0:
            dr = _Image(disparity_map_right, np.int16, "disparity_map_right", batched)
            if (dr.n, dr.h, dr.w) != (dl.n, dl.h, dl.w):
                raise AdfError(_lib.ADF_ESIZE, "left and right disparity maps differ in size")
        elif self._use_confidence:
            raise AdfError(_lib.ADF_EBADARG, "disparity_map_right is required with use_confidence")
        if gv.device != dl.device or (dr is not None and dr.device != dl.device):
            raise AdfError(_lib.ADF_EBADARG, "inputs must all be numpy arrays or all be CUDA tensors")
        if filtered_disparity_map is None:
            filtered_disparity_map = _out_like(gv, batched, np.int16)
        out = _Image(filtered_disparity_map, np.int16, "filtered_disparity_map", batched)
        if (out.n, out.h, out.w) != (gv.n, gv.h, gv.w) or out.device != dl.device:
            raise AdfError(_lib.ADF_ESIZE, "filtered_disparity_map has the wrong size or placement")
        if dl.device:
            _check_device(self._dev, (dl, gv, dr, out), "this DisparityWLSFilter")
        roi = _as_rect(ROI)
        args = (self._h, dl.n,
                dl.ptr, dl.stride, dl.pair_stride, dl.w, dl.h,
                gv.ptr, gv.stride, gv.pair_stride, gv.c, gv.w, gv.h,
                out.ptr, out.stride, out.pair_stride,
                dr.ptr if dr else None, dr.stride if dr else 0, dr.pair_stride if dr else 0,
                C.byref(roi) if roi is not None else None)
        if dl.device:
            _lib.check(_lib.lib().adf_wls_filter_scaled_device(*args, _stream_of(dl)))
        else:
            _lib.check(_lib.lib().adf_wls_filter_scaled_host(*args))
        self._last = (batched, dl.device, gv)
        return filtered_disparity_map

    def getConfidenceMap(self, pair=None):
        if self._last is None or not self._use_confidence:
            return np.zeros((0, 0), np.float32)
        batched, device, ex = self._last
        pairs = range(ex.n) if pair is None else [pair]
        outs = []
        for k in pairs:
            o = _empty(ex, (ex.h, ex.w), np.float32)
            _call("adf_wls_get_confidence", ex, (self._h, k, o.data_ptr() if device else o.ctypes.data, ex.w * 4))
            outs.append(o)
        if pair is not None or not batched:
            return outs[0]
        return torch.stack(outs) if device else np.stack(outs)

    def getROI(self):
        r = Rect()
        _lib.check(_lib.lib().adf_wls_get_roi(self._h, C.byref(r)))
        return (r.x, r.y, r.width, r.height)

    def sync(self, stream=None):
        _lib.check(_lib.lib().adf_wls_sync(self._h, stream))


def _accessors(*names):
    def pair(name):
        return (lambda self: getattr(self, name)), (lambda self, v: setattr(self, name, v))

    def add(cls):
        for name in names:
            for prefix, fn in zip(("get", "set"), pair(name)):
                fn.__name__ = prefix + name[0].upper() + name[1:]
                setattr(cls, fn.__name__, fn)
        return cls
    return add


@_accessors("minDisparity", "numDisparities", "blockSize", "disp12MaxDiff", "speckleWindowSize", "uniquenessRatio")
class StereoMatcher(_Handle):
    _channels = (1,)

    def __init__(self, minDisparity=0, numDisparities=16, blockSize=3):
        self.minDisparity, self.numDisparities, self.blockSize = minDisparity, numDisparities, blockSize
        self.disp12MaxDiff, self.speckleWindowSize, self.uniquenessRatio = -1, 0, 10

    def _views(self, left, right, device_only=None):
        nd = len(left.shape)
        color = 3 in self._channels and nd in (3, 4) and left.shape[-1] == 3
        batched = nd == (4 if color else 3)
        L = _Image(left, np.uint8, "left", batched, self._channels)
        R = _Image(right, np.uint8, "right", batched, self._channels)
        if device_only and not (L.device and R.device):
            raise AdfError(_lib.ADF_EBADARG, device_only)
        if (L.n, L.h, L.w, L.c) != (R.n, R.h, R.w, R.c):
            raise AdfError(_lib.ADF_ESIZE, "All the images must have the same size")
        return L, R, batched

    @staticmethod
    def _outputs(maps, names, L, batched, mismatch):
        maps = [_out_like(L, batched, np.int16) if m is None else m for m in maps]
        descs = [_Image(m, np.int16, what, batched) for m, what in zip(maps, names)]
        for D in descs:
            if (D.n, D.h, D.w) != (L.n, L.h, L.w) or D.device != L.device:
                raise AdfError(_lib.ADF_ESIZE, mismatch)
        return maps, descs

    def compute(self, left, right, disparity=None):
        self._refuse()
        if self.speckleWindowSize > 0:
            raise AdfError(_lib.ADF_EBADARG, "speckle filtering is not implemented inside compute(); "
                                             "use filterSpeckles on the result")
        L, R, batched = self._views(left, right)
        if L.device != R.device:
            raise AdfError(_lib.ADF_EBADARG, "left and right must live on the same side (host or device)")
        (disparity,), (D,) = self._outputs((disparity,), ("disparity",), L, batched, "disparity must match the views")
        self._prepare((L, R, D))
        _call(self._entry, L, self._args(L, R, D))
        return disparity


@_accessors("textureThreshold", "preFilterCap")
class StereoBM(StereoMatcher):
    _destroy, _entry = "adf_bm_destroy", "adf_bm_compute"

    def __init__(self, numDisparities=0, blockSize=21):
        super().__init__(0, numDisparities if numDisparities > 0 else 64, blockSize)
        self.textureThreshold, self.uniquenessRatio, self.preFilterCap = 10, 15, 31

    @staticmethod
    def create(numDisparities=0, blockSize=21):
        return StereoBM(numDisparities, blockSize)

    def _left_right_check_on(self):
        return 0 <= self.disp12MaxDiff < 1000000

# ... 386 lines not shown
```

### include/adf_wls.h

```cpp
#ifndef ADF_WLS_H
#define ADF_WLS_H

#include <stddef.h>
#include <stdint.h>

#ifdef __cplusplus
extern "C" {
#endif

#define ADF_VERSION 100

enum adf_status {
    ADF_OK = 0,
    ADF_EBADARG = 1,
    ADF_ESIZE = 2,
    ADF_EHIP = 3,
    ADF_ENOMEM = 4,
    ADF_ENODEV = 5
};

enum adf_solver { ADF_SOLVER_EXACT = 0, ADF_SOLVER_WAVE = 1 };

enum adf_depth { ADF_8U = 0, ADF_16S = 3, ADF_32F = 5 };

typedef struct adf_wls adf_wls_t;
typedef struct adf_fgs adf_fgs_t;

typedef struct adf_rect { int x, y, width, height; } adf_rect;

int adf_version(void);
const char* adf_last_error(void);
int adf_device_count(void);
int adf_device_pci_bus_id(int device, char* buf, int len);


int adf_wls_create(adf_wls_t** out, int use_confidence, int left_offset, int right_offset,
                   int top_offset, int bottom_offset, int min_disp);
void adf_wls_destroy(adf_wls_t* h);

int adf_wls_set_lambda(adf_wls_t* h, double lambda);
int adf_wls_get_lambda(const adf_wls_t* h, double* lambda);
int adf_wls_set_sigma_color(adf_wls_t* h, double sigma_color);
int adf_wls_get_sigma_color(const adf_wls_t* h, double* sigma_color);
int adf_wls_set_lrc_thresh(adf_wls_t* h, int lrc_thresh);
int adf_wls_get_lrc_thresh(const adf_wls_t* h, int* lrc_thresh);
int adf_wls_set_depth_discontinuity_radius(adf_wls_t* h, int radius);
int adf_wls_get_depth_discontinuity_radius(const adf_wls_t* h, int* radius);

int adf_wls_set_fgs_params(adf_wls_t* h, double lambda_attenuation, int num_iter);
int adf_wls_set_solver(adf_wls_t* h, int solver);
int adf_wls_get_solver(const adf_wls_t* h, int* solver);
int adf_wls_get_last_solver(const adf_wls_t* h, int* solver);
#define ADF_PATH_CONF_BAND 1
#define ADF_PATH_FUSED_FIRST_PASS 2
#define ADF_PATH_MERGED_PREP 4
#define ADF_PATH_SCALED_FUSED 8
#define ADF_PATH_SCALED_HALF 16
int adf_wls_get_last_path(const adf_wls_t* h, int* path_flags);

int adf_wls_filter_device(adf_wls_t* h, int n_pairs,
                          const int16_t* disp_left, ptrdiff_t disp_left_stride, ptrdiff_t disp_left_pair_stride,
                          const uint8_t* left_view, ptrdiff_t view_stride, ptrdiff_t view_pair_stride,
                          int view_channels, int W, int H,
                          int16_t* out, ptrdiff_t out_stride, ptrdiff_t out_pair_stride,
                          const int16_t* disp_right, ptrdiff_t disp_right_stride, ptrdiff_t disp_right_pair_stride,
                          const adf_rect* roi, void* stream);

int adf_wls_filter_host(adf_wls_t* h, int n_pairs,
                        const int16_t* disp_left, ptrdiff_t disp_left_stride, ptrdiff_t disp_left_pair_stride,
                        const uint8_t* left_view, ptrdiff_t view_stride, ptrdiff_t view_pair_stride,
                        int view_channels, int W, int H,
                        int16_t* out, ptrdiff_t out_stride, ptrdiff_t out_pair_stride,
                        const int16_t* disp_right, ptrdiff_t disp_right_stride, ptrdiff_t disp_right_pair_stride,
                        const adf_rect* roi);

int adf_wls_filter_scaled_device(adf_wls_t* h, int n_pairs,
                                 const int16_t* disp_left, ptrdiff_t disp_left_stride, ptrdiff_t disp_left_pair_stride,
                                 int disp_W, int disp_H,
                                 const uint8_t* left_view, ptrdiff_t view_stride, ptrdiff_t view_pair_stride,
                                 int view_channels, int W, int H,
                                 int16_t* out, ptrdiff_t out_stride, ptrdiff_t out_pair_stride,
                                 const int16_t* disp_right, ptrdiff_t disp_right_stride, ptrdiff_t disp_right_pair_stride,
                                 const adf_rect* roi, void* stream);
int adf_wls_filter_scaled_host(adf_wls_t* h, int n_pairs,
                               const int16_t* disp_left, ptrdiff_t disp_left_stride, ptrdiff_t disp_left_pair_stride,
                               int disp_W, int disp_H,
                               const uint8_t* left_view, ptrdiff_t view_stride, ptrdiff_t view_pair_stride,
                               int view_channels, int W, int H,
                               int16_t* out, ptrdiff_t out_stride, ptrdiff_t out_pair_stride,
                               const int16_t* disp_right, ptrdiff_t disp_right_stride, ptrdiff_t disp_right_pair_stride,
                               const adf_rect* roi);

int adf_wls_get_confidence_device(adf_wls_t* h, int pair, float* dst, ptrdiff_t dst_stride, void* stream);
int adf_wls_get_confidence_host(adf_wls_t* h, int pair, float* dst, ptrdiff_t dst_stride);
int adf_wls_get_device(const adf_wls_t* h, int* device);
int adf_wls_get_roi(const adf_wls_t* h, adf_rect* roi);
int adf_wls_sync(adf_wls_t* h, void* stream);
size_t adf_wls_workspace_bytes(const adf_wls_t* h);

typedef struct adf_kernel_time {
    char name[48];
    int launches;
    double total_ms;
    double alg_bytes;
    double moved_bytes;
} adf_kernel_time;
int adf_wls_profile_enable(adf_wls_t* h, int on);
int adf_wls_profile_read(adf_wls_t* h, adf_kernel_time* out, int capacity, int* count);


int adf_fgs_create(adf_fgs_t** out, const uint8_t* guide, ptrdiff_t guide_stride, int guide_channels,
                   int w, int h, double lambda, double sigma_color, double lambda_attenuation,
                   int num_iter, int solver);
int adf_fgs_create_device(adf_fgs_t** out, const uint8_t* guide, ptrdiff_t guide_stride, int guide_channels,
                          int w, int h, double lambda, double sigma_color, double lambda_attenuation,
                          int num_iter, int solver, void* stream);
void adf_fgs_destroy(adf_fgs_t* h);
void adf_release_cached_memory(void);
#define ADF_WEIGHT_TABLE_LEVELS (3 * 256 * 256)
int adf_weight_table_host(float sigma_color, float* table, int levels);
int adf_fgs_get_device(const adf_fgs_t* h, int* device);
int adf_fgs_get_solver(const adf_fgs_t* h, int* solver);

int adf_fgs_filter_host(adf_fgs_t* h, const void* src, ptrdiff_t src_stride, void* dst,
                        ptrdiff_t dst_stride, int depth, int channels);
int adf_fgs_filter_device(adf_fgs_t* h, const void* src, ptrdiff_t src_stride, void* dst,
                          ptrdiff_t dst_stride, int depth, int channels, void* stream);


#define ADF_UNKNOWN_DISPARITY 16320

int adf_compute_mse_host(const int16_t* gt, ptrdiff_t gt_stride, const int16_t* src, ptrdiff_t src_stride,
                         int W, int H, const adf_rect* roi, double* mse);
int adf_compute_mse_device(const int16_t* gt, ptrdiff_t gt_stride, const int16_t* src, ptrdiff_t src_stride,
                           int W, int H, const adf_rect* roi, double* mse, void* stream);
int adf_compute_bad_pixel_percent_host(const int16_t* gt, ptrdiff_t gt_stride, const int16_t* src, ptrdiff_t src_stride,
                                       int W, int H, const adf_rect* roi, int thresh, double* percent);
int adf_compute_bad_pixel_percent_device(const int16_t* gt, ptrdiff_t gt_stride, const int16_t* src, ptrdiff_t src_stride,
                                         int W, int H, const adf_rect* roi, int thresh, double* percent, void* stream);
int adf_get_disparity_vis_host(const int16_t* src, ptrdiff_t src_stride, uint8_t* dst, ptrdiff_t dst_stride,
                               int W, int H, double scale);
int adf_get_disparity_vis_device(const int16_t* src, ptrdiff_t src_stride, uint8_t* dst, ptrdiff_t dst_stride,
                                 int W, int H, double scale, void* stream);

typedef struct adf_bm adf_bm_t;
int adf_bm_create(adf_bm_t** out, int num_disparities, int block_size);
void adf_bm_destroy(adf_bm_t* h);
int adf_bm_set_params(adf_bm_t* h, int min_disparity, int num_disparities, int block_size,
                      int prefilter_cap, int texture_threshold, int uniqueness_ratio);
int adf_bm_get_device(const adf_bm_t* h, int* device);
int adf_bm_get_params(const adf_bm_t* h, int* min_disparity, int* num_disparities, int* block_size,
                      int* prefilter_cap, int* texture_threshold, int* uniqueness_ratio);
int adf_bm_compute_device(adf_bm_t* h, int n_pairs,
                          const uint8_t* left, ptrdiff_t left_stride, ptrdiff_t left_pair_stride,
                          const uint8_t* right, ptrdiff_t right_stride, ptrdiff_t right_pair_stride,
                          int W, int H,
                          int16_t* disparity, ptrdiff_t disp_stride, ptrdiff_t disp_pair_stride,
                          void* stream);
int adf_bm_compute_both_device(adf_bm_t* h, int n_pairs,
                               const uint8_t* left, ptrdiff_t left_stride, ptrdiff_t left_pair_stride,
                               const uint8_t* right, ptrdiff_t right_stride, ptrdiff_t right_pair_stride,
                               int W, int H,
                               int16_t* disp_left, ptrdiff_t disp_left_stride, ptrdiff_t disp_left_pair_stride,
                               int16_t* disp_right, ptrdiff_t disp_right_stride, ptrdiff_t disp_right_pair_stride,
                               void* stream);
int adf_bm_compute_host(adf_bm_t* h, int n_pairs,
                        const uint8_t* left, ptrdiff_t left_stride, ptrdiff_t left_pair_stride,
                        const uint8_t* right, ptrdiff_t right_stride, ptrdiff_t right_pair_stride,
                        int W, int H,
                        int16_t* disparity, ptrdiff_t disp_stride, ptrdiff_t disp_pair_stride);

#define ADF_SGBM_MODE_SGBM 0
#define ADF_SGBM_MODE_HH 1
#define ADF_SGBM_MODE_3WAY 2
typedef struct adf_sgbm adf_sgbm_t;
int adf_sgbm_create(adf_sgbm_t** out, int min_disparity, int num_disparities, int block_size);
void adf_sgbm_destroy(adf_sgbm_t* h);
int adf_sgbm_get_device(const adf_sgbm_t* h, int* device);
int adf_sgbm_set_params(adf_sgbm_t* h, int min_disparity, int num_disparities, int block_size, int P1, int P2,
                        int prefilter_cap, int uniqueness_ratio, int mode);
int adf_sgbm_set_disp12_max_diff(adf_sgbm_t* h, int disp12_max_diff);
int adf_sgbm_get_disp12_max_diff(const adf_sgbm_t* h, int* disp12_max_diff);
int adf_sgbm_get_params(const adf_sgbm_t* h, int* min_disparity, int* num_disparities, int* block_size, int* P1, int* P2,
                        int* prefilter_cap, int* uniqueness_ratio, int* mode);
int adf_sgbm_compute_device(adf_sgbm_t* h, int n_pairs,
                            const uint8_t* left, ptrdiff_t left_stride, ptrdiff_t left_pair_stride,
                            const uint8_t* right, ptrdiff_t right_stride, ptrdiff_t right_pair_stride,
                            int channels, int W, int H,
                            int16_t* disparity, ptrdiff_t disp_stride, ptrdiff_t disp_pair_stride,
                            void* stream);
int adf_sgbm_compute_host(adf_sgbm_t* h, int n_pairs,
                          const uint8_t* left, ptrdiff_t left_stride, ptrdiff_t left_pair_stride,
                          const uint8_t* right, ptrdiff_t right_stride, ptrdiff_t right_pair_stride,
                          int channels, int W, int H,
                          int16_t* disparity, ptrdiff_t disp_stride, ptrdiff_t disp_pair_stride);

size_t adf_filter_speckles_workspace_bytes(int n_maps, int W, int H);
int adf_filter_speckles_device(int n_maps, int16_t* img, ptrdiff_t stride, ptrdiff_t map_stride, int W, int H,
                               int new_val, int max_speckle_size, int max_diff,
                               void* workspace, size_t workspace_bytes, void* stream);
int adf_filter_speckles_host(int n_maps, int16_t* img, ptrdiff_t stride, ptrdiff_t map_stride, int W, int H,
                             int new_val, int max_speckle_size, int max_diff);

int adf_half_size(int n, int* half);
int adf_prepare_views_device(int n_images, const uint8_t* src, ptrdiff_t src_stride, ptrdiff_t src_image_stride,
                             int W, int H, int src_channels,
                             uint8_t* dst, ptrdiff_t dst_stride, ptrdiff_t dst_image_stride,
                             int dst_W, int dst_H, int dst_channels, void* stream);
int adf_prepare_views_host(int n_images, const uint8_t* src, ptrdiff_t src_stride, ptrdiff_t src_image_stride,
                           int W, int H, int src_channels,
                           uint8_t* dst, ptrdiff_t dst_stride, ptrdiff_t dst_image_stride,
// ... 7 lines not shown
```

Measured before the change: 40960.

## Store horizontal WLS weights as 16-bit LUT indices and look them up in the wave pass

Adds a weight format option where the weights kernel writes the horizontal edge weights as uint16 indices into the sigma LUT instead of f32 values. The horizontal wave pass then resolves each index through the LUT. This halves the CH plane's storage and its write and read traffic. The index path is used under AUTO only when the LUT tail is constant beyond index 65535 and the merged small-prep path would not otherwise be chosen, and it adds a gather per weight inside the scan kernel.

```diff
diff --git a/addingdisparityfiltering_amd/__init__.py b/addingdisparityfiltering_amd/__init__.py
--- a/addingdisparityfiltering_amd/__init__.py
+++ b/addingdisparityfiltering_amd/__init__.py
@@ -12,6 +12,9 @@
     PATH_SCALED_HALF,
     SOLVER_EXACT,
     SOLVER_WAVE,
+    WEIGHT_AUTO,
+    WEIGHT_FLOAT,
+    WEIGHT_INDEX,
     StereoBM,
     StereoMatcher,
     StereoSGBM,
diff --git a/addingdisparityfiltering_amd/_lib.py b/addingdisparityfiltering_amd/_lib.py
--- a/addingdisparityfiltering_amd/_lib.py
+++ b/addingdisparityfiltering_amd/_lib.py
@@ -7,6 +7,7 @@
 ADF_OK, ADF_EBADARG, ADF_ESIZE, ADF_EHIP, ADF_ENOMEM, ADF_ENODEV = range(6)
 SOLVER_EXACT, SOLVER_WAVE = 0, 1
 PATH_CONF_BAND, PATH_FUSED_FIRST_PASS, PATH_MERGED_PREP, PATH_SCALED_FUSED, PATH_SCALED_HALF = 1, 2, 4, 8, 16
+WEIGHT_AUTO, WEIGHT_FLOAT, WEIGHT_INDEX = 0, 1, 2
 DEPTH_8U, DEPTH_16S, DEPTH_32F = 0, 3, 5
 
 
@@ -51,6 +52,9 @@
     ("adf_wls_get_solver", _i, [_vp, C.POINTER(_i)]),
     ("adf_wls_get_last_solver", _i, [_vp, C.POINTER(_i)]),
     ("adf_wls_get_last_path", _i, [_vp, C.POINTER(_i)]),
+    ("adf_wls_set_weight_format", _i, [_vp, _i]),
+    ("adf_wls_get_weight_format", _i, [_vp, C.POINTER(_i)]),
+    ("adf_wls_get_last_weight_format", _i, [_vp, C.POINTER(_i)]),
     ("adf_wls_filter_device", _i, _FILTER_DEV),
     ("adf_wls_filter_host", _i, _FILTER_DEV[:-1]),
     ("adf_wls_filter_scaled_device", _i, _FILTER_SCALED_DEV),
diff --git a/addingdisparityfiltering_amd/csrc/adf_api.hip b/addingdisparityfiltering_amd/csrc/adf_api.hip
--- a/addingdisparityfiltering_amd/csrc/adf_api.hip
+++ b/addingdisparityfiltering_amd/csrc/adf_api.hip
@@ -83,7 +83,7 @@
 
 static int run_passes(bool wave, const Geom& g, const SolvePlanes& p, int n_rhs, float lambda, float atten, int num_iter,
                       const FinalOut& fo, int n_pairs, hipStream_t st, Profiler* prof = nullptr,
-                      const FusedInputs* fuse = nullptr)
+                      const FusedInputs* fuse = nullptr, const float* index_lut = nullptr)
 {
     const double px = (double)g.rw * g.rh * n_pairs;
     float lam = lambda;
@@ -94,6 +94,7 @@
         const double hb = fused ? (4.0 + lo_b + 8.0) * px : (4.0 + 8.0 * n_rhs) * px;
         const double out_b = (last ? epilogue_bytes(fo.epilogue) : 4.0 * n_rhs) * px;
         const double vb = (4.0 + 4.0 * n_rhs) * px + out_b;
+        const double idx_saved = index_lut ? 2.0 * px : 0.0;
         if (wave) {
             WavePassArgs h{}, v{};
             h.C = p.CH; h.U0 = p.A0; h.U1 = p.A1;
@@ -102,8 +103,9 @@
             v.C = p.CV; v.U0 = p.A0; v.U1 = p.A1;
             v.nscan = g.rw; v.len = g.rh; v.pitch = g.pw; v.plane = g.plane; v.lambda = lam;
             if (last) set_final_out(v, fo);
+            if (index_lut) { h.c_fmt = WFMT_U16; h.lut = index_lut; }
             {
-                ProfScope ps(prof, fused ? K_PASS_H_FIRST : K_PASS_H, hb, hb, st);
+                ProfScope ps(prof, fused ? K_PASS_H_FIRST : K_PASS_H, hb, hb - idx_saved, st);
                 HIP_TRY(launch_wave_hpass(h, n_rhs, n_pairs, st));
             }
             ProfScope ps(prof, last ? K_PASS_V_LAST : K_PASS_V, vb, vb, st);
@@ -148,12 +150,14 @@
     float roll_off = 0.001f;
     double atten = 0.25; int num_iter = 3;
     int solver = ADF_SOLVER_WAVE;
+    int weight_format = ADF_WEIGHT_AUTO;
     int last_solver = ADF_SOLVER_WAVE;
     adf_rect roi{0, 0, 0, 0};
     int last_W = 0, last_H = 0, last_pairs = 0;
     int last_cpitch = 0, last_cx0 = 0;
     long long conf_sig[4] = {0, 0, 0, 0};
     int last_path = 0;
+    int last_weight_format = ADF_WEIGHT_FLOAT;
     Lut lut;
     DevBuf ws;
     DevBuf conf;
@@ -251,6 +255,15 @@
     return ADF_OK;
 }
 extern "C" int adf_wls_get_solver(const adf_wls_t* h, int* v) { NEED_HANDLE(h); if (v) *v = h->solver; return ADF_OK; }
+extern "C" int adf_wls_set_weight_format(adf_wls_t* h, int format)
+{
+    NEED_HANDLE(h);
+    if (format != ADF_WEIGHT_AUTO && format != ADF_WEIGHT_FLOAT && format != ADF_WEIGHT_INDEX) return fail(ADF_EBADARG, "unknown weight format %d", format);
+    h->weight_format = format;
+    return ADF_OK;
+}
+extern "C" int adf_wls_get_weight_format(const adf_wls_t* h, int* v) { NEED_HANDLE(h); if (v) *v = h->weight_format; return ADF_OK; }
+extern "C" int adf_wls_get_last_weight_format(const adf_wls_t* h, int* v) { NEED_HANDLE(h); if (v) *v = h->last_weight_format; return ADF_OK; }
 extern "C" int adf_wls_get_last_solver(const adf_wls_t* h, int* v) { NEED_HANDLE(h); if (v) *v = h->last_solver; return ADF_OK; }
 extern "C" int adf_wls_get_last_path(const adf_wls_t* h, int* v) { NEED_HANDLE(h); if (v) *v = h->last_path; return ADF_OK; }
 
@@ -281,10 +294,10 @@
     return ADF_OK;
 }
 
-static size_t wls_pair_ws_bytes(const Geom& g, bool conf, bool wave, bool disc_maps)
+static size_t wls_pair_ws_bytes(const Geom& g, bool conf, bool wave, bool disc_maps, bool windex)
 {
     size_t planes = wave ? (conf ? 4 : 3) : (conf ? 9 : 6);
-    return planes * g.plane * sizeof(float) + (conf && disc_maps ? 2 * g.frame * sizeof(float) : 0);
+    return (planes * g.plane - (windex ? g.plane / 2 : 0)) * sizeof(float) + (conf && disc_maps ? 2 * g.frame * sizeof(float) : 0);
 }
 
 static int resolve_roi(const adf_wls* h, const adf_rect* roi_in, int w, int hgt, adf_rect& roi)
@@ -428,6 +441,7 @@
     bool wave;
     bool fused_first;
     bool band;
+    bool windex;
     size_t per_pair; int chunk;
     ChunkPlan full, tail;
     int path;
@@ -454,16 +468,28 @@
                      wave_hpass_can_fuse(first_pass_probe(view_fuse(planes, dispL, sL, psL, g), g.rw)));
     p.band = stage == CONF_LEFT && p.fused_first && h->conf_band && conf_band_fits(g, h->disc_radius);
     if (p.band) stage = CONF_BAND;
-    p.per_pair = wls_pair_ws_bytes(g, conf, p.wave, !p.band);
-    p.chunk = (int)(h->ws_limit / p.per_pair);
-    if (p.chunk < 1) p.chunk = 1;
-    if (p.chunk > n_pairs) p.chunk = n_pairs;
-    auto chunk_of = [&](int n) {
-        const bool merged = p.band && h->merge_small && prep_small_fits(g, h->disc_radius, gch, n) && prep_small_guide_fits(g, sG, gch);
-        return plan_chunk(h, merged ? CONF_MERGED : stage, p.wave);
+    struct Layout { size_t per_pair; int chunk; ChunkPlan full, tail; bool merged; };
+    auto lay_out = [&](bool windex) {
+        Layout l{};
+        l.per_pair = wls_pair_ws_bytes(g, conf, p.wave, !p.band, windex);
+        l.chunk = (int)(h->ws_limit / l.per_pair);
+        if (l.chunk < 1) l.chunk = 1;
+        if (l.chunk > n_pairs) l.chunk = n_pairs;
+        auto chunk_of = [&](int n) {
+            const bool merged = !windex && p.band && h->merge_small && prep_small_fits(g, h->disc_radius, gch, n) &&
+                                prep_small_guide_fits(g, sG, gch);
+            return plan_chunk(h, merged ? CONF_MERGED : stage, p.wave);
+        };
+        l.full = chunk_of(l.chunk);
+        l.tail = chunk_of(n_pairs % l.chunk ? n_pairs % l.chunk : l.chunk);
+        l.merged = l.full.stage == CONF_MERGED || l.tail.stage == CONF_MERGED;
+        return l;
     };
-    p.full = chunk_of(p.chunk);
-    p.tail = chunk_of(n_pairs % p.chunk ? n_pairs % p.chunk : p.chunk);
+    const Layout fl = lay_out(false);
+    p.windex = p.wave && h->weight_format != ADF_WEIGHT_FLOAT && h->lut.index_ok && stage != CONF_SCALED_LO &&
+               weights_index_fits(sG, g.W, gch) && !(fl.merged && h->weight_format != ADF_WEIGHT_INDEX);
+    const Layout l = p.windex ? lay_out(true) : fl;
+    p.per_pair = l.per_pair; p.chunk = l.chunk; p.full = l.full; p.tail = l.tail;
     p.path = ((p.band || (scaled && scaled->lo.band_map)) ? ADF_PATH_CONF_BAND : 0) |
              (p.fused_first ? ADF_PATH_FUSED_FIRST_PASS : 0) |
              ((p.full.stage == CONF_MERGED || p.tail.stage == CONF_MERGED) ? ADF_PATH_MERGED_PREP : 0);
@@ -502,13 +528,15 @@
     h->last_cpitch = g.cpitch; h->last_cx0 = g.cx0; h->last_path = 0;
 
     if ((rc = h->lut.ensure((float)h->sigma_color, st))) return rc;
+    if (h->weight_format == ADF_WEIGHT_INDEX && !h->lut.index_ok)
+        return fail(ADF_EBADARG, "ADF_WEIGHT_INDEX: the weight table of sigma_color %g cannot be addressed by 16-bit indices", h->sigma_color);
     const WlsPlan plan = plan_wls(h, g, n_pairs, dispL, sL, psL, sG, gch, scaled);
     const bool wave = plan.wave;
     h->last_solver = wave ? ADF_SOLVER_WAVE : ADF_SOLVER_EXACT;
     if ((rc = h->ws.reserve(plan.per_pair * (size_t)plan.chunk, st, FILL_ZERO))) return rc;
     if (conf && !scaled && (rc = ensure_conf_planes(h, g, n_pairs, st))) return rc;
     {
-        const long long sig[8] = {W, H, roi.x, roi.y, roi.width, roi.height, (long long)plan.band * 4 + (long long)wave * 2 + conf, plan.chunk};
+        const long long sig[8] = {W, H, roi.x, roi.y, roi.width, roi.height, (long long)plan.windex * 8 + (long long)plan.band * 4 + (long long)wave * 2 + conf, plan.chunk};
         if (memcmp(sig, h->ws_sig, sizeof(sig)) != 0) {
             HIP_TRY(hipMemsetAsync(h->ws.p, 0, h->ws.bytes, st));
             memcpy(h->ws_sig, sig, sizeof(sig));
@@ -517,7 +545,8 @@
     float* base = (float*)h->ws.p;
     auto take = [&](size_t elems) { float* p = base; base += elems * (size_t)plan.chunk; return p; };
     SolvePlanes p{};
-    p.CH = take(g.plane); p.CV = take(g.plane); p.A0 = take(g.plane);
+    p.CH = take(plan.windex ? g.plane / 2 : g.plane);
+    p.CV = take(g.plane); p.A0 = take(g.plane);
     if (!wave) { p.D = take(g.plane); p.F0 = take(g.plane); p.B0 = take(g.plane); }
     float *cL = nullptr, *cR = nullptr;
     if (conf) {
@@ -533,6 +562,7 @@
     const int thresh = (int)(1.0f * h->lrc_thresh);
     Profiler* prof = &h->prof;
     h->last_path = plan.path;
+    h->last_weight_format = plan.windex ? ADF_WEIGHT_INDEX : ADF_WEIGHT_FLOAT;
 
     for (int first = 0; first < n_pairs; first += plan.chunk) {
         const int n = (n_pairs - first < plan.chunk) ? n_pairs - first : plan.chunk;
@@ -547,7 +577,8 @@
         const double ob = (oa.conf ? 6.0 : 2.0) * (F - P);
         auto fill_outside = [&](hipStream_t s) { ProfScope ps(prof, K_FILL, ob, ob, s); return launch_outside(oa, n, s); };
         WeightArgs wa{gv, sG, psG, gch, h->lut.cur, p.CH, p.CV, orient_h, orient_cv, g,
-                      wave ? nullptr : p.B0};
+                      wave ? nullptr : p.B0,
+                      plan.windex ? WFMT_U16 : WFMT_F32};
         ConfBandArgs ba{dL, sL, psL, dR, sR, psR, confp, g, rrx, thresh, h->disc_radius, h->roll_off, 0};
         DiscArgs da{{dL, dR}, {sL, sR}, {psL, psR}, {roi.x, rrx}, roi.y, roi.width, roi.height, h->disc_radius, h->roll_off,
                     {cL, cR}, W, g.frame, cp.stage == CONF_LEFT ? 1 : -1};
@@ -563,7 +594,7 @@
         if (cp.stage == CONF_NONE || cp.outside_on_side) HIP_TRY(fill_outside(wst));
         if (cp.stage == CONF_NONE && scaled && first == 0 && (rc = scaled_resize(h, *scaled, st, prof))) return rc;
         if (cp.stage != CONF_MERGED) {
-            ProfScope ps(prof, K_WEIGHTS, (gch + 8.0) * P, (gch + 8.0) * P, wst);
+            ProfScope ps(prof, K_WEIGHTS, (gch + 8.0) * P, (gch + (plan.windex ? 6.0 : 8.0)) * P, wst);
             HIP_TRY(launch_weights(wa, n, wst));
         }
         if (cp.fork_weights) HIP_TRY(hipEventRecord(h->ev_join, h->side));
@@ -635,7 +666,7 @@
         if (cp.fork_weights) HIP_TRY(hipStreamWaitEvent(st, h->ev_join, 0));
         FinalOut fo{conf ? EPI_WLS_CONF : EPI_I16, o, sO, psO, roi.x, roi.y, 1, 0};
         rc = run_passes(wave, g, p, conf ? 2 : 1, (float)h->lambda, (float)h->atten, h->num_iter, fo, n, st, prof,
-                        plan.fused_first ? &fuse : nullptr);
+                        plan.fused_first ? &fuse : nullptr, plan.windex ? h->lut.cur : nullptr);
         if (rc) return rc;
     }
     return ADF_OK;
diff --git a/addingdisparityfiltering_amd/csrc/adf_host.h b/addingdisparityfiltering_amd/csrc/adf_host.h
--- a/addingdisparityfiltering_amd/csrc/adf_host.h
+++ b/addingdisparityfiltering_amd/csrc/adf_host.h
@@ -57,10 +57,11 @@
     struct Entry { std::shared_ptr<LutTable> t; unsigned long long used; };
     std::vector<Entry> tables;
     const float* cur = nullptr;
+    bool index_ok = false;
     unsigned long long tick = 0;
     size_t bytes() const { return tables.size() * sizeof(float) * ADF_LUT_LEVELS; }
     int ensure(float s, hipStream_t st);
-    void release() { tables.clear(); cur = nullptr; }
+    void release() { tables.clear(); cur = nullptr; index_ok = false; }
 };
 
 int copy_images(void* dst, size_t dst_pitch, ptrdiff_t dst_image_stride, const void* src, size_t src_pitch,
diff --git a/addingdisparityfiltering_amd/csrc/adf_host.hip b/addingdisparityfiltering_amd/csrc/adf_host.hip
--- a/addingdisparityfiltering_amd/csrc/adf_host.hip
+++ b/addingdisparityfiltering_amd/csrc/adf_host.hip
@@ -3,6 +3,7 @@
 #include <cmath>
 #include <cstdarg>
 #include <cstdio>
+#include <cstring>
 #include <mutex>
 #include <thread>
 
@@ -56,6 +57,7 @@
 
 struct adf::LutTable {
     int device = 0; float sigma = 0; float* dev = nullptr;
+    bool index_ok = false;
     LutTable() = default;
     LutTable(const LutTable&) = delete;
     LutTable& operator=(const LutTable&) = delete;
@@ -121,7 +123,7 @@
 int adf::Lut::ensure(float s, hipStream_t st)
 {
     for (auto& e : tables)
-        if (e.t->sigma == s) { e.used = ++tick; cur = e.t->dev; return ADF_OK; }
+        if (e.t->sigma == s) { e.used = ++tick; cur = e.t->dev; index_ok = e.t->index_ok; return ADF_OK; }
     if ((int)tables.size() >= LUT_CACHE) {
         size_t lru = 0;
         for (size_t k = 1; k < tables.size(); k++) if (tables[k].used < tables[lru].used) lru = k;
@@ -140,10 +142,16 @@
         if (e != hipSuccess) { hipFree(d); return fail(ADF_EHIP, "LUT upload failed: %s", hipGetErrorString(e)); }
         t = std::make_shared<LutTable>();
         t->device = device; t->sigma = s; t->dev = d;
+        t->index_ok = true;
+        {
+            uint32_t tail, v;
+            memcpy(&tail, &host[WIDX_MAX], sizeof(tail));
+            for (size_t i = WIDX_MAX + 1; i < host.size() && t->index_ok; i++) { memcpy(&v, &host[i], sizeof(v)); t->index_ok = v == tail; }
+        }
         LutStore::get().add(t);
     }
     tables.push_back(Entry{t, ++tick});
-    cur = t->dev;
+    cur = t->dev; index_ok = t->index_ok;
     return ADF_OK;
 }
 
diff --git a/addingdisparityfiltering_amd/csrc/adf_internal.h b/addingdisparityfiltering_amd/csrc/adf_internal.h
--- a/addingdisparityfiltering_amd/csrc/adf_internal.h
+++ b/addingdisparityfiltering_amd/csrc/adf_internal.h
@@ -91,12 +91,16 @@
     int zero_outside = 0, vx0 = 0, vy0 = 0, vx1 = 0, vy1 = 0;
 };
 
+enum WeightFmt { WFMT_F32 = 0, WFMT_U16 = 1 };
+constexpr int WIDX_MAX = 65535;
+
 struct WeightArgs {
     const uint8_t* guide; ptrdiff_t stride, pair_stride; int ch;
     const float* lut;
     float* chor; float* cvert; int chor_orient, cvert_orient;
     Geom g;
     float* scratch;
+    int fmt;
 };
 
 struct PassArgs {
@@ -130,8 +134,10 @@
     int nscan, len, pitch;
     size_t plane;
     float lambda;
+    int c_fmt;
+    const float* lut;
 };
-static_assert(sizeof(WavePassArgs) == 280 && offsetof(WavePassArgs, out) == 208 && offsetof(WavePassArgs, nscan) == 248 &&
+static_assert(sizeof(WavePassArgs) == 288 && offsetof(WavePassArgs, out) == 208 && offsetof(WavePassArgs, nscan) == 248 &&
               offsetof(WavePassArgs, plane) == 264 && offsetof(WavePassArgs, lambda) == 272, "WavePassArgs layout");
 
 hipError_t launch_discontinuity(const DiscArgs& a, int n_pairs, hipStream_t st);
@@ -146,6 +152,7 @@
 int conf_left_max_radius();
 hipError_t launch_plain_prologue(const PlainPrologueArgs& a, int n_pairs, hipStream_t st);
 hipError_t launch_weights(const WeightArgs& a, int n_pairs, hipStream_t st);
+bool weights_index_fits(ptrdiff_t guide_stride, int W, int channels);
 hipError_t launch_resize_linear(const ResizeArgs& a, int n_pairs, hipStream_t st);
 hipError_t launch_exact_pass(const PassArgs& a, int n_rhs, int epilogue, int n_pairs, hipStream_t st);
 hipError_t launch_wave_hpass(const WavePassArgs& a, int n_rhs, int n_pairs, hipStream_t st);
diff --git a/addingdisparityfiltering_amd/csrc/fgs_wave_h.hip b/addingdisparityfiltering_amd/csrc/fgs_wave_h.hip
--- a/addingdisparityfiltering_amd/csrc/fgs_wave_h.hip
+++ b/addingdisparityfiltering_amd/csrc/fgs_wave_h.hip
@@ -10,6 +10,7 @@
 constexpr int H_TWO_WAVE_MAX = 60;
 
 constexpr int FUSE_NONE = 0, FUSE_VIEW = 1, FUSE_LO = 2, FUSE_LO_HALF = 3;
+constexpr unsigned H_DROP = 0x80000000u;
 
 __host__ __device__ __forceinline__ void lin_tap(int d, double scale, int sn, int& s0, float& fx)
 {
@@ -30,12 +31,15 @@
 __host__ __device__ constexpr int lo_row_cap(int m) { return (((m * 64) / 3) & ~7) < 168 ? 168 : (((m * 64) / 3) & ~7); }
 __host__ __device__ constexpr int lo_stage_vec4(int m) { return 12 * lo_row_cap(m) > 256 * m ? (12 * lo_row_cap(m) + 15) / 16 : m * 16; }
 
-template <int M, int R, int FUSED, int NW = 1>
+template <int M, int R, int FUSED, int NW = 1, bool CIDX = false>
 __global__ void __launch_bounds__(64 * NW, (M > (NW == 2 ? 40 : H_TWO_WAVE_MAX) && R > 1) ? 1 : 2) wave_hpass_kernel(WavePassArgs a)
 {
     static_assert(M % 4 == 0 && M >= 4, "chunk length must be a multiple of 4");
     static_assert(NW == 1 || NW == 2, "one or two wavefronts per row");
     constexpr bool LO = FUSED == FUSE_LO || FUSED == FUSE_LO_HALF;
+    static_assert(!(CIDX && LO), "the low-resolution forms read float weights");
+    constexpr int HEADN = 32 * M;
+    constexpr int MQ8 = (M + 7) / 8;
     __shared__ float4 stage_all[NW][LO ? lo_stage_vec4(M) : M * 16];
     __shared__ float xch[NW == 2 ? 5 : 1];
     __shared__ float red[NW == 2 ? 5 : 1][NW == 2 ? 128 : 1];
@@ -53,7 +57,24 @@
     constexpr int MQ = M / 4;
     float c[M], f0[M], f1[M];
 
-    float4 tC[M / 4], t0[M / 4], t1[M / 4];
+    float4 tC[CIDX ? 1 : M / 4], t0[M / 4], t1[M / 4];
+    uint4 tI[CIDX ? MQ8 : 1];
+    if constexpr (CIDX) {
+#pragma unroll
+        for (int k = 0; k < (8 * M + 63) / 64; k++) {
+            const int q = 64 * k + lane;
+            if (q < 8 * M) stage[8 * M + q] = reinterpret_cast<const float4*>(a.lut)[q];
+        }
+        typedef unsigned v4u __attribute__((ext_vector_type(4)));
+        const v4u* sI = reinterpret_cast<const v4u*>(reinterpret_cast<const uint16_t*>(a.C) + off);
+        const int nvecI = a.pitch >> 3;
+#pragma unroll
+        for (int k = 0; k < MQ8; k++) {
+            const int q = 64 * k + lane;
+            tI[k] = make_uint4(0u, 0u, 0u, 0u);
+            if (q < 8 * M && wv * 8 * M + q < nvecI) { const v4u v = __builtin_nontemporal_load(sI + wv * 8 * M + q); tI[k] = make_uint4(v.x, v.y, v.z, v.w); }
+        }
+    }
     {
         const float4* sC = reinterpret_cast<const float4*>(a.C + off);
         const float4* s0 = reinterpret_cast<const float4*>(a.U0 + offU);
@@ -261,10 +282,12 @@
 #pragma unroll
         for (int k = 0; k < M / 4; k++) {
             const int idx = v0 + 64 * k + lane, uidx = u0 + 64 * k + lane;
-            tC[k] = make_float4(0.f, 0.f, 0.f, 0.f); t0[k] = tC[k]; t1[k] = tC[k];
+            t0[k] = make_float4(0.f, 0.f, 0.f, 0.f); t1[k] = t0[k];
+            if constexpr (!CIDX) tC[k] = t0[k];
             if (FUSED == FUSE_VIEW) draw[k] = make_short4(0, 0, 0, 0);
             if (FUSED == FUSE_VIEW) {
                 typedef float v4f __attribute__((ext_vector_type(4)));
+                if constexpr (!CIDX)
                 if (idx < nvec) { const v4f q = __builtin_nontemporal_load(reinterpret_cast<const v4f*>(sC) + idx); tC[k] = make_float4(q.x, q.y, q.z, q.w); }
                 if (idx < nfused) {
                     const v4f cq = __builtin_nontemporal_load(reinterpret_cast<const v4f*>(sF) + idx);
@@ -275,6 +298,7 @@
                 }
             } else {
                 typedef float v4f __attribute__((ext_vector_type(4)));
+                if constexpr (!CIDX)
                 if (idx < nvec) { const v4f q = __builtin_nontemporal_load(reinterpret_cast<const v4f*>(sC) + idx); tC[k] = make_float4(q.x, q.y, q.z, q.w); }
                 if (uidx < nvecU) { const v4f q = __builtin_nontemporal_load(reinterpret_cast<const v4f*>(s0) + ADF_PIDX(uidx)); t0[k] = make_float4(q.x, q.y, q.z, q.w); }
                 if (PAIR && uidx + 64 * MQ < nvecU) { const v4f q = __builtin_nontemporal_load(reinterpret_cast<const v4f*>(s0) + ADF_PIDX(uidx + 64 * MQ)); t1[k] = make_float4(q.x, q.y, q.z, q.w); }
@@ -326,7 +350,47 @@
         }                                                                                 \
         __syncthreads();                                                                  \
     }
+    if constexpr (CIDX) {
+#pragma unroll
+        for (int k = 0; k < MQ8; k++)
+            if (64 * k + lane < 8 * M) reinterpret_cast<uint4*>(stage)[64 * k + lane] = tI[k];
+        __syncthreads();
+        const uintptr_t lb = reinterpret_cast<uintptr_t>(a.lut);
+        const unsigned llo = (unsigned)__builtin_amdgcn_readfirstlane((int)(unsigned)(lb & 0xffffffffu));
+        const unsigned lhi = (unsigned)__builtin_amdgcn_readfirstlane((int)(unsigned)(lb >> 32));
+        const __amdgpu_buffer_rsrc_t lutwin = __builtin_amdgcn_make_buffer_rsrc(reinterpret_cast<void*>((uintptr_t)llo | ((uintptr_t)lhi << 32)), (short)0,
+                                                                                (int)(sizeof(float) * (WIDX_MAX + 1)), 0x00020000);
+        const float* head = reinterpret_cast<const float*>(stage + 8 * M);
+        const uint2* mine = reinterpret_cast<const uint2*>(stage) + lane * MQ;
+        auto index_of = [](const uint2& q, int e) -> unsigned { const unsigned w = (e & 2) ? q.y : q.x; return (e & 1) ? w >> 16 : w & 0xffffu; };
+#pragma unroll
+        for (int k = 0; k < MQ; k++) {
+            const uint2 q = mine[k];
+#pragma unroll
+            for (int e = 0; e < 4; e++) {
+                const unsigned ix = index_of(q, e);
+                c[4 * k + e] = __uint_as_float(__builtin_amdgcn_raw_buffer_load_b32(lutwin, ix >= (unsigned)HEADN ? ix * 4u : H_DROP, 0, 0));
+            }
+            ADF_STEP_FENCE();
+        }
+        const int lim = a.len - 1 - (64 * wv + lane) * M;
+#pragma unroll
+        for (int k = 0; k < MQ; k++) {
+            const uint2 q = mine[k];
+#pragma unroll
+            for (int e = 0; e < 4; e++) {
+                const int i = 4 * k + e;
+                const unsigned l = __float_as_uint(head[min(index_of(q, e), (unsigned)HEADN - 1u)]);
+                const unsigned gq = __float_as_uint(c[i]);
+                c[i] = __uint_as_float(i < lim ? (gq != 0u ? gq : l) : 0u) * a.lambda;
+                asm volatile("" : "+v"(c[i]));
+            }
+            ADF_STEP_FENCE();
+        }
+        __syncthreads();
+    } else {
     ADF_TRANSPOSE_IN(tC, c, a.lambda)
+    }
     if (PAIR && FUSED == FUSE_NONE) {
         ADF_PAIR_IN(t0, 0)
         ADF_PAIR_IN(t1, 1)
@@ -427,6 +491,12 @@
             hipLaunchKernelGGL((wave_hpass_kernel<M, 2, FUSE_LO_HALF, NW>), grid, block, 0, st, a);
         else
             hipLaunchKernelGGL((wave_hpass_kernel<M, 2, FUSE_LO, NW>), grid, block, 0, st, a);
+    } else if (a.c_fmt == WFMT_U16) {
+        if (a.fuse.conf_in) {
+            if (n_rhs != 2) return hipErrorInvalidValue;
+            hipLaunchKernelGGL((wave_hpass_kernel<M, 2, FUSE_VIEW, NW, true>), grid, block, 0, st, a);
+        } else if (n_rhs == 2) hipLaunchKernelGGL((wave_hpass_kernel<M, 2, FUSE_NONE, NW, true>), grid, block, 0, st, a);
+        else hipLaunchKernelGGL((wave_hpass_kernel<M, 1, FUSE_NONE, NW, true>), grid, block, 0, st, a);
     } else if (a.fuse.conf_in) {
         if (n_rhs != 2) return hipErrorInvalidValue;
         hipLaunchKernelGGL((wave_hpass_kernel<M, 2, FUSE_VIEW, NW>), grid, block, 0, st, a);
@@ -492,6 +562,7 @@
 {
     if (a.len < 2 || a.len > wave_max_row_len() || a.pitch % 64 != 0 || a.pitch < a.len) return hipErrorInvalidValue;
     if (a.fuse.lo_conf && !wave_hpass_can_fuse_lo(a)) return hipErrorInvalidValue;
+    if (a.c_fmt == WFMT_U16 && (a.fuse.lo_conf || !a.lut)) return hipErrorInvalidValue;
     if (!a.fuse.lo_conf && a.fuse.conf_in && !wave_hpass_can_fuse(a)) return hipErrorInvalidValue;
     return dispatch_index<N_ROW_BUCKETS>(bucket_index(ROW_BUCKETS, a.len), [&](auto I) {
         constexpr Bucket b = ROW_BUCKETS[decltype(I)::value];
diff --git a/addingdisparityfiltering_amd/csrc/fgs_wave_v.hip b/addingdisparityfiltering_amd/csrc/fgs_wave_v.hip
--- a/addingdisparityfiltering_amd/csrc/fgs_wave_v.hip
+++ b/addingdisparityfiltering_amd/csrc/fgs_wave_v.hip
@@ -244,6 +244,7 @@
 hipError_t launch_wave_vpass(const WavePassArgs& a, int n_rhs, int epilogue, int n_pairs, hipStream_t st)
 {
     if (a.len < 2 || a.len > wave_max_col_len() || a.pitch % 64 != 0 || a.pitch < a.nscan) return hipErrorInvalidValue;
+    if (a.c_fmt != WFMT_F32) return hipErrorInvalidValue;
     return dispatch_index<N_COL_BUCKETS>(bucket_index(COL_BUCKETS, a.len), [&](auto I) {
         constexpr Bucket b = COL_BUCKETS[decltype(I)::value];
         return launch_v<b.m, b.chunks == 64 ? VC : VC / 2, b.chunks>(a, n_rhs, epilogue, n_pairs, st);
diff --git a/addingdisparityfiltering_amd/csrc/prep_bodies.h b/addingdisparityfiltering_amd/csrc/prep_bodies.h
--- a/addingdisparityfiltering_amd/csrc/prep_bodies.h
+++ b/addingdisparityfiltering_amd/csrc/prep_bodies.h
@@ -1,5 +1,7 @@
 #pragma once
 #include "adf_internal.h"
+
+#include <type_traits>
 
 namespace adf {
 namespace prep {
@@ -123,22 +125,46 @@
         wv[k] = p.g[WS_COLS + k] != 0u ? __uint_as_float(p.g[WS_COLS + k]) : p.wl[WS_COLS + k];
     }
 }
-
+struct WsPendingV { float wl[WS_COLS]; unsigned g[WS_COLS]; };
+__device__ __forceinline__ void ws_lookup_issue(const float* lut_head, const __amdgpu_buffer_rsrc_t& lutwin, const int (&vidx)[WS_COLS], WsPendingV& p)
+{
+#pragma unroll
+    for (int k = 0; k < WS_COLS; k++) p.wl[k] = lut_head[min(vidx[k], WS_LUT_HEAD - 1)];
+#pragma unroll
+    for (int k = 0; k < WS_COLS; k++)
+        p.g[k] = __builtin_amdgcn_raw_buffer_load_b32(lutwin, vidx[k] >= WS_LUT_HEAD ? (unsigned)vidx[k] * 4u : WS_DROP, 0, 0);
+}
+__device__ __forceinline__ void ws_lookup_finish(const WsPendingV& p, float (&wv)[WS_COLS])
+{
+#pragma unroll
+    for (int k = 0; k < WS_COLS; k++) wv[k] = p.g[k] != 0u ? __uint_as_float(p.g[k]) : p.wl[k];
+}
+
+template <class WT = float>
 struct WsOut {
+    static constexpr unsigned HSZ = sizeof(WT), VSZ = sizeof(float);
     __amdgpu_buffer_rsrc_t chor, cvert; unsigned mh[WS_COLS], mv[WS_COLS]; unsigned ho, vo, hstep, vstep; bool st_ok, strip;
     __device__ __forceinline__ void init(const WeightArgs& a, size_t pz, int j0, int y_first)
     {
         const Geom& g = a.g;
-        chor = ws_window(a.chor + pz * g.plane, g.plane * sizeof(float));
-        cvert = ws_window(a.cvert + pz * g.plane, g.plane * sizeof(float));
+        chor = ws_window(reinterpret_cast<const char*>(a.chor) + pz * g.plane * HSZ, g.plane * HSZ);
+        cvert = ws_window(a.cvert + pz * g.plane, g.plane * VSZ);
         strip = a.cvert_orient == ORIENT_STRIP;
 #pragma unroll
         for (int k = 0; k < WS_COLS; k++) { mh[k] = (j0 + k < g.rw - 1) ? 0xffffffffu : 0u; mv[k] = (j0 + k < g.rw) ? 0xffffffffu : 0u; }
         st_ok = j0 >= 0 && j0 < g.pw;
-        ho = ((unsigned)y_first * (unsigned)g.pw + (unsigned)j0) * 4u;
+        ho = ((unsigned)y_first * (unsigned)g.pw + (unsigned)j0) * HSZ;
         vo = (strip ? ((unsigned)(j0 >> 4) * (unsigned)g.rh + (unsigned)y_first) * ADF_STRIP + (unsigned)(j0 & 15)
-                    : (unsigned)y_first * (unsigned)g.pw + (unsigned)j0) * 4u;
-        hstep = (unsigned)g.pw * 4u; vstep = (strip ? (unsigned)ADF_STRIP : (unsigned)g.pw) * 4u;
+                    : (unsigned)y_first * (unsigned)g.pw + (unsigned)j0) * VSZ;
+        hstep = (unsigned)g.pw * HSZ; vstep = (strip ? (unsigned)ADF_STRIP : (unsigned)g.pw) * VSZ;
+    }
+    __device__ __forceinline__ void store_h(int t, const int (&hidx)[WS_COLS], bool on) const
+    {
+        unsigned q[WS_COLS];
+#pragma unroll
+        for (int k = 0; k < WS_COLS; k++) q[k] = min((unsigned)hidx[k], (unsigned)WIDX_MAX) & mh[k];
+        __builtin_amdgcn_raw_buffer_store_b64(ws_v2u{q[0] | (q[1] << 16), q[2] | (q[3] << 16)}, chor,
+                                              (on && st_ok) ? ho + (unsigned)t * hstep : WS_DROP, 0, 2 );
     }
     __device__ __forceinline__ void store_h(int t, const float (&wh)[WS_COLS], bool on) const
     {
@@ -159,15 +185,16 @@
     }
 };
 
-template <int CH>
+template <int CH, class WT = float>
 __device__ __forceinline__ void weights_stream_body(const WeightArgs& a, int bx, int by, int nby, size_t pz, WsShared<CH>& sh, bool active)
 {
     static_assert(CH == 1 || CH == 3, "guides have one or three channels");
-    float (&lut_head)[WS_LUT_HEAD] = sh.lut_head;
+    constexpr bool INDEX = std::is_same_v<WT, uint16_t>;
+    static_assert(INDEX || std::is_same_v<WT, float>, "planes of floats or of uint16 indices");
     const Geom& g = a.g;
     const int tid = active ? (int)threadIdx.x : 0;
     if (active)
-        for (int q = tid; q < WS_LUT_HEAD; q += WS_NT) lut_head[q] = a.lut[q];
+        for (int q = tid; q < WS_LUT_HEAD; q += WS_NT) sh.lut_head[q] = a.lut[q];
     __syncthreads();
     const int ws_rows = (g.rh + nby - 1) / nby;
     const int x0 = bx * WS_BCOLS, y0 = by * ws_rows;
@@ -185,20 +212,22 @@
     auto row_off = [&](int n) -> unsigned { return col_off + (unsigned)(min(y0 + n, g.rh - 1) - y0) * gd.stride; };
     auto load = [&](int n) -> WsWin<CH> { return ws_load<CH>(gd, (row_off(n) & ~3u) + lane_off); };
 
-    WsOut out;
+    WsOut<WT> out;
     out.init(a, pz, j0, y0);
-    const __amdgpu_buffer_rsrc_t lutwin = ws_window(a.lut, sizeof(float) * ADF_LUT_LEVELS);
     WsPrev<CH> pv;
 #pragma unroll
     for (int k = 0; k < WS_COLS; k++) { pv.q[k] = 0; pv.qa[k] = 0; }
     WsWin<CH> nxt[WS_U], cur[WS_U];
 #pragma unroll
     for (int s = 0; s < WS_U; s++) nxt[s] = load(s < nrows ? s : nrows - 1);
-    WsPending pend;
+    float (&lut_head)[WS_LUT_HEAD] = sh.lut_head;
+    const __amdgpu_buffer_rsrc_t lutwin = ws_window(a.lut, sizeof(float) * ADF_LUT_LEVELS);
+    std::conditional_t<INDEX, WsPendingV, WsPending> pend;
     {
         int hidx[WS_COLS], vidx[WS_COLS];
         ws_indices<CH>(nxt[0], row_off(0) & 3u, pv, hidx, vidx);
-        ws_lookup_issue(lut_head, lutwin, hidx, vidx, pend);
+        if constexpr (INDEX) { out.store_h(0, hidx, 0 < nrows - 1); ws_lookup_issue(lut_head, lutwin, vidx, pend); }
+        else ws_lookup_issue(lut_head, lutwin, hidx, vidx, pend);
     }
     for (int n0 = 0; n0 < nrows; n0 += WS_U) {
 #pragma unroll
@@ -211,15 +240,19 @@
 #pragma unroll
         for (int s = 0; s < WS_U; s++) {
             const int n = n0 + s;
-            WsPending ahead;
+            decltype(pend) ahead;
             {
                 int hidx[WS_COLS], vidx[WS_COLS];
                 ws_indices<CH>(s + 1 < WS_U ? cur[s + 1 < WS_U ? s + 1 : 0] : nxt[0], row_off(min(n + 1, nrows - 1)) & 3u, pv, hidx, vidx);
-                ws_lookup_issue(lut_head, lutwin, hidx, vidx, ahead);
+                if constexpr (INDEX) { out.store_h(n + 1, hidx, n + 1 < nrows - 1); ws_lookup_issue(lut_head, lutwin, vidx, ahead); }
+                else ws_lookup_issue(lut_head, lutwin, hidx, vidx, ahead);
             }
             float wh[WS_COLS], wv[WS_COLS];
-            ws_lookup_finish(pend, wh, wv);
-            out.store_h(n, wh, n < nrows - 1);
+            if constexpr (INDEX) ws_lookup_finish(pend, wv);
+            else {
+                ws_lookup_finish(pend, wh, wv);
+                out.store_h(n, wh, n < nrows - 1);
+            }
             out.store_v(n - 1, wv, y0 + n - 1 == g.rh - 1, n >= 1 && n < nrows);
             pend = ahead;
         }
diff --git a/addingdisparityfiltering_amd/csrc/weights_kernels.hip b/addingdisparityfiltering_amd/csrc/weights_kernels.hip
--- a/addingdisparityfiltering_amd/csrc/weights_kernels.hip
+++ b/addingdisparityfiltering_amd/csrc/weights_kernels.hip
@@ -96,11 +96,11 @@
     }
 }
 
-template <int CH>
+template <int CH, class WT>
 __global__ void __launch_bounds__(prep::WS_NT) weights_stream_kernel(WeightArgs a)
 {
     __shared__ prep::WsShared<CH> sh;
-    prep::weights_stream_body<CH>(a, blockIdx.x, blockIdx.y, gridDim.y, blockIdx.z, sh, true);
+    prep::weights_stream_body<CH, WT>(a, blockIdx.x, blockIdx.y, gridDim.y, blockIdx.z, sh, true);
 }
 
 __global__ void __launch_bounds__(256) transpose_n_to_t_kernel(const float* __restrict__ src, float* __restrict__ dst, Geom g)
@@ -128,6 +128,17 @@
     }
 }
 
+bool force_generic()
+{
+    static const bool f = [] { const char* e = getenv("ADF_WEIGHTS_GENERIC"); return e && atoi(e) != 0; }();
+    return f;
+}
+
+}
+
+bool weights_index_fits(ptrdiff_t guide_stride, int W, int channels)
+{
+    return !force_generic() && guide_stride > 0 && guide_stride < ((ptrdiff_t)1 << 29) && (size_t)W * channels < ((size_t)1 << 29);
 }
 
 hipError_t launch_weights(const WeightArgs& a, int n_pairs, hipStream_t st)
@@ -142,8 +153,9 @@
         return hipGetLastError();
     }
     if (a.cvert_orient != ORIENT_N && !(a.cvert_orient == ORIENT_STRIP && a.chor_orient == ORIENT_N)) return hipErrorInvalidValue;
-    static const bool force_generic = [] { const char* e = getenv("ADF_WEIGHTS_GENERIC"); return e && atoi(e) != 0; }();
-    if (!force_generic && a.chor_orient == ORIENT_N && a.stride > 0 && a.stride < ((ptrdiff_t)1 << 29) && (size_t)a.g.W * a.ch < ((size_t)1 << 29)) {
+    const bool index = a.fmt == WFMT_U16;
+    if (index && !(a.chor_orient == ORIENT_N && a.cvert_orient == ORIENT_STRIP && weights_index_fits(a.stride, a.g.W, a.ch))) return hipErrorInvalidValue;
+    if (a.chor_orient == ORIENT_N && weights_index_fits(a.stride, a.g.W, a.ch)) {
         dim3 sgrid((a.g.rw + prep::WS_BCOLS - 1) / prep::WS_BCOLS, 1, n_pairs);
         {
             int rpb = 128;
@@ -152,8 +164,10 @@
             while (rpb > 1 && (size_t)(rpb + 1) * (size_t)a.stride >= ((size_t)1 << 30)) rpb >>= 1;
             sgrid.y = (a.g.rh + rpb - 1) / rpb;
         }
-        if (a.ch == 1) hipLaunchKernelGGL(weights_stream_kernel<1>, sgrid, dim3(prep::WS_NT), 0, st, a);
-        else if (a.ch == 3) hipLaunchKernelGGL(weights_stream_kernel<3>, sgrid, dim3(prep::WS_NT), 0, st, a);
+        if (a.ch == 1 && index) hipLaunchKernelGGL((weights_stream_kernel<1, uint16_t>), sgrid, dim3(prep::WS_NT), 0, st, a);
+        else if (a.ch == 3 && index) hipLaunchKernelGGL((weights_stream_kernel<3, uint16_t>), sgrid, dim3(prep::WS_NT), 0, st, a);
+        else if (a.ch == 1) hipLaunchKernelGGL((weights_stream_kernel<1, float>), sgrid, dim3(prep::WS_NT), 0, st, a);
+        else if (a.ch == 3) hipLaunchKernelGGL((weights_stream_kernel<3, float>), sgrid, dim3(prep::WS_NT), 0, st, a);
         else return hipErrorInvalidValue;
         return hipGetLastError();
     }
diff --git a/addingdisparityfiltering_amd/ximgproc.py b/addingdisparityfiltering_amd/ximgproc.py
--- a/addingdisparityfiltering_amd/ximgproc.py
+++ b/addingdisparityfiltering_amd/ximgproc.py
@@ -4,7 +4,7 @@
 import numpy as np
 
 from . import _lib
-from ._lib import AdfError, PATH_CONF_BAND, PATH_FUSED_FIRST_PASS, PATH_MERGED_PREP, PATH_SCALED_FUSED, PATH_SCALED_HALF, Rect, SOLVER_EXACT, SOLVER_WAVE
+from ._lib import AdfError, PATH_CONF_BAND, PATH_FUSED_FIRST_PASS, PATH_MERGED_PREP, PATH_SCALED_FUSED, PATH_SCALED_HALF, Rect, SOLVER_EXACT, SOLVER_WAVE, WEIGHT_AUTO, WEIGHT_FLOAT, WEIGHT_INDEX
 
 try:
     import torch
@@ -183,6 +183,15 @@
 
     def getLastSolver(self):
         return _read(_lib.lib().adf_wls_get_last_solver, C.c_int, self._h)
+
+    def setWeightFormat(self, fmt):
+        _lib.check(_lib.lib().adf_wls_set_weight_format(self._h, int(fmt)))
+
+    def getWeightFormat(self):
+        return _read(_lib.lib().adf_wls_get_weight_format, C.c_int, self._h)
+
+    def getLastWeightFormat(self):
+        return _read(_lib.lib().adf_wls_get_last_weight_format, C.c_int, self._h)
 
     def getLastPath(self):
         return _read(_lib.lib().adf_wls_get_last_path, C.c_int, self._h)
diff --git a/include/adf_wls.h b/include/adf_wls.h
--- a/include/adf_wls.h
+++ b/include/adf_wls.h
@@ -57,6 +57,12 @@
 #define ADF_PATH_SCALED_FUSED 8
 #define ADF_PATH_SCALED_HALF 16
 int adf_wls_get_last_path(const adf_wls_t* h, int* path_flags);
+#define ADF_WEIGHT_AUTO 0
+#define ADF_WEIGHT_FLOAT 1
+#define ADF_WEIGHT_INDEX 2
+int adf_wls_set_weight_format(adf_wls_t* h, int format);
+int adf_wls_get_weight_format(const adf_wls_t* h, int* format);
+int adf_wls_get_last_weight_format(const adf_wls_t* h, int* format);
 
 int adf_wls_filter_device(adf_wls_t* h, int n_pairs,
                           const int16_t* disp_left, ptrdiff_t disp_left_stride, ptrdiff_t disp_left_pair_stride,
```

Measured after the change: 42900 (median of 6 runs). 1.05x the previous value.
